# aticejiang/MLAgg-UNet

Measured on AMD Instinct MI355X. Metric: images/sec (train step) MLAgg-UNet-2D 256x256 bs10, higher is better.
Workload: dtype f32; 1 GPU; nnUNetTrainer_MLAgg_2D_dt_MS train step, AbdomenMRI-shaped 256x256x1, 14 classes, attention variant B (BASELINE.json configs[1]); batch_per_gpu=10, global_batch=10, parallelism=dp1, launch=eager, miopen=tuned find-db (mlagg-unet_amd/miopen_db), library_gemm=TunableOp table (mlagg-unet_amd/gemm_db), tuning off

## Files before the change

include/mlagg_hip.h:

```cpp
#ifndef MLAGG_HIP_H
#define MLAGG_HIP_H

#include <stddef.h>

#ifdef __cplusplus
extern "C" {
#endif

#define MLAGG_E_UNSUPPORTED (-1)
#define MLAGG_E_NULLPTR     (-2)
#define MLAGG_E_WORKSPACE   (-3)

#define MLAGG_DTYPE_F32  0
#define MLAGG_DTYPE_BF16 1
#define MLAGG_DTYPE_F16  2
#define MLAGG_DTYPE_BF16X3 3

const char *mlagg_version(void);
const char *mlagg_error_string(int code);

int mlagg_profile_kernel_count(void);
const char *mlagg_profile_kernel_name(int id);
int mlagg_profile_select(int id);
int mlagg_profile_collect(double *ms, int *counts);

size_t mlagg_selscan_state_floats(int batch, int dim, int L, int N);
int mlagg_selscan_fwd(const float *u, const float *delta, const float *A, const float *B, const float *C,
                      const float *D, const float *delta_bias, float *out, float *chunk_state,
                      int batch, int dim, int L, int N, int G, int delta_softplus, void *stream);

size_t mlagg_selscan_bwd_workspace_floats(int batch, int dim, int L, int N);
int mlagg_selscan_bwd(const float *u, const float *delta, const float *A, const float *B, const float *C,
                      const float *D, const float *delta_bias, const float *dout, const float *chunk_state,
                      float *du, float *ddelta, float *dA, float *dB, float *dC, float *dD,
                      float *ddelta_bias, float *workspace,
                      int batch, int dim, int L, int N, int G, int delta_softplus, void *stream);

int mlagg_selscan_lowrank_fwd(const float *u, const float *dtr, const float *Wdt, int R, const float *A, const float *B,
                              const float *C, const float *D, const float *delta_bias, float *out, float *chunk_state,
                              int batch, int dim, int L, int N, int G, int delta_softplus, void *stream);
int mlagg_selscan_lowrank_bwd(const float *u, const float *dtr, const float *Wdt, int R, const float *A, const float *B,
                              const float *C, const float *D, const float *delta_bias, const float *dout,
                              const float *chunk_state, float *du, float *ddtr, float *dWdt, float *dA, float *dB,
                              float *dC, float *dD, float *ddelta_bias, float *workspace, int batch, int dim, int L,
                              int N, int G, int delta_softplus, void *stream);

int mlagg_local_attn_fwd(const float *q, int q_stride, const float *kv, int kv_stride,
                         const float *lam, const float *subln_w, const float *lepe_w, const float *lepe_b,
                         float *out, int out_stride, int batch, int H, int W, int nh, float scale,
                         void *stream);
size_t mlagg_local_attn_bwd_workspace_floats(int batch, int H, int W, int nh);
int mlagg_local_attn_bwd(const float *q, int q_stride, const float *kv, int kv_stride,
                         const float *lam, const float *subln_w, const float *lepe_w,
                         const float *dout, int dout_stride,
                         float *dq, int dq_stride, float *dkv, int dkv_stride,
                         float *dlam, float *dsubln_w, float *dlepe_w, float *dlepe_b, float *workspace,
                         int batch, int H, int W, int nh, float scale, void *stream);

int mlagg_pooled_attn_fwd(const float *q, int q_stride, const float *kp, int kp_stride,
                          const float *vp, int vp_stride, const float *lam, const float *subln_w,
                          float *out, int out_stride,
                          float *lse,
                          float *o_pre,
                          int batch, int N, int P, int nh, float scale, void *stream);
size_t mlagg_pooled_attn_bwd_workspace_floats(int batch, int N, int P, int nh);
int mlagg_pooled_attn_bwd(const float *q, int q_stride, const float *kp, int kp_stride,
                          const float *vp, int vp_stride, const float *lam, const float *subln_w,
                          const float *dout, int dout_stride, const float *lse, const float *o_pre,
                          float *dq, int dq_stride, float *dkp, int dkp_stride, float *dvp, int dvp_stride,
                          float *dlam, float *dsubln_w, float *workspace,
                          int batch, int N, int P, int nh, float scale, void *stream);

int mlagg_dwconv3x3_fwd(const float *x, int x_stride, const float *w, const float *bias, const float *res, float *y,
                        int y_stride, float *pre, int batch, int H, int W, int C, int silu, void *stream);
size_t mlagg_dwconv3x3_bwd_workspace_floats(int batch, int H, int W, int C);
int mlagg_dwconv3x3_gated_fwd(const float *x, int x_stride, const float *w, const float *bias, const float *gate, int gate_stride, float *y,
                              int y_stride, float *pre, int batch, int H, int W, int C, void *stream);
int mlagg_dwconv3x3_gated_bwd(const float *x, int x_stride, const float *w, const float *dy, int dy_stride, const float *pre,
                              const float *gate, int gate_stride, float *dx, int dx_stride, float *dgate, int dgate_stride, float *dw,
                              float *dbias, float *workspace, int batch, int H, int W, int C, void *stream);
int mlagg_dwconv3x3_bwd(const float *x, int x_stride, const float *w, const float *dy, int dy_stride,
                        const float *pre, float *dx, int dx_stride, float *dw, float *dbias, float *workspace,
                        int batch, int H, int W, int C, int silu, void *stream);

int mlagg_linear_fwd(const float *x, int x_stride, const float *w, const float *bias, float *y, int y_stride,
                     int M, int N, int K, void *stream);
int mlagg_linear_dgrad(const float *dy, int dy_stride, const float *w, float *dx, int dx_stride, int M, int O, int I,
                       void *stream);
int mlagg_linear_lp_fwd(const float *x, int x_stride, const float *w, const float *bias, float *y, int y_stride,
                        int M, int N, int K, int dtype, void *stream);
int mlagg_linear_lp_dgrad(const float *dy, int dy_stride, const float *w, float *dx, int dx_stride, int M, int O, int I,
                          int dtype, void *stream);
size_t mlagg_linear_wgrad_workspace_floats(int M, int O, int I);
int mlagg_linear_wgrad(const float *dy, int dy_stride, const float *x, int x_stride, float *dW, float *db,
                       float *workspace, int M, int O, int I, void *stream);
int mlagg_linear_wgrad_x3(const float *dy, int dy_stride, const float *x, int x_stride, float *dW, float *db, float *workspace,
                          int M, int O, int I, void *stream);

int mlagg_flash_attn_fwd(const void *q, const void *k, const void *v, void *out, float *lse, int B, int N, int P, int nh,
                         int head_dim, float softmax_scale, int dtype, void *stream);
size_t mlagg_flash_attn_bwd_workspace_floats(int B, int N, int P, int nh, int head_dim);
int mlagg_flash_attn_bwd(const void *q, const void *k, const void *v, const void *out, const void *dout, const float *lse,
                         void *dq, float *workspace, int B, int N, int P, int nh, int head_dim, float softmax_scale,
                         int dtype, void *stream);

int mlagg_layernorm_supported(int C);
int mlagg_layernorm_fwd(const float *x, int x_stride, const float *gamma, const float *beta, float *y,
                        float *stats, int rows, int C, float eps, void *stream);
size_t mlagg_layernorm_bwd_workspace_floats(int rows, int C);
int mlagg_layernorm_bwd(const float *x, int x_stride, const float *dy, int dy_stride, const float *gamma,
                        const float *stats, float *dx, float *dgamma, float *dbeta, float *workspace,
                        int rows, int C, void *stream);
int mlagg_residual_layernorm_fwd(const float *skip, const float *branch, const float *scale, const float *gamma, const float *beta,
                                 float *xsum, float *y, float *stats, int rows, int rows_per_sample, int C, float eps, void *stream);
int mlagg_residual_layernorm_bwd(const float *xsum, const float *dy, int dy_stride, const float *dres, const float *scale,
                                 const float *gamma, const float *stats, float *dskip, float *dbranch, float *dgamma, float *dbeta,
                                 float *workspace, int rows, int rows_per_sample, int C, void *stream);

int mlagg_dwconv3d_fwd(const float *x, int x_stride, const float *w, const float *bias, float *y, int y_stride,
                       float *pre, int batch, int D, int H, int W, int C, int silu, void *stream);
size_t mlagg_dwconv3d_bwd_workspace_floats(int batch, int D, int H, int W, int C);
int mlagg_dwconv3d_bwd(const float *x, int x_stride, const float *w, const float *dy, int dy_stride, const float *pre,
                       float *dx, int dx_stride, float *dw, float *dbias, float *workspace, int batch, int D, int H,
                       int W, int C, int silu, void *stream);

int mlagg_dwconv3x3_nchw_fwd(const float *x, const float *w, const float *bias, float *y, int B, int C, int H, int W,
                             int stride, void *stream);
size_t mlagg_dwconv3x3_nchw_bwd_workspace_floats(int B, int C, int H, int W, int stride);
int mlagg_dwconv3x3_nchw_bwd(const float *x, const float *w, const float *dy, float *dx, float *dw, float *dbias,
                             float *workspace, int B, int C, int H, int W, int stride, void *stream);
int mlagg_dwconv3x3_nchw_bwd_res(const float *x, const float *w, const float *dy, const float *dres, float *dx, float *dw, float *dbias,
                                 float *workspace, int B, int C, int H, int W, int stride, void *stream);

int mlagg_cross_scan(const float *tok, int tok_stride, int blk_stride, float *seq, int B, int nscale,
                     const int *H, const int *W, int CB, int nblk, void *stream);
int mlagg_cross_merge(const float *seq, float *tok, int tok_stride, int blk_stride, int B, int nscale,
                      const int *H, const int *W, int CB, int nblk, void *stream);

int mlagg_conv1x1_supported(int O, int I, long P);
int mlagg_conv1x1_fwd(const float *x, long x_batch, const float *w, const float *bias, float *y, long y_batch, int B, int O, int I,
                      long P, void *stream);
size_t mlagg_conv1x1_wgrad_workspace_floats(int B, int O, int I, long P);
int mlagg_conv1x1_wgrad(const float *dy, long dy_batch, const float *x, long x_batch, float *dW, float *workspace, int B, int O,
                        int I, long P, void *stream);
int mlagg_conv1x1_fwd_lp(const float *x, long x_batch, const float *w, const float *bias, float *y, long y_batch, int B, int O, int I,
                         long P, int dtype, void *stream);
int mlagg_conv1x1_wgrad_lp(const float *dy, long dy_batch, const float *x, long x_batch, float *dW, float *workspace, int B, int O,
                           int I, long P, int dtype, void *stream);
int mlagg_conv1x1_fwd_ragged(const float *x, long x_batch, const float *w, const float *bias, float *y, long y_batch, int B, int O, int I,
                             int I_valid, long P, int dtype, void *stream);
int mlagg_conv1x1_fwd_acc(const float *x, long x_batch, const float *w, const float *bias, float *y, long y_batch, int B, int O, int I,
                          int I_valid, long P, int dtype, int accumulate, void *stream);

int mlagg_conv3x3_supported(int O, int I, int H, int W);
size_t mlagg_conv3x3_workspace_bytes(int O, int I);
int mlagg_conv3x3_fwd(const float *x, long x_batch, const float *w, int transposed, const float *bias, float *y, long y_batch,
                      void *workspace, int B, int O, int I, int H, int W, void *stream);
int mlagg_conv3x3x3_supported(int O, int I, int D, int H, int W);
size_t mlagg_conv3x3x3_workspace_bytes(int O, int I);
int mlagg_conv3x3x3_fwd(const float *x, long x_batch, const float *w, int transposed, const float *bias, float *y, long y_batch,
                        void *workspace, int B, int O, int I, int D, int H, int W, void *stream);
int mlagg_conv3x3_wgrad_supported(int O, int I, int H, int W);
int mlagg_conv3x3x3_wgrad_supported(int O, int I, int D, int H, int W);
size_t mlagg_conv3x3x3_wgrad_workspace_floats(int B, int O, int I, int D, int H, int W);
int mlagg_conv3x3x3_wgrad(const float *dy, long dy_batch, const float *x, long x_batch, float *dW, float *workspace, int B, int O,
                          int I, int D, int H, int W, void *stream);
size_t mlagg_conv3x3_wgrad_workspace_floats(int B, int O, int I, int H, int W);
int mlagg_conv3x3_wgrad(const float *dy, long dy_batch, const float *x, long x_batch, float *dW, float *workspace, int B, int O,
                        int I, int H, int W, void *stream);
int mlagg_conv3x3_fwd_lp(const float *x, long x_batch, const float *w, int transposed, const float *bias, float *y, long y_batch,
                         void *workspace, int B, int O, int I, int H, int W, int dtype, void *stream);
int mlagg_conv3x3_wgrad_lp(const float *dy, long dy_batch, const float *x, long x_batch, float *dW, float *workspace, int B, int O,
                           int I, int H, int W, int dtype, void *stream);

int mlagg_conv3x3_s2t_supported(int O, int I, int H, int W);
size_t mlagg_conv3x3_s2t_workspace_bytes(int O, int I);
int mlagg_conv3x3_s2t_fwd(const float *x, long x_batch, const float *w, float *y, long y_batch, void *workspace, int B, int O, int I,
                          int H, int W, int dtype, void *stream);
int mlagg_conv3x3_s2_dgrad(const float *dy, long dy_batch, long dy_chan_stride, long dy_row_stride, const float *w, float *dx,
                           long dx_batch, void *workspace, int B, int O, int I, int H, int W, int dtype, void *stream);
size_t mlagg_conv3x3_s2t_wgrad_workspace_floats(int B, int O, int I, int H, int W);
int mlagg_conv3x3_s2t_wgrad(const float *x, long x_batch, const float *dy, long dy_batch, long dy_chan_stride, long dy_row_stride,
                            float *dW, float *workspace, int B, int O, int I, int H, int W, int dtype, void *stream);

int mlagg_gelu_pool_fwd(const float *s, int s_stride, float *pooled, int batch, int H, int W, int d, int r, void *stream);
int mlagg_gelu_pool_bwd(const float *s, int s_stride, const float *dpooled, float *ds, int ds_stride, int batch, int H, int W, int d,
                        int r, void *stream);

int mlagg_gate_fwd(const float *a0, const float *a1, const float *act, int act_stride, float *out, long rows, int h,
                   void *stream);
int mlagg_gate_bwd(const float *dout, int dout_stride, const float *a0, const float *a1, const float *act, int act_stride,
                   float *da0, float *da1, float *dact, int dact_stride, long rows, int h, void *stream);

int mlagg_diff_lambda_fwd(const float *q1, const float *k1, const float *q2, const float *k2, float lambda_init, int n,
                          float *lam, float *saved_exp, void *stream);
int mlagg_diff_lambda_bwd(const float *dlam, const float *q1, const float *k1, const float *q2, const float *k2,
                          const float *saved_exp, int n, float *dq1, float *dk1, float *dq2, float *dk2, void *stream);
int mlagg_scaled_residual(const float *skip, const float *branch, const float *scale, float *out, int batch,
                          long per_sample, void *stream);
int mlagg_transpose_2d(const float *src, long src_batch_stride, float *dst, int batch, int R, int C, void *stream);
int mlagg_transpose_2d_into(const float *src, long src_batch_stride, float *dst, long dst_batch_stride, int batch, int R, int C,
                            void *stream);
int mlagg_pixel_shuffle2(const float *src, float *dst, int B, int O, int H, int W, int inverse, void *stream);
int mlagg_pixel_unshuffle2_strided(const float *src, long src_batch, float *dst, int B, int O, int H, int W, void *stream);
size_t mlagg_channel_sum_workspace_floats(int B, int C);
int mlagg_channel_sum(const float *g, float *out, float *workspace, int B, int C, long HW, void *stream);
size_t mlagg_column_sum_workspace_floats(int rows, int cols);
int mlagg_column_sum(const float *x, int x_stride, float *out, float *workspace, int rows, int cols, void *stream);

int mlagg_index_scan(const float *tok, long tok_stride, int blk_stride, const int *idx, float *seq, int B, int L, int K, int CB,
                     void *stream);
int mlagg_index_merge(const float *seq, const int *idx, float *tok, long tok_stride, int blk_stride, int B, int L, int K, int CB,
                      void *stream);
int mlagg_block_sum(const float *wide, float *out, long rows, int K, int CB, void *stream);

int mlagg_msmm_scan_supported(int d_inner, int d_state, int dt_rank, int directions, int L);
size_t mlagg_msmm_scan_state_floats(int batch, int L);
size_t mlagg_msmm_scan_fwd_workspace_floats(int batch, int L);
size_t mlagg_msmm_scan_bwd_workspace_floats(int batch, int L);
int mlagg_msmm_scan_fwd(const float *xc, const float *xdbl, const int *idx, const float *Wdt, const float *A, const float *D,
                        const float *delta_bias, float *y, float *state, float *workspace, int batch, int L, void *stream);
int mlagg_msmm_scan_bwd(const float *xc, const float *xdbl, const int *idx, const float *Wdt, const float *A, const float *D,
                        const float *delta_bias, const float *dy, const float *state, float *dxc, float *dxdbl, float *dWdt,
                        float *dA, float *dD, float *ddelta_bias, float *workspace, int batch, int L, void *stream);

int mlagg_selscan1_chunk(int B, int L, int K);
size_t mlagg_selscan1_state_floats(int B, int L, int C, int K);
int mlagg_selscan1_fwd(const float *tok, long tok_stride, const int *idx, const float *dtr, const float *Bs, const float *Cs,
                       const float *Wdt, int R, const float *A, const float *D, const float *bias, float *yk, float *state,
                       int B, int L, int C, int K, void *stream);
size_t mlagg_selscan1_bwd_workspace_floats(int B, int L, int C, int K, int R);
int mlagg_selscan1_bwd(const float *tok, long tok_stride, const int *idx, const float *dtr, const float *Bs, const float *Cs,
                       const float *Wdt, int R, const float *A, const float *D, const float *bias, const float *dout,
                       long dout_stride, const float *state, float *duk, float *ddtr, float *dBs, float *dCs, float *dparams,
                       float *workspace, int B, int L, int C, int K, void *stream);

int mlagg_channel_epilogue_fwd(float *x, const float *bias, const float *res, float *y, int B, int C, long HW, int act,
                               void *stream);
int mlagg_channel_gelu_bwd(const float *pre, const float *dy, float *dpre, float *dbias, float *workspace, int B, int C,
                           long HW, void *stream);
int mlagg_channel_epilogue_lp_fwd(const void *x, int x_dtype, const float *bias, const void *res, int res_dtype, void *y, int y_dtype,
                                  int B, int C, long HW, int act, void *stream);
int mlagg_channel_epilogue_lp_bwd(const void *x, int x_dtype, const float *bias, const void *res, int res_dtype, const void *dy,
                                  int dy_dtype, void *dx, int dx_dtype, float *dbias, float *workspace, int B, int C, long HW, int act,
                                  void *stream);

int mlagg_dice_ce_max_classes(void);
size_t mlagg_dice_ce_stats_workspace_floats(int B, int C, long HW);
int mlagg_dice_ce_stats(const float *logits, const float *target, float *stats_ip, float *stats_g, float *ce_sum,
                        float *workspace, int B, int C, long HW, int ignore_label, void *stream);
int mlagg_dice_ce_grad(const float *logits, const float *target, const float *g_ip, const float *g_ce, float *dlogits, int B,
                       int C, long HW, int ignore_label, void *stream);

size_t mlagg_plane_norm_fwd_workspace_floats(int B, int C, long HW);
int mlagg_plane_norm_fwd(const void *x, const float *gamma, const float *beta, const void *res, void *y, float *stats,
                         float *workspace, int B, int C, long HW, float eps, int act, float slope, int x_dtype, int res_dtype,
                         int y_dtype, void *stream);
size_t mlagg_plane_norm_bwd_workspace_floats(int B, int C, long HW);
int mlagg_plane_norm_bwd(const void *x, const void *dy, const float *gamma, const float *beta, const void *res, const float *stats,
                         void *dx, void *dres, float *dgamma, float *dbeta, float *workspace, int B, int C, long HW, int act,
                         float slope, int x_dtype, int dy_dtype, int res_dtype, void *stream);
int mlagg_plane_norm_bwd_strided(const void *x, const void *dy, long dy_batch, const float *gamma, const float *beta, const void *res,
                                 const float *stats, void *dx, void *dres, float *dgamma, float *dbeta, float *workspace, int B, int C,
                                 long HW, int act, float slope, int x_dtype, int dy_dtype, int res_dtype, void *stream);

int mlagg_pooled_attn_lp_fwd(const float *q, int q_stride, const float *kp, int kp_stride, const float *vp, int vp_stride,
                             const float *lam, const float *subln_w, float *out, int out_stride, float *lse, float *o1, float *o2,
                             int batch, int N, int P, int nh, float scale, int dtype, void *stream);
size_t mlagg_pooled_attn_lp_bwd_workspace_floats(int batch, int N, int P, int nh);
int mlagg_pooled_attn_lp_bwd(const float *q, int q_stride, const float *kp, int kp_stride, const float *vp, int vp_stride,
                             const float *lam, const float *subln_w, const float *dout, int dout_stride, const float *lse,
                             const float *o1, const float *o2, float *dq, int dq_stride, float *dkp, int dkp_stride, float *dvp,
                             int dvp_stride, float *dlam, float *dsubln_w, float *workspace, int batch, int N, int P, int nh,
                             float scale, int dtype, void *stream);

int mlagg_conv_pad_geometry(int D, int H, int W, int stride, int wide, int *Dq, int *Hq, int *Wq, long *guard);
int mlagg_volume_pad(const float *src, float *dst, int B, int C, int D, int H, int W, int stride, int wide, int as_output, int out_D,
                     int out_H, int out_W, void *stream);
size_t mlagg_conv_wgrad_taps_workspace_floats(int batch, long Q, int O, int I, int ntaps);
int mlagg_conv_taps(const float *xp, long x_batch, long x_row, const float *weight, long w_so, long w_si, int flip, const long *tap_off,
                    int ntaps, float *y, int B, int O, int I, int D, int H, int W, void *stream);
int mlagg_conv_wgrad_taps(const float *A, long a_batch, long a_row, const float *B, long b_batch, long b_row, const long *tap_off,
                          int ntaps, long Q, int O, int I, int batch, float *dW, int accumulate, float *workspace, void *stream);

size_t mlagg_weight_image_bytes(int rows, int cols);
int mlagg_weight_image(const float *w, int w_stride, void *img, void *img_t, int N, int K, void *stream);
int mlagg_weight_images(const void *jobs, int n_jobs, int max_tiles, void *stream);
int mlagg_linear_x3_supported(int M, int N, int K);
int mlagg_linear_x3(const float *x, int x_stride, const void *w_image, const float *bias, float *y, int y_stride, float *y_act,
                    const float *pre, int pre_stride, int M, int N, int K, int epilogue, void *stream);

int mlagg_adamw_chunk_elements(void);
int mlagg_adamw_clip_step(const void *tensor_table, const void *work_list, int n_work, double *sumsq, float lr, float beta1,
                          float beta2, float eps, float weight_decay, float max_norm, int step, void *stream);
int mlagg_adamw_clip_step_dev(const void *tensor_table, const void *work_list, int n_work, double *sumsq, const float *lr_dev,
                              int *step_dev, float beta1, float beta2, float eps, float weight_decay, float max_norm, void *stream);

int mlagg_sw_gather(const float *vol, int C, int X, int Y, int Z, const int *origins, int n, const int *flips, int V, float *out,
                    int tx, int ty, int tz, void *stream);
int mlagg_sw_fold(const float *out, int tile, int n, const int *flips, int V, int K, const float *gauss, int tx, int ty, int tz,
                  int ox, int oy, int oz, float *acc, float *w, int X, int Y, int Z, void *stream);
int mlagg_sw_finalize(const float *acc, const float *w, int K, int X, int Y, int Z, int lx, int ly, int lz, int X0, int Y0, int Z0,
                      float *logits, long long *labels, void *stream);

int mlagg_resample_linear(const float *in, int C, int X, int Y, int Z, long long sc, long long sx, long long sy, long long sz,
                          const int *tap_idx, const double *tap_w, float *out, int Xo, int Yo, int Zo, void *stream);
int mlagg_export_segmentation(const float *logits, int K, int X, int Y, int Z, long long sc, long long sx, long long sy, long long sz,
                              const int *tap_idx, const double *tap_w, int Xc, int Yc, int Zc, const int *box_lo, const int *shape,
                              const int *perm, unsigned char *labels, float *probs, void *stream);

#define MLAGG_PP_NONE          0
#define MLAGG_PP_CT            1
#define MLAGG_PP_ZSCORE        2
#define MLAGG_PP_ZSCORE_MASKED 3
#define MLAGG_PP_RESCALE01     4
#define MLAGG_PP_RGB01         5
#define MLAGG_PP_STATS_PARTIALS 256
int mlagg_pp_nonzero_box(const float *in, int C, int X, int Y, int Z, long long sc, long long sx, long long sy, long long sz, int *box,
                         void *stream);
int mlagg_pp_channel_stats(const float *in, int C, int X, int Y, int Z, long long sc, long long sx, long long sy, long long sz,
                           const int *lo, const int *ext, int c, int scheme, const unsigned char *mask, double *partials,
                           float *params, double *stats, void *stream);
int mlagg_pp_normalize(const float *in, int C, int X, int Y, int Z, long long sc, long long sx, long long sy, long long sz,
                       const int *lo, const int *ext, const int *schemes, const float *params, const unsigned char *mask, float *out,
                       void *stream);
int mlagg_pp_clip_ranges(const float *x, int C, int X, int Y, int Z, int axis, unsigned *lo, unsigned *hi, void *stream);
int mlagg_pp_cubic_lines_per_block(int n_in, int M);
int mlagg_pp_cubic_axis(const void *in, int in_f64, void *out, int out_f64, long long outer, int n_in, long long inner, int n_out,
                        const int *start, const double *w, int P0, int M, const double *fir, const unsigned *clip_lo,
                        const unsigned *clip_hi, long long clip_cstride, long long clip_dstride, int clip_D, void *stream);
int mlagg_pp_gather_axis(const double *in, float *out, long long outer, int n_in, long long inner, int n_out, const int *idx,
                         const double *w, void *stream);

#define MLAGG_PP_RANK_BLOCK 2048
#define MLAGG_PP_MAX_GROUPS 64
int mlagg_pp_seg_crop(const short *seg, int X, int Y, int Z, long long sx, long long sy, long long sz, const int *lo, const int *ext,
                      const unsigned char *mask, short *out, int max_label, unsigned long long *hist, void *stream);
int mlagg_pp_seg_resize(const short *in, int X, int Y, int Z, const int *tap_idx, const double *tap_w, short *out, int Xo, int Yo,
                        int Zo, int max_label, unsigned long long *hist, void *stream);
size_t mlagg_pp_rank_rows(long long N);
int mlagg_pp_rank_counts(const short *seg, long long N, const unsigned long long *groups, int max_label, int n_groups,
                         long long *table, long long *totals, void *stream);
int mlagg_pp_rank_select(const short *seg, long long N, int Y, int Z, const unsigned long long *groups, int max_label, int n_groups,
                         int group, const long long *table, const long long *totals, const long long *ranks, long long n_ranks,
                         long long *coords, const float *image, int C, long long sc, long long sx, long long sy, long long sz,
                         float *values, void *stream);

int mlagg_keep_largest_component(const unsigned char *labels, int X, int Y, int Z, const unsigned char *group, int background_label,
                                 int *parent, int *size, int *stats, unsigned char *out, void *stream);

#define MLAGG_SURFACE_STATS_PER_LABEL 10
#define MLAGG_SURFACE_DESC_FIELDS 16
#define MLAGG_SURFACE_MAX_LINE 2560
int mlagg_surface_stats(const unsigned char *gt, const unsigned char *pred, int X, int Y, int Z, const unsigned char *wanted,
                        int *stats, void *stream);
int mlagg_surface_prepare(const unsigned char *gt, const unsigned char *pred, int X, int Y, int Z, const long long *desc, int n_labels,
                          long long total, long long max_crop, long long zlines, long long ylines, int nmax_y, double s1, double s2, unsigned char *codes,
                          int *ft, int *counts, void *stream);
int mlagg_surface_reduce(const unsigned char *codes, const int *ft, const long long *desc, int n_labels, long long total,
                         long long xlines, int nmax_x, const double *tol, const double *area, double s0, double s1, double s2,
                         double *partial, double *sums, double *pairs, int *pair_count, void *stream);

int mlagg_aug3d_resample(const float *vol, const short *lab, int B, int C, int Xi, int Yi, int Zi, const double *affine,
                         const int *resample, float *out, float *out_lab, int Xo, int Yo, int Zo, void *stream);

#ifdef __cplusplus
}
#endif
#endif
```

mlagg-unet_amd/csrc/channel_epilogue.hip:

```cpp
#include <hip/hip_runtime.h>
#include <stdint.h>

#include "internal.h"
#include "lpio.h"
#include "mlagg_hip.h"
#include "prof.h"

namespace {

__device__ __forceinline__ float gelu_f(float x) { return 0.5f * x * (1.f + erff(x * 0.70710678118654752f)); }
__device__ __forceinline__ float gelu_grad_f(float x)
{
    const float cdf = 0.5f * (1.f + erff(x * 0.70710678118654752f));
    return cdf + x * 0.3989422804014327f * __expf(-0.5f * x * x);
}

template <bool GELU>
__global__ void __launch_bounds__(256)
channel_epilogue_fwd_kernel(float *__restrict__ x, const float *__restrict__ bias, const float *__restrict__ res,
                            float *__restrict__ y, int C, long HW)
{
    const int c = blockIdx.x, b = blockIdx.y;
    const size_t off = ((size_t)b * C + c) * HW;
    const float bv = bias ? bias[c] : 0.f;
    float *xp = x + off;
    const float *rp = res ? res + off : nullptr;
    float *yp = GELU ? y + off : xp;
    const long n4 = ((HW & 3) == 0) ? HW >> 2 : 0;
    for (long i = threadIdx.x; i < n4; i += 256) {
        float4 v = reinterpret_cast<float4 *>(xp)[i];
        v.x += bv; v.y += bv; v.z += bv; v.w += bv;
        if (rp) {
            const float4 r = reinterpret_cast<const float4 *>(rp)[i];
            v.x += r.x; v.y += r.y; v.z += r.z; v.w += r.w;
        }
        if (GELU) {
            reinterpret_cast<float4 *>(xp)[i] = v;
            v = make_float4(gelu_f(v.x), gelu_f(v.y), gelu_f(v.z), gelu_f(v.w));
        }
        reinterpret_cast<float4 *>(yp)[i] = v;
    }
    for (long i = 4 * n4 + threadIdx.x; i < HW; i += 256) {
        float v = xp[i] + bv + (rp ? rp[i] : 0.f);
        if (GELU) { xp[i] = v; v = gelu_f(v); }
        yp[i] = v;
    }
}

__global__ void __launch_bounds__(256)
channel_gelu_bwd_kernel(const float *__restrict__ pre, const float *__restrict__ dy, float *__restrict__ dpre,
                        float *__restrict__ part, int C, long HW)
{
    __shared__ float red[4];
    const int c = blockIdx.x, b = blockIdx.y;
    const size_t off = ((size_t)b * C + c) * HW;
    const float *pp = pre + off, *gp = dy + off;
    float *dp = dpre + off;
    float s = 0.f;
    const long n4 = ((HW & 3) == 0) ? HW >> 2 : 0;
    for (long i = threadIdx.x; i < n4; i += 256) {
        const float4 p = reinterpret_cast<const float4 *>(pp)[i], g = reinterpret_cast<const float4 *>(gp)[i];
        const float4 d = make_float4(g.x * gelu_grad_f(p.x), g.y * gelu_grad_f(p.y), g.z * gelu_grad_f(p.z), g.w * gelu_grad_f(p.w));
        reinterpret_cast<float4 *>(dp)[i] = d;
        s += (d.x + d.y) + (d.z + d.w);
    }
    for (long i = 4 * n4 + threadIdx.x; i < HW; i += 256) {
        const float d = gp[i] * gelu_grad_f(pp[i]);
        dp[i] = d;
        s += d;
    }
    if (part) {
#pragma unroll
        for (int o = 32; o > 0; o >>= 1) s += __shfl_xor(s, o, 64);
        if ((threadIdx.x & 63) == 0) red[threadIdx.x >> 6] = s;
        __syncthreads();
        if (threadIdx.x == 0) part[(size_t)b * C + c] = (red[0] + red[1]) + (red[2] + red[3]);
    }
}

using namespace mlagg_lpio;

template <bool GELU>
__global__ void __launch_bounds__(256)
channel_epilogue_lp_fwd_kernel(const void *__restrict__ x, int xdt, const float *__restrict__ bias, const void *__restrict__ res, int rdt,
                               void *__restrict__ y, int ydt, int C, long HW)
{
    const int c = blockIdx.x, b = blockIdx.y;
    const long plane = (long)b * C + c;
    const float bv = bias ? bias[c] : 0.f;
    const void *xp = plane_ptr(x, plane, HW, xdt);
    const void *rp = res ? plane_ptr(res, plane, HW, rdt) : nullptr;
    void *yp = plane_ptr(y, plane, HW, ydt);
    const long n4 = HW >> 2;
    constexpr int UN = 4;
    for (long i0 = threadIdx.x; i0 < n4; i0 += 256 * UN) {
        float4 v[UN], r[UN];
#pragma unroll
        for (int u = 0; u < UN; ++u) {
            const long i = min(i0 + 256 * u, n4 - 1);
            v[u] = ld4(xp, i, xdt);
            r[u] = rp ? ld4(rp, i, rdt) : make_float4(0.f, 0.f, 0.f, 0.f);
        }
#pragma unroll
        for (int u = 0; u < UN; ++u) {
            const long i = i0 + 256 * u;
            if (i < n4) {
                float4 o = make_float4(v[u].x + bv + r[u].x, v[u].y + bv + r[u].y, v[u].z + bv + r[u].z, v[u].w + bv + r[u].w);
                if (GELU) o = make_float4(gelu_f(o.x), gelu_f(o.y), gelu_f(o.z), gelu_f(o.w));
                st4(yp, i, ydt, o);
            }
        }
    }
}

template <bool GELU>
__global__ void __launch_bounds__(256)
channel_epilogue_lp_bwd_kernel(const void *__restrict__ x, int xdt, const float *__restrict__ bias, const void *__restrict__ res, int rdt,
                               const void *__restrict__ dy, int gdt, void *__restrict__ dx, int dxdt, float *__restrict__ part, int C,
                               long HW)
{
    __shared__ float red[4];
    const int c = blockIdx.x, b = blockIdx.y;
    const long plane = (long)b * C + c;
    const float bv = (GELU && bias) ? bias[c] : 0.f;
    const void *xp = GELU ? plane_ptr(x, plane, HW, xdt) : nullptr;
    const void *rp = (GELU && res) ? plane_ptr(res, plane, HW, rdt) : nullptr;
    const void *gp = plane_ptr(dy, plane, HW, gdt);
    void *dp = plane_ptr(dx, plane, HW, dxdt);
    const long n4 = HW >> 2;
    float s = 0.f;
    constexpr int UN = 4;
    for (long i0 = threadIdx.x; i0 < n4; i0 += 256 * UN) {
        float4 v[UN], r[UN], g[UN];
#pragma unroll
        for (int u = 0; u < UN; ++u) {
            const long i = min(i0 + 256 * u, n4 - 1);
            g[u] = ld4(gp, i, gdt);
            v[u] = GELU ? ld4(xp, i, xdt) : make_float4(0.f, 0.f, 0.f, 0.f);
            r[u] = rp ? ld4(rp, i, rdt) : make_float4(0.f, 0.f, 0.f, 0.f);
        }
#pragma unroll
        for (int u = 0; u < UN; ++u) {
            const long i = i0 + 256 * u;
            if (i < n4) {
                float4 d = g[u];
                if (GELU)
                    d = make_float4(d.x * gelu_grad_f(v[u].x + bv + r[u].x), d.y * gelu_grad_f(v[u].y + bv + r[u].y),
                                    d.z * gelu_grad_f(v[u].z + bv + r[u].z), d.w * gelu_grad_f(v[u].w + bv + r[u].w));
                st4(dp, i, dxdt, d);
                s += (d.x + d.y) + (d.z + d.w);
            }
        }
    }
    if (part) {
#pragma unroll
        for (int o = 32; o > 0; o >>= 1) s += __shfl_xor(s, o, 64);
        if ((threadIdx.x & 63) == 0) red[threadIdx.x >> 6] = s;
        __syncthreads();
        if (threadIdx.x == 0) part[plane] = (red[0] + red[1]) + (red[2] + red[3]);
    }
}

inline bool lp_ok(int dt) { return dt == MLAGG_DTYPE_F32 || dt == MLAGG_DTYPE_BF16 || dt == MLAGG_DTYPE_F16; }
inline bool lp_aligned(const void *p, int dt) { return (((uintptr_t)p) & (dt == 0 ? 15 : 7)) == 0; }

}

extern "C" int mlagg_channel_epilogue_lp_fwd(const void *x, int x_dtype, const float *bias, const void *res, int res_dtype, void *y,
                                             int y_dtype, int B, int C, long HW, int act, void *stream)
{
    if (!x || !y) return MLAGG_E_NULLPTR;
    if (B <= 0 || C <= 0 || HW <= 0 || B > 65535 || (HW & 3) || (act != 0 && act != 1)) return MLAGG_E_UNSUPPORTED;
    if (!lp_ok(x_dtype) || !lp_ok(y_dtype) || (res && !lp_ok(res_dtype))) return MLAGG_E_UNSUPPORTED;
    if (!lp_aligned(x, x_dtype) || !lp_aligned(y, y_dtype) || (res && !lp_aligned(res, res_dtype))) return MLAGG_E_UNSUPPORTED;
    hipStream_t st = static_cast<hipStream_t>(stream);
    MLAGG_TIMED(K_CHANNEL_EPI, st);
    if (act == 1) hipLaunchKernelGGL(channel_epilogue_lp_fwd_kernel<true>, dim3(C, B), dim3(256), 0, st, x, x_dtype, bias, res, res_dtype, y, y_dtype, C, HW);
    else hipLaunchKernelGGL(channel_epilogue_lp_fwd_kernel<false>, dim3(C, B), dim3(256), 0, st, x, x_dtype, bias, res, res_dtype, y, y_dtype, C, HW);
    return (int)hipGetLastError();
}

extern "C" int mlagg_channel_epilogue_lp_bwd(const void *x, int x_dtype, const float *bias, const void *res, int res_dtype,
                                             const void *dy, int dy_dtype, void *dx, int dx_dtype, float *dbias, float *workspace,
                                             int B, int C, long HW, int act, void *stream)
{
    if (!dy || !dx || (act == 1 && !x) || (dbias && !workspace)) return MLAGG_E_NULLPTR;
    if (B <= 0 || C <= 0 || HW <= 0 || B > 65535 || (HW & 3) || (act != 0 && act != 1)) return MLAGG_E_UNSUPPORTED;
    if (!lp_ok(dy_dtype) || !lp_ok(dx_dtype) || (act == 1 && !lp_ok(x_dtype)) || (act == 1 && res && !lp_ok(res_dtype))) return MLAGG_E_UNSUPPORTED;
    if (!lp_aligned(dy, dy_dtype) || !lp_aligned(dx, dx_dtype) || (act == 1 && !lp_aligned(x, x_dtype)) ||
        (act == 1 && res && !lp_aligned(res, res_dtype)))
        return MLAGG_E_UNSUPPORTED;
    hipStream_t st = static_cast<hipStream_t>(stream);
    MLAGG_TIMED(K_CHANNEL_EPI, st);
    float *part = dbias ? workspace : nullptr;
    if (act == 1) hipLaunchKernelGGL(channel_epilogue_lp_bwd_kernel<true>, dim3(C, B), dim3(256), 0, st, x, x_dtype, bias, res, res_dtype, dy, dy_dtype, dx, dx_dtype, part, C, HW);
    else hipLaunchKernelGGL(channel_epilogue_lp_bwd_kernel<false>, dim3(C, B), dim3(256), 0, st, x, x_dtype, bias, res, res_dtype, dy, dy_dtype, dx, dx_dtype, part, C, HW);
    if (dbias)
        hipLaunchKernelGGL(mlagg_internal::column_sum_kernel<false>, dim3((C + 63) / 64), dim3(1024), 0, st, workspace, B, C, C, dbias);
    return (int)hipGetLastError();
}

extern "C" int mlagg_channel_epilogue_fwd(float *x, const float *bias, const float *res, float *y, int B, int C, long HW, int act,
                                          void *stream)
{
    if (!x || (act == 1 && !y)) return MLAGG_E_NULLPTR;
    if (B <= 0 || C <= 0 || HW <= 0 || B > 65535 || (act != 0 && act != 1)) return MLAGG_E_UNSUPPORTED;
    if ((((uintptr_t)x) & 15) || (res && (((uintptr_t)res) & 15)) || (y && (((uintptr_t)y) & 15))) return MLAGG_E_UNSUPPORTED;
    hipStream_t st = static_cast<hipStream_t>(stream);
    MLAGG_TIMED(K_CHANNEL_EPI, st);
    if (act == 1) hipLaunchKernelGGL(channel_epilogue_fwd_kernel<true>, dim3(C, B), dim3(256), 0, st, x, bias, res, y, C, HW);
    else hipLaunchKernelGGL(channel_epilogue_fwd_kernel<false>, dim3(C, B), dim3(256), 0, st, x, bias, res, y, C, HW);
    return (int)hipGetLastError();
}

extern "C" int mlagg_channel_gelu_bwd(const float *pre, const float *dy, float *dpre, float *dbias, float *workspace, int B, int C,
                                      long HW, void *stream)
{
    if (!pre || !dy || !dpre || (dbias && !workspace)) return MLAGG_E_NULLPTR;
    if (B <= 0 || C <= 0 || HW <= 0 || B > 65535) return MLAGG_E_UNSUPPORTED;
    if ((((uintptr_t)pre) & 15) || (((uintptr_t)dy) & 15) || (((uintptr_t)dpre) & 15)) return MLAGG_E_UNSUPPORTED;
    hipStream_t st = static_cast<hipStream_t>(stream);
    MLAGG_TIMED(K_CHANNEL_EPI, st);
    hipLaunchKernelGGL(channel_gelu_bwd_kernel, dim3(C, B), dim3(256), 0, st, pre, dy, dpre, dbias ? workspace : nullptr, C, HW);
    if (dbias)
        hipLaunchKernelGGL(mlagg_internal::column_sum_kernel<false>, dim3((C + 63) / 64), dim3(1024), 0, st, workspace, B, C, C, dbias);
    return (int)hipGetLastError();
}
```

mlagg-unet_amd/csrc/conv1x1.hip:

```cpp
#include <hip/hip_runtime.h>

#include <cstdlib>

#include "mlagg_hip.h"
#include "prof.h"
#include "bf16x3.h"
#include "opmode.h"
#include "internal.h"

namespace {

using bf16x3::f32x16;

template <int T>
struct __attribute__((packed, aligned(4))) FVec {
    float v[T];
};

struct C1Geom {
    int B, O, I, P;
    long x_batch, y_batch;
    int I_valid;
    int accumulate;
};

using opmode::split8;

template <int TO, int TP, int DT>
__global__ void __launch_bounds__(64)
conv1x1_fwd_kernel(const float *__restrict__ X, const float *__restrict__ W, const float *__restrict__ bias, float *__restrict__ Y,
                   C1Geom g)
{
    const int lane = threadIdx.x, col = lane & 31, kh = lane >> 5;
    const int p0 = blockIdx.x * (32 * TP), o0 = blockIdx.y * (32 * TO), b = blockIdx.z;
    f32x16 acc[TO][TP];
#pragma unroll
    for (int a = 0; a < TO; ++a)
#pragma unroll
        for (int j = 0; j < TP; ++j)
#pragma unroll
            for (int r = 0; r < 16; ++r) acc[a][j][r] = 0.f;
    const int pnat = p0 + TP * col, pc = min(pnat, g.P - TP);
    const float *xb = X + (size_t)b * g.x_batch + pc;
    const int lastrow = g.I_valid - 1;
    const float *wb[TO];
#pragma unroll
    for (int a = 0; a < TO; ++a) wb[a] = W + (size_t)min(o0 + 32 * a + col, g.O - 1) * g.I + 8 * kh;
    const int nblk = g.I / 16;
    float4 wa[2][TO][2];
    FVec<TP> xv[2][8];
    auto fetch = [&](float4 (&A)[TO][2], FVec<TP> (&Xv)[8], int blk) {
        const int kb = 16 * min(blk, nblk - 1);
#pragma unroll
        for (int t = 0; t < 8; ++t) Xv[t] = *reinterpret_cast<const FVec<TP> *>(xb + (size_t)min(kb + 8 * kh + t, lastrow) * g.P);
#pragma unroll
        for (int a = 0; a < TO; ++a) {
            A[a][0] = *reinterpret_cast<const float4 *>(wb[a] + kb);
            A[a][1] = *reinterpret_cast<const float4 *>(wb[a] + kb + 4);
        }
    };
    auto consume = [&](const float4 (&A)[TO][2], const FVec<TP> (&Xv)[8]) {
        uint4 bq[TP][3];
#pragma unroll
        for (int j = 0; j < TP; ++j) {
            const float f[8] = {Xv[0].v[j], Xv[1].v[j], Xv[2].v[j], Xv[3].v[j], Xv[4].v[j], Xv[5].v[j], Xv[6].v[j], Xv[7].v[j]};
            split8<DT>(f, bq[j]);
        }
        uint4 aq[TO][3];
#pragma unroll
        for (int a = 0; a < TO; ++a) {
            const float f[8] = {A[a][0].x, A[a][0].y, A[a][0].z, A[a][0].w, A[a][1].x, A[a][1].y, A[a][1].z, A[a][1].w};
            split8<DT>(f, aq[a]);
        }
        opmode::mfma_tiles<DT, TO, TP>(aq, bq, acc);
    };
    fetch(wa[0], xv[0], 0);
    int blk = 0;
    for (; blk + 2 <= nblk; blk += 2) {
        fetch(wa[1], xv[1], blk + 1);
        consume(wa[0], xv[0]);
        fetch(wa[0], xv[0], blk + 2);
        consume(wa[1], xv[1]);
    }
    if (blk < nblk) consume(wa[0], xv[0]);
    float *yb = Y + (size_t)b * g.y_batch + pc;
#pragma unroll
    for (int a = 0; a < TO; ++a) {
#pragma unroll
        for (int r = 0; r < 16; ++r) {
            const int o = o0 + 32 * a + (r & 3) + 8 * (r >> 2) + 4 * kh;
            if (o >= g.O) continue;
            const float bv = bias ? bias[o] : 0.f;
            float *dst = yb + (size_t)o * g.P;
            if (pc == pnat) {
                FVec<TP> v;
#pragma unroll
                for (int j = 0; j < TP; ++j) v.v[j] = acc[a][j][r] + bv;
                if (g.accumulate) {
                    const FVec<TP> old = *reinterpret_cast<const FVec<TP> *>(dst);
#pragma unroll
                    for (int j = 0; j < TP; ++j) v.v[j] += old.v[j];
                }
                *reinterpret_cast<FVec<TP> *>(dst) = v;
            } else {
#pragma unroll
                for (int j = 0; j < TP; ++j)
                    if (pc + j >= pnat) dst[j] = acc[a][j][r] + bv + (g.accumulate ? dst[j] : 0.f);
            }
        }
    }
}

struct W1Geom {
    int B, O, I, P;
    long dy_batch, x_batch;
    int slab, nslabs;
};

template <int TO, int TI, int DT>
__global__ void __launch_bounds__(64)
conv1x1_wgrad_kernel(const float *__restrict__ dY, const float *__restrict__ X, float *__restrict__ part, W1Geom g)
{
    const int lane = threadIdx.x, col = lane & 31, kh = lane >> 5;
    const int b = blockIdx.x / g.nslabs, s = blockIdx.x % g.nslabs;
    const int o0 = blockIdx.y * (32 * TO), i0 = blockIdx.z * (32 * TI);
    f32x16 acc[TO][TI];
#pragma unroll
    for (int a = 0; a < TO; ++a)
#pragma unroll
        for (int j = 0; j < TI; ++j)
#pragma unroll
            for (int r = 0; r < 16; ++r) acc[a][j][r] = 0.f;
    const int pb = s * g.slab, pe = min(pb + g.slab, g.P);
    const int nblk = (pe - pb) / 16;
    const float *ap[TO], *bp[TI];
#pragma unroll
    for (int a = 0; a < TO; ++a) ap[a] = dY + (size_t)b * g.dy_batch + (size_t)min(o0 + 32 * a + col, g.O - 1) * g.P + pb + 8 * kh;
#pragma unroll
    for (int j = 0; j < TI; ++j) bp[j] = X + (size_t)b * g.x_batch + (size_t)min(i0 + 32 * j + col, g.I - 1) * g.P + pb + 8 * kh;
    float4 av[2][TO][2], bv[2][TI][2];
    auto fetch = [&](float4 (&A)[TO][2], float4 (&Bv)[TI][2], int blk) {
        const int off = 16 * min(blk, nblk - 1);
#pragma unroll
        for (int a = 0; a < TO; ++a) {
            A[a][0] = *reinterpret_cast<const float4 *>(ap[a] + off);
            A[a][1] = *reinterpret_cast<const float4 *>(ap[a] + off + 4);
        }
#pragma unroll
        for (int j = 0; j < TI; ++j) {
            Bv[j][0] = *reinterpret_cast<const float4 *>(bp[j] + off);
            Bv[j][1] = *reinterpret_cast<const float4 *>(bp[j] + off + 4);
        }
    };
    auto consume = [&](const float4 (&A)[TO][2], const float4 (&Bv)[TI][2]) {
        uint4 bq[TI][3];
#pragma unroll
        for (int j = 0; j < TI; ++j) {
            const float f[8] = {Bv[j][0].x, Bv[j][0].y, Bv[j][0].z, Bv[j][0].w, Bv[j][1].x, Bv[j][1].y, Bv[j][1].z, Bv[j][1].w};
            split8<DT>(f, bq[j]);
        }
        uint4 aq[TO][3];
#pragma unroll
        for (int a = 0; a < TO; ++a) {
            const float f[8] = {A[a][0].x, A[a][0].y, A[a][0].z, A[a][0].w, A[a][1].x, A[a][1].y, A[a][1].z, A[a][1].w};
            split8<DT>(f, aq[a]);
        }
        opmode::mfma_tiles<DT, TO, TI>(aq, bq, acc);
    };
    if (nblk > 0) {
        fetch(av[0], bv[0], 0);
        int blk = 0;
        for (; blk + 2 <= nblk; blk += 2) {
            fetch(av[1], bv[1], blk + 1);
            consume(av[0], bv[0]);
            fetch(av[0], bv[0], blk + 2);
            consume(av[1], bv[1]);
        }
        if (blk < nblk) consume(av[0], bv[0]);
    }
    float *prow = part + (size_t)blockIdx.x * ((size_t)g.O * g.I);
#pragma unroll
    for (int a = 0; a < TO; ++a) {
#pragma unroll
        for (int j = 0; j < TI; ++j) {
            const int i = i0 + 32 * j + col;
            if (i >= g.I) continue;
#pragma unroll
            for (int r = 0; r < 16; ++r) {
                const int o = o0 + 32 * a + (r & 3) + 8 * (r >> 2) + 4 * kh;
                if (o < g.O) prow[(size_t)o * g.I + i] = acc[a][j][r];
            }
        }
    }
}

int make_wgeom(W1Geom &g, int B, int O, int I, int P, long dy_batch, long x_batch)
{
    if (B <= 0 || O <= 0 || I <= 0 || P <= 0 || (P & 15)) return MLAGG_E_UNSUPPORTED;
    if (dy_batch < (long)O * P || x_batch < (long)I * P || ((dy_batch | x_batch) & 3)) return MLAGG_E_UNSUPPORTED;
    g = W1Geom{B, O, I, P, dy_batch, x_batch, 0, 0};
    const int og = (O + 95) / 96, ig = (I + 95) / 96;
    static const int target = [] { const char *e = getenv("MLAGG_K18_WAVES"); const int v = e ? atoi(e) : 0; return v > 0 ? v : 1536; }();
    int per_sample = (target + B * og * ig - 1) / (B * og * ig);
    if (per_sample < 1) per_sample = 1;
    int slab = (P + per_sample - 1) / per_sample;
    slab = ((slab + 15) / 16) * 16;
    if (slab < 64) slab = 64;
    g.slab = slab;
    g.nslabs = (P + slab - 1) / slab;
    if ((long)B * g.nslabs > 2147483647L || og > 65535 || ig > 65535) return MLAGG_E_UNSUPPORTED;
    return 0;
}

void pick_fwd_tile(int B, int O, int I, int P, int &to, int &tp)
{
    static const char *env = getenv("MLAGG_K18_TILE");
    if (env && env[0] >= '1' && env[0] <= '3' && env[1] == ',' && env[2] >= '1' && env[2] <= '3') {
        to = env[0] - '0';
        tp = env[2] - '0';
        if (32 * (to - 1) >= O) to = (O + 31) / 32;
    }
}

template <int TO, int TP>
void launch_fwd(const float *x, const float *w, const float *bias, float *y, const C1Geom &g, int dt, hipStream_t st)
{
    const dim3 grid((g.P + 32 * TP - 1) / (32 * TP), (g.O + 32 * TO - 1) / (32 * TO), g.B);
    if (dt == MLAGG_DTYPE_BF16)
        hipLaunchKernelGGL((conv1x1_fwd_kernel<TO, TP, MLAGG_DTYPE_BF16>), grid, dim3(64), 0, st, x, w, bias, y, g);
    else if (dt == MLAGG_DTYPE_F16)
        hipLaunchKernelGGL((conv1x1_fwd_kernel<TO, TP, MLAGG_DTYPE_F16>), grid, dim3(64), 0, st, x, w, bias, y, g);
    else
        hipLaunchKernelGGL((conv1x1_fwd_kernel<TO, TP, MLAGG_DTYPE_BF16X3>), grid, dim3(64), 0, st, x, w, bias, y, g);
}

template <int TO, int TI>
void launch_wgrad(const float *dy, const float *x, float *part, const W1Geom &g, int dt, hipStream_t st)
{
    const dim3 grid(g.B * g.nslabs, (g.O + 32 * TO - 1) / (32 * TO), (g.I + 32 * TI - 1) / (32 * TI));
    if (dt == MLAGG_DTYPE_BF16)
        hipLaunchKernelGGL((conv1x1_wgrad_kernel<TO, TI, MLAGG_DTYPE_BF16>), grid, dim3(64), 0, st, dy, x, part, g);
    else if (dt == MLAGG_DTYPE_F16)
        hipLaunchKernelGGL((conv1x1_wgrad_kernel<TO, TI, MLAGG_DTYPE_F16>), grid, dim3(64), 0, st, dy, x, part, g);
    else
        hipLaunchKernelGGL((conv1x1_wgrad_kernel<TO, TI, MLAGG_DTYPE_BF16X3>), grid, dim3(64), 0, st, dy, x, part, g);
}

}

extern "C" int mlagg_conv1x1_supported(int O, int I, long P)
{
    return O > 0 && I > 0 && (I % 16) == 0 && P >= 96 && (P % 16) == 0 && P < (1L << 30);
}

extern "C" int mlagg_conv1x1_fwd_ragged(const float *x, long x_batch, const float *w, const float *bias, float *y, long y_batch, int B,
                                        int O, int I, int I_valid, long P, int dtype, void *stream)
{
    return mlagg_conv1x1_fwd_acc(x, x_batch, w, bias, y, y_batch, B, O, I, I_valid, P, dtype, 0, stream);
}

extern "C" int mlagg_conv1x1_fwd_acc(const float *x, long x_batch, const float *w, const float *bias, float *y, long y_batch, int B,
                                     int O, int I, int I_valid, long P, int dtype, int accumulate, void *stream)
{
    if (!x || !w || !y) return MLAGG_E_NULLPTR;
    if (!opmode::valid(dtype) || I_valid <= 0 || I_valid > I) return MLAGG_E_UNSUPPORTED;
    if (B <= 0 || B > 65535 || !mlagg_conv1x1_supported(O, I, P)) return MLAGG_E_UNSUPPORTED;
    if (x_batch < (long)I_valid * P || y_batch < (long)O * P || (reinterpret_cast<uintptr_t>(w) & 15)) return MLAGG_E_UNSUPPORTED;
    C1Geom g{B, O, I, (int)P, x_batch, y_batch, I_valid, accumulate ? 1 : 0};
    hipStream_t st = static_cast<hipStream_t>(stream);
    MLAGG_TIMED(K_CONV1X1, st);
    int to = O <= 32 ? 1 : (O <= 64 ? 2 : 3), tp = O <= 64 ? 3 : 2;
    pick_fwd_tile(B, O, I, (int)P, to, tp);
    switch (to * 4 + tp) {
    case 1 * 4 + 1: launch_fwd<1, 1>(x, w, bias, y, g, dtype, st); break;
    case 1 * 4 + 2: launch_fwd<1, 2>(x, w, bias, y, g, dtype, st); break;
    case 1 * 4 + 3: launch_fwd<1, 3>(x, w, bias, y, g, dtype, st); break;
    case 2 * 4 + 1: launch_fwd<2, 1>(x, w, bias, y, g, dtype, st); break;
    case 2 * 4 + 2: launch_fwd<2, 2>(x, w, bias, y, g, dtype, st); break;
    case 2 * 4 + 3: launch_fwd<2, 3>(x, w, bias, y, g, dtype, st); break;
    case 3 * 4 + 1: launch_fwd<3, 1>(x, w, bias, y, g, dtype, st); break;
    case 3 * 4 + 2: launch_fwd<3, 2>(x, w, bias, y, g, dtype, st); break;
    default: launch_fwd<3, 3>(x, w, bias, y, g, dtype, st); break;
    }
    return (int)hipGetLastError();
}

extern "C" int mlagg_conv1x1_fwd_lp(const float *x, long x_batch, const float *w, const float *bias, float *y, long y_batch, int B,
                                    int O, int I, long P, int dtype, void *stream)
{
    return mlagg_conv1x1_fwd_ragged(x, x_batch, w, bias, y, y_batch, B, O, I, I, P, dtype, stream);
}

extern "C" int mlagg_conv1x1_fwd(const float *x, long x_batch, const float *w, const float *bias, float *y, long y_batch, int B,
                                 int O, int I, long P, void *stream)
{
    return mlagg_conv1x1_fwd_lp(x, x_batch, w, bias, y, y_batch, B, O, I, P, MLAGG_DTYPE_BF16X3, stream);
}

extern "C" size_t mlagg_conv1x1_wgrad_workspace_floats(int B, int O, int I, long P)
{
    W1Geom g;
    if (P >= (1L << 30) || make_wgeom(g, B, O, I, (int)P, (long)O * P, (long)I * P)) return 0;
    return (size_t)B * g.nslabs * O * I;
}

extern "C" int mlagg_conv1x1_wgrad_lp(const float *dy, long dy_batch, const float *x, long x_batch, float *dW, float *workspace, int B,
                                      int O, int I, long P, int dtype, void *stream)
{
    if (!dy || !x || !dW || !workspace) return MLAGG_E_NULLPTR;
    if (!opmode::valid(dtype)) return MLAGG_E_UNSUPPORTED;
    if (P >= (1L << 30)) return MLAGG_E_UNSUPPORTED;
    W1Geom g;
    if (int rc = make_wgeom(g, B, O, I, (int)P, dy_batch, x_batch)) return rc;
    if ((reinterpret_cast<uintptr_t>(dy) | reinterpret_cast<uintptr_t>(x)) & 15) return MLAGG_E_UNSUPPORTED;
    hipStream_t st = static_cast<hipStream_t>(stream);
    MLAGG_TIMED(K_CONV1X1, st);
    const int to = O > 64 ? 3 : (O + 31) / 32, ti = I > 64 ? 3 : (I + 31) / 32;
    switch (to * 4 + ti) {
    case 1 * 4 + 1: launch_wgrad<1, 1>(dy, x, workspace, g, dtype, st); break;
    case 1 * 4 + 2: launch_wgrad<1, 2>(dy, x, workspace, g, dtype, st); break;
    case 1 * 4 + 3: launch_wgrad<1, 3>(dy, x, workspace, g, dtype, st); break;
    case 2 * 4 + 1: launch_wgrad<2, 1>(dy, x, workspace, g, dtype, st); break;
    case 2 * 4 + 2: launch_wgrad<2, 2>(dy, x, workspace, g, dtype, st); break;
    case 2 * 4 + 3: launch_wgrad<2, 3>(dy, x, workspace, g, dtype, st); break;
    case 3 * 4 + 1: launch_wgrad<3, 1>(dy, x, workspace, g, dtype, st); break;
    case 3 * 4 + 2: launch_wgrad<3, 2>(dy, x, workspace, g, dtype, st); break;
    default: launch_wgrad<3, 3>(dy, x, workspace, g, dtype, st); break;
    }
    const int n = O * I;
    hipLaunchKernelGGL(mlagg_internal::column_sum_kernel<false>, dim3((n + 63) / 64), dim3(1024), 0, st, workspace, B * g.nslabs, n, n,
                       dW);
    return (int)hipGetLastError();
}

extern "C" int mlagg_conv1x1_wgrad(const float *dy, long dy_batch, const float *x, long x_batch, float *dW, float *workspace, int B,
                                   int O, int I, long P, void *stream)
{
    return mlagg_conv1x1_wgrad_lp(dy, dy_batch, x, x_batch, dW, workspace, B, O, I, P, MLAGG_DTYPE_BF16X3, stream);
}
```

mlagg-unet_amd/csrc/conv3x3.hip:

```cpp
#include <hip/hip_runtime.h>

#include <cstdlib>

#include "mlagg_hip.h"
#include "prof.h"
#include "bf16x3.h"
#include "opmode.h"

namespace {

using bf16x3::f32x16;
typedef unsigned u32x4 __attribute__((ext_vector_type(4)));

template <int T>
struct __attribute__((packed, aligned(4))) FVec {
    float v[T];
};

struct C3Geom {
    int B, O, I, D, H, W, P;
    long x_batch, y_batch;
};

template <int DT>
__global__ void __launch_bounds__(256)
conv3x3_weight_image_kernel(const float *__restrict__ w, unsigned short *__restrict__ img, int O, int I, int ntaps, int flip)
{
    const int n = ntaps * O * I;
    const int idx = blockIdx.x * blockDim.x + threadIdx.x;
    if (idx >= n) return;
    const int i = idx % I, o = (idx / I) % O, t = idx / (I * O);
    const float v = flip ? w[((size_t)i * O + o) * ntaps + (ntaps - 1 - t)] : w[((size_t)o * I + i) * ntaps + t];
    unsigned short p[3];
    opmode::pieces<DT>(v, p);
#pragma unroll
    for (int q = 0; q < opmode::Form<DT>::NQ; ++q) img[(size_t)q * n + idx] = p[q];
}

#ifndef K19_INTERLEAVE
#define K19_INTERLEAVE 0
#endif
constexpr int WAVES = 4;

#ifndef K19_OCC3
#define K19_OCC3 1
#endif
template <int TO, int TP, int NR, int DT>
__global__ void __launch_bounds__(64 * WAVES, (K19_OCC3 && NR == 3 && TO <= 2 && TO * TP <= 4) ? 3 : 2)
conv3x3_kernel(const float *__restrict__ X, const unsigned short *__restrict__ Wimg, const float *__restrict__ bias,
               float *__restrict__ Y, C3Geom g)
{
    constexpr int ROWS = 32 * TO;
    constexpr int NQ = opmode::Form<DT>::NQ, NT = opmode::Form<DT>::NT;
    constexpr int STAGE = 3 * NQ * ROWS * 2;
    constexpr int WL = (STAGE + 64 * WAVES - 1) / (64 * WAVES);
    __shared__ u32x4 sW[2][STAGE];
    const int tid = threadIdx.x, lane = tid & 63, wave = tid >> 6, col = lane & 31, kh = lane >> 5;
    const int p0 = (blockIdx.x * WAVES + wave) * (32 * TP), o0 = blockIdx.y * ROWS, b = blockIdx.z;
    f32x16 acc[TO][TP];
#pragma unroll
    for (int a = 0; a < TO; ++a)
#pragma unroll
        for (int j = 0; j < TP; ++j)
#pragma unroll
            for (int r = 0; r < 16; ++r) acc[a][j][r] = 0.f;
    const int pnat = p0 + TP * col, pc = max(min(pnat, g.P - TP), 0);
    const int x0 = pc % g.W, yz = pc / g.W, y0 = yz % g.H, z0 = yz / g.H;
    bool row_ok[NR];
#pragma unroll
    for (int r = 0; r < NR; ++r) {
        const int kz = NR == 9 ? r / 3 : 1, ky = NR == 9 ? r % 3 : r;
        row_ok[r] = (unsigned)(z0 + kz - 1) < (unsigned)g.D && (unsigned)(y0 + ky - 1) < (unsigned)g.H;
    }
    const bool left_ok = x0 > 0, right_ok = x0 + TP < g.W;
    const __amdgpu_buffer_rsrc_t xrs = __builtin_amdgcn_make_buffer_rsrc(const_cast<float *>(X + (size_t)b * g.x_batch), 0, 0x7fffffff, 0x00020000);
    constexpr unsigned OOB = 0x80000000u;
    unsigned offc[NR], offl[NR], offr[NR];
#pragma unroll
    for (int r = 0; r < NR; ++r) {
        const int kz = NR == 9 ? r / 3 : 1, ky = NR == 9 ? r % 3 : r;
        const int q = pc + (kz - 1) * g.H * g.W + (ky - 1) * g.W;
        offc[r] = row_ok[r] ? 4u * (unsigned)(8 * kh * g.P + q) : OOB;
        offl[r] = (row_ok[r] && left_ok) ? 4u * (unsigned)(8 * kh * g.P + q - 1) : OOB;
        offr[r] = (row_ok[r] && right_ok) ? 4u * (unsigned)(8 * kh * g.P + q + TP) : OOB;
    }
    const size_t img = (size_t)(3 * NR) * g.O * g.I;
    const size_t tstride = (size_t)g.O * g.I;
    const int nblk = g.I / 16, nstage = NR * nblk;
    unsigned wsrc[WL];
#pragma unroll
    for (int i = 0; i < WL; ++i) {
        const int e = min(tid + 64 * WAVES * i, STAGE - 1);
        const int h = e & 1, row = (e >> 1) % ROWS, q = ((e >> 1) / ROWS) % NQ, tt = (e >> 1) / (NQ * ROWS);
        wsrc[i] = 2u * (unsigned)(q * img + tt * tstride + (size_t)min(o0 + row, g.O - 1) * g.I + 8 * h);
    }
    u32x4 wreg[WL];
#define K19_WFETCH(S)                                                                                                         \
    {                                                                                                                         \
        const int sc_ = min((S), nstage - 1), blk_ = sc_ / NR, srow_ = sc_ - NR * blk_;                                       \
        const char *base_ = reinterpret_cast<const char *>(Wimg + (size_t)(3 * srow_) * tstride + 16 * blk_);                \
        _Pragma("unroll") for (int i_ = 0; i_ < WL; ++i_) wreg[i_] = *reinterpret_cast<const u32x4 *>(base_ + (size_t)wsrc[i_]); \
    }
#define K19_WSTORE(BUF)                                                                                                       \
    {                                                                                                                         \
        _Pragma("unroll") for (int i_ = 0; i_ < WL; ++i_) sW[(BUF)][min(tid + 64 * WAVES * i_, STAGE - 1)] = wreg[i_];        \
    }
    FVec<TP> xc[2][8];
    float xl[2][8], xr[2][8];
    auto xfetch = [&](FVec<TP> (&C)[8], float (&L)[8], float (&R)[8], int blk_, int ky) __attribute__((always_inline)) {
        const int blk = min(blk_, nblk - 1);
#pragma unroll
        for (int r = 0; r < 8; ++r) {
            const unsigned so = 4u * (unsigned)((16 * blk + r) * g.P);
            if constexpr (TP == 1) {
                C[r].v[0] = __builtin_bit_cast(float, __builtin_amdgcn_raw_buffer_load_b32(xrs, offc[ky], so, 0));
            } else {
                static_assert(TP == 2, "pixel runs of one or two");
                C[r].v[0] = __builtin_bit_cast(float, __builtin_amdgcn_raw_buffer_load_b32(xrs, offc[ky], so, 0));
                C[r].v[1] = __builtin_bit_cast(float, __builtin_amdgcn_raw_buffer_load_b32(xrs, offc[ky] + 4u, so, 0));
            }
            L[r] = __builtin_bit_cast(float, __builtin_amdgcn_raw_buffer_load_b32(xrs, offl[ky], so, 0));
            R[r] = __builtin_bit_cast(float, __builtin_amdgcn_raw_buffer_load_b32(xrs, offr[ky], so, 0));
        }
    };
    auto consume = [&](const u32x4 *wst, const FVec<TP> (&C)[8], const float (&L)[8], const float (&R)[8], int ky)
                       __attribute__((always_inline)) {
        uint4 src[TP + 2][3];
#pragma unroll
        for (int m = 0; m < TP + 2; ++m) {
            float f[8];
#pragma unroll
            for (int r = 0; r < 8; ++r) f[r] = m == 0 ? L[r] : (m == TP + 1 ? R[r] : C[r].v[(m >= 1 && m <= TP) ? m - 1 : 0]);
            opmode::split8<DT>(f, src[m]);
        }
#if K19_INTERLEAVE
#pragma unroll
        for (int i = 0; i < 3 * NT * TO * TP; ++i) {
            __builtin_amdgcn_sched_group_barrier(0x008, 1, 0);
            __builtin_amdgcn_sched_group_barrier(0x002, K19_INTERLEAVE, 0);
        }
#endif
#pragma unroll
        for (int tt = 0; tt < 3; ++tt) {
            uint4 aq[TO][3];
#pragma unroll
            for (int a = 0; a < TO; ++a)
#pragma unroll
                for (int q = 0; q < NQ; ++q) {
                    const u32x4 v = wst[(tt * NQ + q) * ROWS * 2 + (32 * a + col) * 2 + kh];
                    aq[a][q] = make_uint4(v.x, v.y, v.z, v.w);
                }
#pragma unroll
            for (int term = 0; term < NT; ++term)
#pragma unroll
                for (int a = 0; a < TO; ++a)
#pragma unroll
                    for (int j = 0; j < TP; ++j)
                        acc[a][j] = opmode::mfma<DT>(aq[a][opmode::Form<DT>::termA(term)], src[j + tt][opmode::Form<DT>::termB(term)], acc[a][j]);
        }
    };
    auto stage = [&](int blk_, int ky, int par) __attribute__((always_inline)) {
        K19_WFETCH(NR * blk_ + ky + 1)
        xfetch(xc[par ^ 1], xl[par ^ 1], xr[par ^ 1], ky == NR - 1 ? blk_ + 1 : blk_, ky == NR - 1 ? 0 : ky + 1);
        consume(sW[par], xc[par], xl[par], xr[par], ky);
        K19_WSTORE(par ^ 1)
        __syncthreads();
    };
    K19_WFETCH(0)
    K19_WSTORE(0)
    xfetch(xc[0], xl[0], xr[0], 0, 0);
    __syncthreads();
    int blk = 0;
#pragma unroll 1
    for (; blk + 2 <= nblk; blk += 2) {
#pragma unroll
        for (int r = 0; r < NR; ++r) stage(blk, r, r & 1);
#pragma unroll
        for (int r = 0; r < NR; ++r) stage(blk + 1, r, (r + 1) & 1);
    }
    if (blk < nblk) {
#pragma unroll
        for (int r = 0; r < NR; ++r) stage(blk, r, r & 1);
    }
    float *yb = Y + (size_t)b * g.y_batch + pc;
#pragma unroll
    for (int a = 0; a < TO; ++a) {
#pragma unroll
        for (int r = 0; r < 16; ++r) {
            const int o = o0 + 32 * a + (r & 3) + 8 * (r >> 2) + 4 * kh;
            if (o >= g.O) continue;
            const float bv = bias ? bias[o] : 0.f;
            float *dst = yb + (size_t)o * g.P;
            if (pc == pnat) {
                FVec<TP> v;
#pragma unroll
                for (int j = 0; j < TP; ++j) v.v[j] = acc[a][j][r] + bv;
                *reinterpret_cast<FVec<TP> *>(dst) = v;
            } else {
#pragma unroll
                for (int j = 0; j < TP; ++j)
                    if (pc + j >= pnat && pnat < g.P) dst[j] = acc[a][j][r] + bv;
            }
        }
    }
}

#undef K19_WFETCH
#undef K19_WSTORE

struct W3Geom {
    int B, O, I, D, H, W, P;
    int nz;
    long dy_batch, x_batch;
    int slab, nslabs;
    long x_last;
};

template <int DT>
__global__ void __launch_bounds__(64)
conv3x3_wgrad_kernel(const float *__restrict__ dY, const float *__restrict__ X, float *__restrict__ part, W3Geom g)
{
    const int lane = threadIdx.x, col = lane & 31, kh = lane >> 5;
    const int kz = (int)(blockIdx.x % g.nz) + (g.nz == 1 ? 1 : 0);
    const int bs = blockIdx.x / g.nz, b = bs / g.nslabs, s = bs % g.nslabs;
    const int o0 = blockIdx.y * 32, i0 = blockIdx.z * 32;
    f32x16 acc[1][9];
#pragma unroll
    for (int t = 0; t < 9; ++t)
#pragma unroll
        for (int r = 0; r < 16; ++r) acc[0][t][r] = 0.f;
    const int pb = s * g.slab, pe = min(pb + g.slab, g.P);
    const int nblk = (pe - pb) / 16;
    const int oc = min(o0 + col, g.O - 1), ic = min(i0 + col, g.I - 1);
    const float *ap = dY + (size_t)b * g.dy_batch + (size_t)oc * g.P + pb + 8 * kh;
    const long xrow = (long)b * g.x_batch + (long)ic * g.P + pb + 8 * kh;
    float4 av[2][2], bv[2][2];
    float be[2][2];
    auto fetch = [&](float4 (&A)[2], float4 (&Bv)[2], float (&E)[2], int blk, int ky) __attribute__((always_inline)) {
        const int bc = min(blk, nblk - 1);
        if (ky == 0) {
            A[0] = *reinterpret_cast<const float4 *>(ap + 16 * bc);
            A[1] = *reinterpret_cast<const float4 *>(ap + 16 * bc + 4);
        }
        const long want = xrow + 16 * bc + (long)(ky - 1) * g.W + (long)(kz - 1) * g.H * g.W;
        const long at = min(max(want, 0L), g.x_last);
        Bv[0] = *reinterpret_cast<const float4 *>(X + at);
        Bv[1] = *reinterpret_cast<const float4 *>(X + at + 4);
        E[0] = X[min(max(want - 1, 0L), g.x_last + 7)];
        E[1] = X[min(max(want + 8, 0L), g.x_last + 7)];
    };
    uint4 aq[1][3];
    auto consume = [&](const float4 (&A)[2], const float4 (&Bv)[2], const float (&E)[2], int blk, int ky) __attribute__((always_inline)) {
        if (ky == 0) {
            const float f[8] = {A[0].x, A[0].y, A[0].z, A[0].w, A[1].x, A[1].y, A[1].z, A[1].w};
            opmode::split8<DT>(f, aq[0]);
        }
        const int p = pb + 16 * blk + 8 * kh;
        const int x0 = p % g.W, yz = p / g.W, y = yz % g.H, z = yz / g.H;
        const bool rok = (unsigned)(y + ky - 1) < (unsigned)g.H && (unsigned)(z + kz - 1) < (unsigned)g.D;
        if (!__any(rok)) return;
        const float left = (!rok || x0 == 0) ? 0.f : E[0];
        const float right = (!rok || x0 + 8 == g.W) ? 0.f : E[1];
        float4 c0 = Bv[0], c1 = Bv[1];
        if (!rok) c0 = c1 = make_float4(0.f, 0.f, 0.f, 0.f);
        unsigned d[3][5];
        opmode::split<DT>(left, c0.x, d[0][0], d[1][0], d[2][0]);
        opmode::split<DT>(c0.y, c0.z, d[0][1], d[1][1], d[2][1]);
        opmode::split<DT>(c0.w, c1.x, d[0][2], d[1][2], d[2][2]);
        opmode::split<DT>(c1.y, c1.z, d[0][3], d[1][3], d[2][3]);
        opmode::split<DT>(c1.w, right, d[0][4], d[1][4], d[2][4]);
        uint4 bq[3][3];
#pragma unroll
        for (int q = 0; q < opmode::Form<DT>::NQ; ++q) {
            bq[0][q] = make_uint4(d[q][0], d[q][1], d[q][2], d[q][3]);
            bq[2][q] = make_uint4(d[q][1], d[q][2], d[q][3], d[q][4]);
            bq[1][q] = make_uint4(__builtin_amdgcn_alignbit(d[q][1], d[q][0], 16), __builtin_amdgcn_alignbit(d[q][2], d[q][1], 16),
                                  __builtin_amdgcn_alignbit(d[q][3], d[q][2], 16), __builtin_amdgcn_alignbit(d[q][4], d[q][3], 16));
        }
#pragma unroll
        for (int term = 0; term < opmode::Form<DT>::NT; ++term)
#pragma unroll
            for (int kx = 0; kx < 3; ++kx)
                acc[0][3 * ky + kx] = opmode::mfma<DT>(aq[0][opmode::Form<DT>::termA(term)], bq[kx][opmode::Form<DT>::termB(term)],
                                                       acc[0][3 * ky + kx]);
    };
    if (nblk > 0) {
        fetch(av[0], bv[0], be[0], 0, 0);
#pragma unroll 1
        for (int blk = 0; blk < nblk; blk += 2) {
            fetch(av[1], bv[1], be[1], blk, 1);
            consume(av[0], bv[0], be[0], blk, 0);
            fetch(av[0], bv[0], be[0], blk, 2);
            consume(av[0], bv[1], be[1], blk, 1);
            fetch(av[1], bv[1], be[1], blk + 1, 0);
            consume(av[0], bv[0], be[0], blk, 2);
            if (blk + 1 < nblk) {
                fetch(av[0], bv[0], be[0], blk + 1, 1);
                consume(av[1], bv[1], be[1], blk + 1, 0);
                fetch(av[1], bv[1], be[1], blk + 1, 2);
                consume(av[1], bv[0], be[0], blk + 1, 1);
                fetch(av[0], bv[0], be[0], blk + 2, 0);
                consume(av[1], bv[1], be[1], blk + 1, 2);
            }
        }
    }
    const int ntaps = 9 * g.nz, t0 = g.nz == 1 ? 0 : 9 * kz;
    float *prow = part + (size_t)bs * ((size_t)ntaps * g.O * g.I);
    const int i = i0 + col;
#pragma unroll
    for (int t = 0; t < 9; ++t)
#pragma unroll
        for (int r = 0; r < 16; ++r) {
            const int o = o0 + (r & 3) + 8 * (r >> 2) + 4 * kh;
            if (o < g.O && i < g.I) prow[((size_t)(t0 + t) * g.O + o) * g.I + i] = acc[0][t][r];
        }
}

__global__ void __launch_bounds__(1024)
conv3x3_wgrad_reduce_kernel(const float *__restrict__ part, int nparts, int O, int I, int ntaps, float *__restrict__ dW)
{
    __shared__ float red[16][65];
    const int n = ntaps * O * I;
    const int cx = threadIdx.x & 63, rg = threadIdx.x >> 6;
    const int idx = blockIdx.x * 64 + cx;
    float s0 = 0.f, s1 = 0.f;
    if (idx < n) {
        int r = rg;
        for (; r + 16 < nparts; r += 32) {
            s0 += part[(size_t)r * n + idx];
            s1 += part[(size_t)(r + 16) * n + idx];
        }
        if (r < nparts) s0 += part[(size_t)r * n + idx];
    }
    red[rg][cx] = s0 + s1;
    __syncthreads();
    if (rg == 0 && idx < n) {
        float v = 0.f;
#pragma unroll
        for (int k = 0; k < 16; ++k) v += red[k][cx];
        const int i = idx % I, o = (idx / I) % O, t = idx / (I * O);
        dW[((size_t)o * I + i) * ntaps + t] = v;
    }
}

struct W16Geom {
    int B, O, I, H, W, P;
    long dy_batch, x_batch;
    int slab, nslabs, nbs;
    long x_last;
    int q32, r32;
};

template <int TO, int TI, int DT>
__global__ void __launch_bounds__(64)
conv3x3_wgrad16_kernel(const float *__restrict__ dY, const float *__restrict__ X, float *__restrict__ part, W16Geom g)
{
    using opmode::f32x4;
    constexpr int NQ = opmode::Form<DT>::NQ, NT = opmode::Form<DT>::NT;
    const int lane = threadIdx.x, r16 = lane & 15, kg = lane >> 4;
    const int id = blockIdx.x, slot = id >> 3;
    const int ky = slot % 3, bs = (slot / 3) * 8 + (id & 7);
    if (bs >= g.nbs) return;
    const int b = bs / g.nslabs, s = bs % g.nslabs;
    const int o0 = blockIdx.y * (16 * TO), i0 = blockIdx.z * (16 * TI);
    f32x4 acc[TO][TI][3];
#pragma unroll
    for (int a = 0; a < TO; ++a)
#pragma unroll
        for (int j = 0; j < TI; ++j)
#pragma unroll
            for (int kx = 0; kx < 3; ++kx) acc[a][j][kx] = f32x4{0.f, 0.f, 0.f, 0.f};
    const int pb = s * g.slab, pe = min(pb + g.slab, g.P);
    const int nblk = (pe - pb + 31) / 32;
    const float *ap[TO];
    long xrow[TI];
#pragma unroll
    for (int a = 0; a < TO; ++a) ap[a] = dY + (size_t)b * g.dy_batch + (size_t)min(o0 + 16 * a + r16, g.O - 1) * g.P;
#pragma unroll
    for (int j = 0; j < TI; ++j) xrow[j] = (long)b * g.x_batch + (long)min(i0 + 16 * j + r16, g.I - 1) * g.P + (long)(ky - 1) * g.W;
    struct Raw {
        float4 a[TO][2], b[TI][2];
        float e[TI][2];
    };
    auto fetch = [&](Raw &R, int blk) __attribute__((always_inline)) {
        const int p = min(pb + 32 * min(blk, nblk - 1) + 8 * kg, g.P - 8);
#pragma unroll
        for (int a = 0; a < TO; ++a) {
            R.a[a][0] = *reinterpret_cast<const float4 *>(ap[a] + p);
            R.a[a][1] = *reinterpret_cast<const float4 *>(ap[a] + p + 4);
        }
#pragma unroll
        for (int j = 0; j < TI; ++j) {
            const long want = xrow[j] + p;
            const long at = min(max(want, 0L), g.x_last);
            R.b[j][0] = *reinterpret_cast<const float4 *>(X + at);
            R.b[j][1] = *reinterpret_cast<const float4 *>(X + at + 4);
            R.e[j][0] = X[min(max(want - 1, 0L), g.x_last + 7)];
            R.e[j][1] = X[min(max(want + 8, 0L), g.x_last + 7)];
        }
    };
    int x0 = (pb + 8 * kg) % g.W, y = (pb + 8 * kg) / g.W, pl = pb + 8 * kg;
    auto consume = [&](const Raw &R) __attribute__((always_inline)) {
        const bool live = pl < pe;
        const bool rok = (unsigned)(y + ky - 1) < (unsigned)g.H;
        if (__any(live && rok)) {
            uint4 aq[TO][3];
#pragma unroll
            for (int a = 0; a < TO; ++a) {
                float f[8] = {R.a[a][0].x, R.a[a][0].y, R.a[a][0].z, R.a[a][0].w, R.a[a][1].x, R.a[a][1].y, R.a[a][1].z, R.a[a][1].w};
#pragma unroll
                for (int k = 0; k < 8; ++k) f[k] = live ? f[k] : 0.f;
                opmode::split8<DT>(f, aq[a]);
            }
#pragma unroll
            for (int j = 0; j < TI; ++j) {
                float4 c0 = R.b[j][0], c1 = R.b[j][1];
                if (!rok) c0 = c1 = make_float4(0.f, 0.f, 0.f, 0.f);
                const float left = (!rok || x0 == 0) ? 0.f : R.e[j][0];
                const float right = (!rok || x0 + 8 == g.W) ? 0.f : R.e[j][1];
                unsigned d[3][5];
                opmode::split<DT>(left, c0.x, d[0][0], d[1][0], d[2][0]);
                opmode::split<DT>(c0.y, c0.z, d[0][1], d[1][1], d[2][1]);
                opmode::split<DT>(c0.w, c1.x, d[0][2], d[1][2], d[2][2]);
                opmode::split<DT>(c1.y, c1.z, d[0][3], d[1][3], d[2][3]);
                opmode::split<DT>(c1.w, right, d[0][4], d[1][4], d[2][4]);
                uint4 bq[3][3];
#pragma unroll
                for (int q = 0; q < NQ; ++q) {
                    bq[0][q] = make_uint4(d[q][0], d[q][1], d[q][2], d[q][3]);
                    bq[2][q] = make_uint4(d[q][1], d[q][2], d[q][3], d[q][4]);
                    bq[1][q] = make_uint4(__builtin_amdgcn_alignbit(d[q][1], d[q][0], 16), __builtin_amdgcn_alignbit(d[q][2], d[q][1], 16),
                                          __builtin_amdgcn_alignbit(d[q][3], d[q][2], 16), __builtin_amdgcn_alignbit(d[q][4], d[q][3], 16));
                }
#pragma unroll
                for (int term = 0; term < NT; ++term)
#pragma unroll
                    for (int a = 0; a < TO; ++a)
#pragma unroll
                        for (int kx = 0; kx < 3; ++kx)
                            acc[a][j][kx] = opmode::mfma16<DT>(aq[a][opmode::Form<DT>::termA(term)], bq[kx][opmode::Form<DT>::termB(term)],
                                                               acc[a][j][kx]);
            }
        }
        pl += 32;
        x0 += g.r32;
        y += g.q32;
        if (x0 >= g.W) {
            x0 -= g.W;
            ++y;
        }
    };
    Raw r0, r1;
    fetch(r0, 0);
    int blk = 0;
#pragma unroll 1
    for (; blk + 1 < nblk; blk += 2) {
        fetch(r1, blk + 1);
        consume(r0);
        fetch(r0, blk + 2);
        consume(r1);
    }
    if (blk < nblk) consume(r0);
    float *prow = part + (size_t)bs * ((size_t)9 * g.O * g.I) + (size_t)(3 * ky) * g.O * g.I;
#pragma unroll
    for (int a = 0; a < TO; ++a)
#pragma unroll
        for (int j = 0; j < TI; ++j) {
            const int i = i0 + 16 * j + r16;
#pragma unroll
            for (int kx = 0; kx < 3; ++kx)
#pragma unroll
                for (int r = 0; r < 4; ++r) {
                    const int o = o0 + 16 * a + 4 * kg + r;
                    if (o < g.O && i < g.I) prow[((size_t)kx * g.O + o) * g.I + i] = acc[a][j][kx][r];
                }
        }
}

template <int TO, int TI, int DT>
__global__ void __launch_bounds__(64)
conv3x3_wgrad16_lds_kernel(const float *__restrict__ dY, const float *__restrict__ X, float *__restrict__ part, W16Geom g, long dy_last)
{
    using opmode::f32x4;
    constexpr int NQ = opmode::Form<DT>::NQ, NT = opmode::Form<DT>::NT;
    constexpr int AP = 36, BP = 44;
    constexpr int AROWS = 16 * TO, BROWS = 16 * TI;
    constexpr int NLA = AROWS / 8;
    constexpr int NLB = (BROWS * 10 + 63) / 64;
    __shared__ float sA[2][AROWS * AP];
    __shared__ float sB[2][BROWS * BP];
    const int lane = threadIdx.x, r16 = lane & 15, kg = lane >> 4;
    const int id = blockIdx.x, slot = id >> 3;
    const int ky = slot % 3, bs = (slot / 3) * 8 + (id & 7);
    if (bs >= g.nbs) return;
    const int b = bs / g.nslabs, s = bs % g.nslabs;
    const int o0 = blockIdx.y * (16 * TO), i0 = blockIdx.z * (16 * TI);
    f32x4 acc[TO][TI][3];
#pragma unroll
    for (int a = 0; a < TO; ++a)
#pragma unroll
        for (int j = 0; j < TI; ++j)
#pragma unroll
            for (int kx = 0; kx < 3; ++kx) acc[a][j][kx] = f32x4{0.f, 0.f, 0.f, 0.f};
    const int pb = s * g.slab, pe = min(pb + g.slab, g.P);
    const int nblk = (pe - pb + 31) / 32;
    int offA[NLA], offB[NLB];
    int ldsA[NLA], ldsB[NLB];
#pragma unroll
    for (int m = 0; m < NLA; ++m) {
        const int row = 8 * m + (lane >> 3), c = lane & 7;
        offA[m] = min(o0 + row, g.O - 1) * g.P + 4 * c;
        ldsA[m] = row * AP + 4 * c;
    }
#pragma unroll
    for (int m = 0; m < NLB; ++m) {
        const int idx = 64 * m + lane, row = min(idx / 10, BROWS - 1), c = idx % 10;
        offB[m] = min(i0 + row, g.I - 1) * g.P + 4 * c;
        ldsB[m] = row * BP + 4 * c;
    }
    const long baseA = (long)b * g.dy_batch + pb;
    const long baseB = (long)b * g.x_batch + pb + (long)(ky - 1) * g.W - 4;
    opmode::f32x4 ga[NLA], gb[NLB];
    auto fetch = [&](int blk) __attribute__((always_inline)) {
        const long ua = baseA + 32L * min(blk, nblk - 1), ub = baseB + 32L * min(blk, nblk - 1);
        const int hiA = (int)min(dy_last - ua, 0x7fffffffL);
        const int loB = (int)min(max(-ub, 0L), 0x7fffffffL), hiB = (int)min(g.x_last + 4 - ub, 0x7fffffffL);
        const float *pa = dY + ua, *pbx = X + ub;
#pragma unroll
        for (int m = 0; m < NLA; ++m) ga[m] = *reinterpret_cast<const opmode::f32x4 *>(pa + min(offA[m], hiA));
#pragma unroll
        for (int m = 0; m < NLB; ++m) gb[m] = *reinterpret_cast<const opmode::f32x4 *>(pbx + min(max(offB[m], loB), hiB));
    };
    auto stage = [&](int buf) __attribute__((always_inline)) {
#pragma unroll
        for (int m = 0; m < NLA; ++m) *reinterpret_cast<opmode::f32x4 *>(&sA[buf][ldsA[m]]) = ga[m];
#pragma unroll
        for (int m = 0; m < NLB; ++m) *reinterpret_cast<opmode::f32x4 *>(&sB[buf][ldsB[m]]) = gb[m];
    };
    int x0 = (pb + 8 * kg) % g.W, y = (pb + 8 * kg) / g.W, pl = pb + 8 * kg;
    auto consume = [&](int buf) __attribute__((always_inline)) {
        const bool live = pl < pe;
        const bool rok = (unsigned)(y + ky - 1) < (unsigned)g.H;
        if (__any(live && rok)) {
            uint4 aq[TO][3];
#pragma unroll
            for (int a = 0; a < TO; ++a) {
                const float *src = &sA[buf][(16 * a + r16) * AP + 8 * kg];
                const float4 v0 = *reinterpret_cast<const float4 *>(src), v1 = *reinterpret_cast<const float4 *>(src + 4);
                float f[8] = {v0.x, v0.y, v0.z, v0.w, v1.x, v1.y, v1.z, v1.w};
#pragma unroll
                for (int k = 0; k < 8; ++k) f[k] = live ? f[k] : 0.f;
                opmode::split8<DT>(f, aq[a]);
            }
#pragma unroll
            for (int j = 0; j < TI; ++j) {
                const float *src = &sB[buf][(16 * j + r16) * BP + 8 * kg];
                float4 c0 = *reinterpret_cast<const float4 *>(src + 4), c1 = *reinterpret_cast<const float4 *>(src + 8);
                if (!rok) c0 = c1 = make_float4(0.f, 0.f, 0.f, 0.f);
                const float left = (!rok || x0 == 0) ? 0.f : src[3];
                const float right = (!rok || x0 + 8 == g.W) ? 0.f : src[12];
                unsigned d[3][5];
                opmode::split<DT>(left, c0.x, d[0][0], d[1][0], d[2][0]);
                opmode::split<DT>(c0.y, c0.z, d[0][1], d[1][1], d[2][1]);
                opmode::split<DT>(c0.w, c1.x, d[0][2], d[1][2], d[2][2]);
                opmode::split<DT>(c1.y, c1.z, d[0][3], d[1][3], d[2][3]);
                opmode::split<DT>(c1.w, right, d[0][4], d[1][4], d[2][4]);
                uint4 bq[3][3];
#pragma unroll
                for (int q = 0; q < NQ; ++q) {
                    bq[0][q] = make_uint4(d[q][0], d[q][1], d[q][2], d[q][3]);
                    bq[2][q] = make_uint4(d[q][1], d[q][2], d[q][3], d[q][4]);
                    bq[1][q] = make_uint4(__builtin_amdgcn_alignbit(d[q][1], d[q][0], 16), __builtin_amdgcn_alignbit(d[q][2], d[q][1], 16),
                                          __builtin_amdgcn_alignbit(d[q][3], d[q][2], 16), __builtin_amdgcn_alignbit(d[q][4], d[q][3], 16));
                }
#pragma unroll
                for (int term = 0; term < NT; ++term)
#pragma unroll
                    for (int a = 0; a < TO; ++a)
#pragma unroll
                        for (int kx = 0; kx < 3; ++kx)
                            acc[a][j][kx] = opmode::mfma16<DT>(aq[a][opmode::Form<DT>::termA(term)], bq[kx][opmode::Form<DT>::termB(term)],
                                                               acc[a][j][kx]);
            }
        }
        pl += 32;
        x0 += g.r32;
        y += g.q32;
        if (x0 >= g.W) {
            x0 -= g.W;
            ++y;
        }
    };
    fetch(0);
    stage(0);
    fetch(1);
    int blk = 0;
#pragma unroll 1
    for (; blk + 1 < nblk; blk += 2) {
        consume(0);
        stage(1);
        fetch(blk + 2);
        consume(1);
        stage(0);
        fetch(blk + 3);
    }
    if (blk < nblk) consume(0);
    float *prow = part + (size_t)bs * ((size_t)9 * g.O * g.I) + (size_t)(3 * ky) * g.O * g.I;
#pragma unroll
    for (int a = 0; a < TO; ++a)
#pragma unroll
        for (int j = 0; j < TI; ++j) {
            const int i = i0 + 16 * j + r16;
#pragma unroll
            for (int kx = 0; kx < 3; ++kx)
#pragma unroll
                for (int r = 0; r < 4; ++r) {
                    const int o = o0 + 16 * a + 4 * kg + r;
                    if (o < g.O && i < g.I) prow[((size_t)kx * g.O + o) * g.I + i] = acc[a][j][kx][r];
                }
        }
}

int make_w16geom(W16Geom &g, int B, int O, int I, int H, int W, long dy_batch, long x_batch, int to, int ti)
{
    if (B <= 0 || O <= 0 || I <= 0 || H <= 0 || W <= 0 || (W & 7)) return MLAGG_E_UNSUPPORTED;
    const long P = (long)H * W;
    if (P >= (1L << 28) || dy_batch < (long)O * P || x_batch < (long)I * P || ((dy_batch | x_batch) & 3)) return MLAGG_E_UNSUPPORTED;
    g = W16Geom{B, O, I, H, W, (int)P, dy_batch, x_batch, 0, 0, 0, (long)(B - 1) * x_batch + (long)I * P - 8, 32 / W, 32 % W};
    const int og = (O + 16 * to - 1) / (16 * to), ig = (I + 16 * ti - 1) / (16 * ti);
    static const int target = [] { const char *e = getenv("MLAGG_K19W16_WAVES"); const int v = e ? atoi(e) : 0; return v > 0 ? v : 2048; }();
    int per_sample = (target + B * og * ig * 3 - 1) / (B * og * ig * 3);
    const long cap = (256L << 20) / (4L * 9 * O * I) / B;
    if (per_sample > cap) per_sample = (int)cap;
    if (per_sample < 1) per_sample = 1;
    int slab = (int)((P + per_sample - 1) / per_sample);
    slab = ((slab + 31) / 32) * 32;
    if (slab < 256) slab = 256;
    g.slab = slab;
    g.nslabs = (int)((P + slab - 1) / slab);
    if ((long)B * g.nslabs > (1L << 26) || og > 65535 || ig > 65535) return MLAGG_E_UNSUPPORTED;
    g.nbs = B * g.nslabs;
    return 0;
}

int w16_tiles(int O, int I, int dt, int &to, int &ti)
{
    static const int mode = [] { const char *e = getenv("MLAGG_K19W16"); return e ? atoi(e) : -1; }();
    if (!mode) return 0;
    to = 3;
    ti = I <= 16 ? 1 : 3;
    return mode < 0 ? (dt == MLAGG_DTYPE_BF16X3 ? 1 : 2) : mode;
}

int make_w3geom(W3Geom &g, int B, int O, int I, int D, int H, int W, long dy_batch, long x_batch)
{
    if (B <= 0 || O <= 0 || I <= 0 || D <= 0 || H <= 0 || W <= 0 || (W & 7)) return MLAGG_E_UNSUPPORTED;
    const long P = (long)D * H * W;
    if ((P & 15) || P >= (1L << 28) || dy_batch < (long)O * P || x_batch < (long)I * P || ((dy_batch | x_batch) & 3)) return MLAGG_E_UNSUPPORTED;
    g = W3Geom{B, O, I, D, H, W, (int)P, D > 1 ? 3 : 1, dy_batch, x_batch, 0, 0, (long)(B - 1) * x_batch + (long)I * P - 8};
    const int og = (O + 31) / 32, ig = (I + 31) / 32;
    static const int target = [] { const char *e = getenv("MLAGG_K19W_WAVES"); const int v = e ? atoi(e) : 0; return v > 0 ? v : 2048; }();
    int per_sample = (target + B * og * ig * g.nz - 1) / (B * og * ig * g.nz);
    const long cap = (256L << 20) / (4L * 9 * g.nz * O * I) / B;
    if (per_sample > cap) per_sample = (int)cap;
    if (per_sample < 1) per_sample = 1;
    int slab = (int)((P + per_sample - 1) / per_sample);
    slab = ((slab + 15) / 16) * 16;
    if (slab < 64) slab = 64;
    g.slab = slab;
    g.nslabs = (int)((P + slab - 1) / slab);
    if ((long)B * g.nslabs > 2147483647L || og > 65535 || ig > 65535) return MLAGG_E_UNSUPPORTED;
    return 0;
}


template <int TO, int TP>
void launch(const float *x, const unsigned short *wimg, const float *bias, float *y, const C3Geom &g, int dt, hipStream_t st)
{
    const int groups = (g.P + 32 * TP - 1) / (32 * TP);
    const dim3 grid((groups + WAVES - 1) / WAVES, (g.O + 32 * TO - 1) / (32 * TO), g.B);
    if (g.D > 1)
        hipLaunchKernelGGL((conv3x3_kernel<TO, TP, 9, MLAGG_DTYPE_BF16X3>), grid, dim3(64 * WAVES), 0, st, x, wimg, bias, y, g);
    else if (dt == MLAGG_DTYPE_BF16)
        hipLaunchKernelGGL((conv3x3_kernel<TO, TP, 3, MLAGG_DTYPE_BF16>), grid, dim3(64 * WAVES), 0, st, x, wimg, bias, y, g);
    else if (dt == MLAGG_DTYPE_F16)
        hipLaunchKernelGGL((conv3x3_kernel<TO, TP, 3, MLAGG_DTYPE_F16>), grid, dim3(64 * WAVES), 0, st, x, wimg, bias, y, g);
    else
        hipLaunchKernelGGL((conv3x3_kernel<TO, TP, 3, MLAGG_DTYPE_BF16X3>), grid, dim3(64 * WAVES), 0, st, x, wimg, bias, y, g);
}

}

namespace {
constexpr long K19_MAX_PLANE = (1LL << 32) / 36 - 1;

int conv_fwd(const float *x, long x_batch, const float *w, int transposed, const float *bias, float *y, long y_batch, void *workspace,
             int B, int O, int I, int D, int H, int W, int dt, void *stream)
{
    if (!x || !w || !y || !workspace) return MLAGG_E_NULLPTR;
    if (!opmode::valid(dt) || (D > 1 && dt != MLAGG_DTYPE_BF16X3)) return MLAGG_E_UNSUPPORTED;
    const long P = (long)D * H * W;
    if (B <= 0 || B > 65535 || O <= 0 || I <= 0 || (I % 16) || D <= 0 || H <= 0 || W <= 0 || P < 96 || P > K19_MAX_PLANE)
        return MLAGG_E_UNSUPPORTED;
    if (x_batch < (long)I * P || y_batch < (long)O * P || (reinterpret_cast<uintptr_t>(workspace) & 15)) return MLAGG_E_UNSUPPORTED;
    if ((long)I * P * 4 >= (1L << 31) - 64) return MLAGG_E_UNSUPPORTED;
    C3Geom g{B, O, I, D, H, W, (int)P, x_batch, y_batch};
    hipStream_t st = static_cast<hipStream_t>(stream);
    MLAGG_TIMED(K_CONV3X3, st);
    unsigned short *img = static_cast<unsigned short *>(workspace);
    const int ntaps = D > 1 ? 27 : 9;
    const int n = ntaps * O * I;
    const dim3 igrid((n + 255) / 256);
    if (dt == MLAGG_DTYPE_BF16)
        hipLaunchKernelGGL(conv3x3_weight_image_kernel<MLAGG_DTYPE_BF16>, igrid, dim3(256), 0, st, w, img, O, I, ntaps, transposed ? 1 : 0);
    else if (dt == MLAGG_DTYPE_F16)
        hipLaunchKernelGGL(conv3x3_weight_image_kernel<MLAGG_DTYPE_F16>, igrid, dim3(256), 0, st, w, img, O, I, ntaps, transposed ? 1 : 0);
    else
        hipLaunchKernelGGL(conv3x3_weight_image_kernel<MLAGG_DTYPE_BF16X3>, igrid, dim3(256), 0, st, w, img, O, I, ntaps, transposed ? 1 : 0);
    int to = O <= 32 ? 1 : 2, tp = 2;
    if (O % 96 == 0 && P >= 16384) {
        to = 3;
        tp = P >= 65536 ? 2 : 1;
    }
    if (W % tp) tp = 1;
    static const char *env = getenv("MLAGG_K19_TILE");
    if (env && env[0] >= '1' && env[0] <= '3' && env[1] == ',' && env[2] >= '1' && env[2] <= '3') {
        to = env[0] - '0';
        tp = env[2] - '0';
        if (32 * (to - 1) >= O) to = (O + 31) / 32;
        if (W % tp) tp = 1;
    }
    if (tp == 3) tp = 2 - (W & 1);
    switch (to * 4 + tp) {
    case 1 * 4 + 1: launch<1, 1>(x, img, bias, y, g, dt, st); break;
    case 1 * 4 + 2: launch<1, 2>(x, img, bias, y, g, dt, st); break;
    case 2 * 4 + 1: launch<2, 1>(x, img, bias, y, g, dt, st); break;
    case 2 * 4 + 2: launch<2, 2>(x, img, bias, y, g, dt, st); break;
    case 3 * 4 + 1: launch<3, 1>(x, img, bias, y, g, dt, st); break;
    default: launch<3, 2>(x, img, bias, y, g, dt, st); break;
    }
    return (int)hipGetLastError();
}
}

extern "C" int mlagg_conv3x3_supported(int O, int I, int H, int W)
{
    return O > 0 && I > 0 && (I % 16) == 0 && H > 0 && W > 0 && (long)H * W >= 96 && (long)H * W <= (1LL << 32) / 36 - 1 &&
           (long)I * H * W * 4 < (1L << 31) - 64;
}

extern "C" size_t mlagg_conv3x3_workspace_bytes(int O, int I) { return O > 0 && I > 0 ? (size_t)3 * 9 * O * I * 2 : 0; }

extern "C" int mlagg_conv3x3_fwd(const float *x, long x_batch, const float *w, int transposed, const float *bias, float *y,
                                 long y_batch, void *workspace, int B, int O, int I, int H, int W, void *stream)
{
    return conv_fwd(x, x_batch, w, transposed, bias, y, y_batch, workspace, B, O, I, 1, H, W, MLAGG_DTYPE_BF16X3, stream);
}

extern "C" int mlagg_conv3x3_fwd_lp(const float *x, long x_batch, const float *w, int transposed, const float *bias, float *y,
                                    long y_batch, void *workspace, int B, int O, int I, int H, int W, int dtype, void *stream)
{
    return conv_fwd(x, x_batch, w, transposed, bias, y, y_batch, workspace, B, O, I, 1, H, W, dtype, stream);
}

extern "C" int mlagg_conv3x3x3_supported(int O, int I, int D, int H, int W)
{
    return O > 0 && I > 0 && (I % 16) == 0 && D > 0 && H > 0 && W > 0 && (long)D * H * W >= 96 && (long)D * H * W <= (1LL << 32) / 36 - 1 &&
           (long)I * D * H * W * 4 < (1L << 31) - 64;
}

extern "C" size_t mlagg_conv3x3x3_workspace_bytes(int O, int I) { return O > 0 && I > 0 ? (size_t)3 * 27 * O * I * 2 : 0; }

extern "C" int mlagg_conv3x3x3_fwd(const float *x, long x_batch, const float *w, int transposed, const float *bias, float *y,
                                   long y_batch, void *workspace, int B, int O, int I, int D, int H, int W, void *stream)
{
    if (D <= 1) return MLAGG_E_UNSUPPORTED;
    return conv_fwd(x, x_batch, w, transposed, bias, y, y_batch, workspace, B, O, I, D, H, W, MLAGG_DTYPE_BF16X3, stream);
}

extern "C" int mlagg_conv3x3_wgrad_supported(int O, int I, int H, int W)
{
    return O > 0 && I > 0 && H > 0 && W >= 8 && (W % 8) == 0 && ((long)H * W) % 16 == 0;
}

extern "C" int mlagg_conv3x3x3_wgrad_supported(int O, int I, int D, int H, int W)
{
    return O > 0 && I > 0 && D > 1 && H > 0 && W >= 8 && (W % 8) == 0 && ((long)D * H * W) % 16 == 0;
}

namespace {
size_t wgrad_ws(int B, int O, int I, int D, int H, int W)
{
    int to = 0, ti = 0;
    if (D == 1 && w16_tiles(O, I, MLAGG_DTYPE_BF16X3, to, ti)) {
        W16Geom g16;
        if (make_w16geom(g16, B, O, I, H, W, (long)O * H * W, (long)I * H * W, to, ti)) return 0;
        return (size_t)g16.nbs * 9 * O * I;
    }
    W3Geom g;
    if (make_w3geom(g, B, O, I, D, H, W, (long)O * D * H * W, (long)I * D * H * W)) return 0;
    return (size_t)B * g.nslabs * 9 * g.nz * O * I;
}

int wgrad3(const float *dy, long dy_batch, const float *x, long x_batch, float *dW, float *workspace, int B, int O, int I, int D, int H,
           int W, int dt, void *stream)
{
    if (!dy || !x || !dW || !workspace) return MLAGG_E_NULLPTR;
    if (!opmode::valid(dt)) return MLAGG_E_UNSUPPORTED;
    if ((reinterpret_cast<uintptr_t>(dy) & 15) || (reinterpret_cast<uintptr_t>(x) & 3)) return MLAGG_E_UNSUPPORTED;
    hipStream_t st = static_cast<hipStream_t>(stream);
    int to = 0, ti = 0;
    const int w16 = D == 1 ? w16_tiles(O, I, dt, to, ti) : 0;
    const bool lds_ok = !(reinterpret_cast<uintptr_t>(x) & 15) && (long)max(O, I) * H * W < (1L << 30);
    if (w16) {
        W16Geom g;
        if (int rc = make_w16geom(g, B, O, I, H, W, dy_batch, x_batch, to, ti)) return rc;
        MLAGG_TIMED(K_CONV3X3, st);
        const dim3 grid(24 * ((g.nbs + 7) / 8), (O + 16 * to - 1) / (16 * to), (I + 16 * ti - 1) / (16 * ti));
        const long dy_last = (long)(B - 1) * dy_batch + (long)O * H * W - 4;
        const bool lds = w16 == 2 && lds_ok;
#define K19W16_LAUNCH(TI_, DT_)                                                                                                       \
    if (lds) hipLaunchKernelGGL((conv3x3_wgrad16_lds_kernel<3, TI_, DT_>), grid, dim3(64), 0, st, dy, x, workspace, g, dy_last);        \
    else hipLaunchKernelGGL((conv3x3_wgrad16_kernel<3, TI_, DT_>), grid, dim3(64), 0, st, dy, x, workspace, g)
        if (ti == 1) {
            if (dt == MLAGG_DTYPE_BF16) { K19W16_LAUNCH(1, MLAGG_DTYPE_BF16); }
            else if (dt == MLAGG_DTYPE_F16) { K19W16_LAUNCH(1, MLAGG_DTYPE_F16); }
            else { K19W16_LAUNCH(1, MLAGG_DTYPE_BF16X3); }
        } else {
            if (dt == MLAGG_DTYPE_BF16) { K19W16_LAUNCH(3, MLAGG_DTYPE_BF16); }
            else if (dt == MLAGG_DTYPE_F16) { K19W16_LAUNCH(3, MLAGG_DTYPE_F16); }
            else { K19W16_LAUNCH(3, MLAGG_DTYPE_BF16X3); }
        }
#undef K19W16_LAUNCH
        const int n = 9 * O * I;
        hipLaunchKernelGGL(conv3x3_wgrad_reduce_kernel, dim3((n + 63) / 64), dim3(1024), 0, st, workspace, g.nbs, O, I, 9, dW);
        return (int)hipGetLastError();
    }
    W3Geom g;
    if (int rc = make_w3geom(g, B, O, I, D, H, W, dy_batch, x_batch)) return rc;
    MLAGG_TIMED(K_CONV3X3, st);
    const dim3 grid(B * g.nslabs * g.nz, (O + 31) / 32, (I + 31) / 32);
    if (dt == MLAGG_DTYPE_BF16)
        hipLaunchKernelGGL(conv3x3_wgrad_kernel<MLAGG_DTYPE_BF16>, grid, dim3(64), 0, st, dy, x, workspace, g);
    else if (dt == MLAGG_DTYPE_F16)
        hipLaunchKernelGGL(conv3x3_wgrad_kernel<MLAGG_DTYPE_F16>, grid, dim3(64), 0, st, dy, x, workspace, g);
    else
        hipLaunchKernelGGL(conv3x3_wgrad_kernel<MLAGG_DTYPE_BF16X3>, grid, dim3(64), 0, st, dy, x, workspace, g);
    const int ntaps = 9 * g.nz, n = ntaps * O * I;
    hipLaunchKernelGGL(conv3x3_wgrad_reduce_kernel, dim3((n + 63) / 64), dim3(1024), 0, st, workspace, B * g.nslabs, O, I, ntaps, dW);
    return (int)hipGetLastError();
}
}

extern "C" size_t mlagg_conv3x3_wgrad_workspace_floats(int B, int O, int I, int H, int W) { return wgrad_ws(B, O, I, 1, H, W); }
extern "C" size_t mlagg_conv3x3x3_wgrad_workspace_floats(int B, int O, int I, int D, int H, int W) { return D > 1 ? wgrad_ws(B, O, I, D, H, W) : 0; }

extern "C" int mlagg_conv3x3_wgrad(const float *dy, long dy_batch, const float *x, long x_batch, float *dW, float *workspace, int B,
                                   int O, int I, int H, int W, void *stream)
{
    return wgrad3(dy, dy_batch, x, x_batch, dW, workspace, B, O, I, 1, H, W, MLAGG_DTYPE_BF16X3, stream);
}

extern "C" int mlagg_conv3x3_wgrad_lp(const float *dy, long dy_batch, const float *x, long x_batch, float *dW, float *workspace, int B,
                                      int O, int I, int H, int W, int dtype, void *stream)
{
    return wgrad3(dy, dy_batch, x, x_batch, dW, workspace, B, O, I, 1, H, W, dtype, stream);
}

extern "C" int mlagg_conv3x3x3_wgrad(const float *dy, long dy_batch, const float *x, long x_batch, float *dW, float *workspace, int B,
                                     int O, int I, int D, int H, int W, void *stream)
{
    if (D <= 1) return MLAGG_E_UNSUPPORTED;
    return wgrad3(dy, dy_batch, x, x_batch, dW, workspace, B, O, I, D, H, W, MLAGG_DTYPE_BF16X3, stream);
}
```

mlagg-unet_amd/model.py:

```python
import math
from typing import Sequence

import torch
import torch.nn as nn
import torch.nn.functional as F

from . import ops

LAMBDA_INIT = 0.8


class _DropPathPool:

    active = None

    def __init__(self):
        self.order, self.keep, self.masks, self.pos, self.recording = [], None, None, 0, False
        self.injected, self.forced = None, False

    def inject(self, factors):
        self.injected = factors

    def begin(self, batch, device):
        if self.injected is not None:
            self.masks = self.injected.to(device=device, dtype=torch.float32).contiguous()
            if self.masks.dim() != 2 or self.masks.shape[1] != batch:
                raise RuntimeError("injected DropPath factors must be (n_calls, batch)")
            self.injected, self.forced, self.pos = None, True, 0
        elif not self.order:
            self.recording = True
        else:
            if self.keep is None or self.keep.device != device or self.keep.shape[1] != batch:
                self.keep = torch.tensor(self.order, device=device, dtype=torch.float32)[:, None].expand(-1, batch).contiguous()
            self.masks = torch.bernoulli(self.keep).div_(self.keep)
            self.pos = 0
        _DropPathPool.active = self

    def end(self):
        forced, self.forced = self.forced, False
        self.recording = False
        _DropPathPool.active = None
        if forced and self.pos != self.masks.shape[0]:
            raise RuntimeError(f"{self.masks.shape[0]} DropPath factors were injected, the forward made {self.pos} calls")

    def next(self, keep, batch):
        if self.forced:
            if self.pos >= self.masks.shape[0]:
                raise RuntimeError("more DropPath calls than injected factors")
            self.pos += 1
            return self.masks[self.pos - 1]
        if self.recording:
            self.order.append(keep)
            return None
        if self.pos >= len(self.order) or self.order[self.pos] != keep or self.masks.shape[1] != batch:
            raise RuntimeError("DropPath call order changed between forward passes")
        self.pos += 1
        return self.masks[self.pos - 1]


class DropPath(nn.Module):

    def __init__(self, p: float = 0.0):
        super().__init__()
        self.drop_prob = float(p)

    def scale_mask(self, x):
        if self.drop_prob == 0.0 or not self.training:
            return None
        keep = 1.0 - self.drop_prob
        pool = _DropPathPool.active
        if pool is not None:
            row = pool.next(keep, x.shape[0])
            if row is not None:
                return row
        return torch.empty(x.shape[0], device=x.device, dtype=x.dtype).bernoulli_(keep).div_(keep)

    def forward(self, x):
        m = self.scale_mask(x)
        return x if m is None else x * m.view((-1,) + (1,) * (x.dim() - 1))

    def residual_norm(self, skip, branch, norm):
        if branch.is_cuda:
            return ops.residual_layer_norm(skip, branch, self.scale_mask(branch), norm.weight, norm.bias, norm.eps)
        x = self.residual(skip, branch)
        return x, norm(x)

    def residual(self, skip, branch):
        m = self.scale_mask(branch)
        if m is None:
            return skip + branch
        if branch.is_cuda and (branch.numel() // branch.shape[0]) % 4 == 0:
            return ops.scaled_residual(skip, branch, m)
        return torch.addcmul(skip, branch, m.view((-1,) + (1,) * (branch.dim() - 1)))


_NO_DROP = DropPath(0.0)


class _ConvMixin:

    def _lib_conv(self, x, w):
        raise NotImplementedError

    def _native(self, x, form):
        return ops.conv2d(x, self.weight, self.stride, self.padding, self.dilation, self.groups, self.transposed, self.output_padding,
                          form)

    def raw(self, x):
        y = self._native(x, ops.conv_form())
        if y is None:
            cdt = ops.conv_dtype()
            y = self._lib_conv(ops.lp(x, cdt), ops.lp(self.weight, cdt))
        return y

    def fused(self, x, res=None, act=ops.EPI_NONE, dtype=None):
        if not x.is_cuda or getattr(self, "padding_mode", "zeros") != "zeros":
            y = self._eager(x)
            y = y if res is None else y + res
            return F.gelu(y) if act == ops.EPI_GELU else y
        y = self.raw(x)
        if y.dtype == torch.float32:
            return ops.channel_epilogue(y, self.bias, res if res is None or res.dtype == torch.float32 else res.float(), act)
        if y.numel() // (y.shape[0] * y.shape[1]) % 4:
            return ops.channel_epilogue(y.float(), self.bias, None if res is None else res.float(), act)
        return ops.channel_epilogue_lp(y, self.bias, res, act, dtype or torch.float32)

    def _device_forward(self, x):
        y = self.raw(x)
        if y.dtype == torch.float32:
            return y if self.bias is None else ops.channel_bias(y, self.bias)
        if y.numel() // (y.shape[0] * y.shape[1]) % 4:
            y = y.float()
            return y if self.bias is None else ops.channel_bias(y, self.bias)
        return ops.channel_epilogue_lp(y, self.bias, None, ops.EPI_NONE, torch.float32)


class Conv2d(_ConvMixin, nn.Conv2d):

    def _lib_conv(self, x, w):
        return F.conv2d(x, w, None, self.stride, self.padding, self.dilation, self.groups)

    def _eager(self, x):
        return nn.Conv2d.forward(self, x)

    def forward(self, x):
        if not x.is_cuda or self.padding_mode != "zeros":
            return nn.Conv2d.forward(self, x)
        return self._device_forward(x)


class ConvTranspose2d(_ConvMixin, nn.ConvTranspose2d):
    def _lib_conv(self, x, w):
        return F.conv_transpose2d(x, w, None, self.stride, self.padding, self.output_padding, self.groups, self.dilation)

    def _eager(self, x):
        return nn.ConvTranspose2d.forward(self, x)

    def forward(self, x, output_size=None):
        if not x.is_cuda or output_size is not None:
            return nn.ConvTranspose2d.forward(self, x, output_size)
        return self._device_forward(x)


class GroupNorm(nn.GroupNorm):

    def forward(self, x, out_dtype=None):
        if self.num_groups == self.num_channels and x.is_cuda and x.dim() == 4:
            return ops.plane_norm(x, self.weight, self.bias, self.eps, out_dtype=out_dtype)
        return super().forward(x)


def _chain_dtype(x):
    cdt = ops.conv_dtype()
    pixels = x.numel() // (x.shape[0] * x.shape[1])
    if cdt == torch.float32 or pixels % 4:
        return None
    if pixels >= ops.LP_K_MIN_PIXELS:
        return None
    return cdt


def _instance_norm_act(norm, x, act=ops.ACT_NONE, slope=0.0, res=None, out_dtype=None):
    if x.is_cuda and not norm.track_running_stats:
        return ops.plane_norm(x, norm.weight, norm.bias, norm.eps, act, slope, res, out_dtype or torch.float32)
    y = norm(x) if res is None else norm(x) + res
    return F.leaky_relu(y, slope) if act == ops.ACT_LEAKY else (F.silu(y) if act == ops.ACT_SILU else y)


class Linear(nn.Linear):

    def forward(self, x):
        return ops.linear(x, self.weight, self.bias)


class LayerNorm(nn.LayerNorm):

    def forward(self, x):
        return ops.layer_norm(x, self.weight, self.bias, self.eps)


class Mlp(nn.Module):
    def __init__(self, dim, hidden):
        super().__init__()
        self.fc1 = Linear(dim, hidden)
        self.fc2 = Linear(hidden, dim)

    def forward(self, x):
        return ops.mlp(x, self.fc1.weight, self.fc1.bias, self.fc2.weight, self.fc2.bias)


class RMSNormWeight(nn.Module):

    def __init__(self, dim):
        super().__init__()
        self.weight = nn.Parameter(torch.ones(dim))


class _StackFn(torch.autograd.Function):

    @staticmethod
    def forward(ctx, buf, ranges, *params):
        ctx.ranges, ctx.shapes = ranges, [tuple(p.shape) for p in params]
        return buf.detach()

    @staticmethod
    def backward(ctx, g):
        out, off = [None, None], 0
        for (lo, hi), shape in zip(ctx.ranges, ctx.shapes):
            piece = g[off:off + hi - lo]
            if lo == 0 and hi == shape[0]:
                out.append(piece)
            else:
                full = torch.zeros(shape, device=g.device, dtype=g.dtype)
                full[lo:hi] = piece
                out.append(full)
            off += hi - lo
        return tuple(out)


def _capturing(t):
    return t.is_cuda and torch.cuda.is_current_stream_capturing()


class _Stack:

    def __init__(self, sources):
        self.sources, self.buf, self.sig = sources, None, None

    @staticmethod
    def _norm(srcs):
        return [(t[0], int(t[1]), int(t[2])) if isinstance(t, tuple) else (t, 0, int(t.shape[0])) for t in srcs]

    def _views(self, srcs):
        rows = sum(hi - lo for _, lo, hi in srcs)
        shape = (rows,) + tuple(srcs[0][0].shape[1:])
        dev, dt = srcs[0][0].device, srcs[0][0].dtype
        if self.buf is None or self.buf.device != dev or tuple(self.buf.shape) != shape:
            self.buf = torch.empty(shape, device=dev, dtype=dt)
            self.sig = None
        out, off = [], 0
        for _, lo, hi in srcs:
            out.append(self.buf[off:off + hi - lo])
            off += hi - lo
        return out

    @staticmethod
    def _rows(srcs):
        return [t.detach()[lo:hi] for t, lo, hi in srcs]

    @staticmethod
    def signature(srcs):
        return (ops.image_epoch(),) + tuple(t._version for t, _, _ in srcs) + tuple(t.data_ptr() for t, _, _ in srcs)

    def stale(self, srcs):
        return self.sig != self.signature(srcs) or _capturing(srcs[0][0])

    def get(self):
        srcs = self._norm(self.sources())
        views = self._views(srcs)
        if self.stale(srcs):
            with torch.no_grad():
                torch._foreach_copy_(views, self._rows(srcs))
            self.sig = self.signature(srcs)
        out = _StackFn.apply(self.buf, [(lo, hi) for _, lo, hi in srcs], *[t for t, _, _ in srcs])
        out._mlagg_buffer = self.buf
        return out


def refresh_stacks(stacks):
    dst, src, done = [], [], []
    for st in stacks:
        srcs = st._norm(st.sources())
        views = st._views(srcs)
        if st.stale(srcs):
            dst += views
            src += st._rows(srcs)
            done.append((st, srcs))
    if dst:
        with torch.no_grad():
            torch._foreach_copy_(dst, src)
    for st, srcs in done:
        st.sig = st.signature(srcs)


class AggregatedAttention(nn.Module):

    def __init__(self, dim, input_resolution, num_heads, local, sr_ratio, variant="B"):
        super().__init__()
        self.dim, self.num_heads, self.local, self.variant = dim, num_heads, local, variant
        self.head_dim = dim // num_heads // 2
        if self.head_dim != 24:
            raise RuntimeError("the gfx950 attention kernels are built for head_dim 24 (every MLAgg-UNet stage)")
        self.scale = self.head_dim ** -0.5
        for nm in ("lambda_q1", "lambda_k1", "lambda_q2", "lambda_k2"):
            setattr(self, nm, nn.Parameter(torch.zeros(self.head_dim).normal_(0, 0.1)))
        self.subln = RMSNormWeight(2 * self.head_dim)
        self.H, self.W = input_resolution
        if not local:
            self.sr_ratio = sr_ratio
            self.pool_H, self.pool_W = self.H // sr_ratio, self.W // sr_ratio
            self.sr = Conv2d(dim, dim, 1)
            self.norm = LayerNorm(dim)
        self.q = Linear(dim, dim)
        self.kv = Linear(dim, 2 * dim)
        self.lepe = Conv2d(dim, dim, 3, padding=1, groups=dim)
        self._w_stack, self._b_stack = _Stack(self._stacked_weights), _Stack(self._stacked_biases)

    def _stacked_weights(self):
        if self.local:
            return [self.q.weight, self.kv.weight]
        d = self.q.weight.shape[0]
        return [self.q.weight, (self.kv.weight, d, 2 * d), self.sr.weight.view(d, d)]

    def _stacked_biases(self):
        if self.local:
            return [self.q.bias, self.kv.bias]
        d = self.q.bias.shape[0]
        return [self.q.bias, (self.kv.bias, d, 2 * d), self.sr.bias]

    def lambda_full(self):
        return ops.diff_lambda(self.lambda_q1, self.lambda_k1, self.lambda_q2, self.lambda_k2, LAMBDA_INIT)

    def forward(self, x):
        B, N, d = x.shape
        lam = self.lambda_full()
        if self.local:
            qkv = ops.linear(x, self._w_stack.get(), self._b_stack.get())
            q, kv = ops.split_cols(qkv, (d, 2 * d))
            return ops.local_diff_attn(q, kv, lam, self.subln.weight, self.lepe.weight, self.lepe.bias,
                                       self.H, self.W, self.num_heads, self.scale)
        qvs = ops.linear(x, self._w_stack.get(), self._b_stack.get())
        q, v_full, s_pre = ops.split_cols(qvs, (d, d, d))
        if self.H % self.sr_ratio == 0 and self.W % self.sr_ratio == 0:
            r = self.sr_ratio
            if s_pre.is_cuda:
                pooled = ops.gelu_pool(s_pre, self.H, self.W, r)
            else:
                pooled = F.gelu(s_pre).view(B, self.pool_H, r, self.pool_W, r, d).mean(dim=(2, 4)).reshape(B, -1, d)
        else:
            img = F.gelu(s_pre).view(B, self.H, self.W, d).permute(0, 3, 1, 2)
            pooled = F.adaptive_avg_pool2d(img, (self.pool_H, self.pool_W)).flatten(2).transpose(1, 2)
        k_pool, v_pool = self.kv(self.norm(pooled)).split([d, d], dim=-1)
        scale = self.scale if self.variant == "B" else self.scale * self.scale
        o = ops.pooled_diff_attn(q, k_pool, v_pool, lam, self.subln.weight, self.num_heads, scale)
        return ops.dwconv3x3_nlc(v_full, self.lepe.weight, self.lepe.bias, self.H, self.W, silu=False, res=o)


class MLLABlock(nn.Module):

    def __init__(self, dim, input_resolution, num_heads, mlp_ratio, drop_path, sr_ratio, variant="B"):
        super().__init__()
        self.dim, self.input_resolution = dim, tuple(input_resolution)
        self.norm1 = LayerNorm(dim)
        self.in_proj = Linear(dim, dim)
        self.act_proj = Linear(dim, dim)
        self.dwc = Conv2d(dim, dim, 3, padding=1, groups=dim)
        self.attn = nn.ModuleList([
            AggregatedAttention(dim // 2, input_resolution, num_heads // 2, True, sr_ratio, variant),
            AggregatedAttention(dim // 2, input_resolution, num_heads // 2, False, sr_ratio, variant)])
        self.out_proj = Linear(dim, dim)
        self.drop_path = DropPath(drop_path) if drop_path > 0.0 else nn.Identity()
        self.norm2 = LayerNorm(dim)
        self.mlp = Mlp(dim, int(dim * mlp_ratio))
        self._w_stack, self._b_stack = _Stack(self._stacked_weights), _Stack(self._stacked_biases)

    def _stacked_weights(self):
        return [self.act_proj.weight, self.in_proj.weight]

    def _stacked_biases(self):
        return [self.act_proj.bias, self.in_proj.bias]

    def forward_tokens(self, x, xn=None, next_norm=None):
        H, W = self.input_resolution
        C = self.dim
        if xn is None:
            xn = self.norm1(x)
        ai = ops.linear(xn, self._w_stack.get(), self._b_stack.get())
        h = C // 2
        act_pre, xz_in = ops.split_cols(ai, (C, C))
        xz = ops.dwconv3x3_nlc(xz_in, self.dwc.weight, self.dwc.bias, H, W, silu=True)
        xa, za = ops.split_cols(xz, (h, h))
        gated = ops.gate(self.attn[0](xa), self.attn[1](za), act_pre)
        dp = self.drop_path if isinstance(self.drop_path, DropPath) else _NO_DROP
        x, n2 = dp.residual_norm(x, self.out_proj(gated), self.norm2)
        y = self.mlp(n2)
        if next_norm is not None:
            return dp.residual_norm(x, y, next_norm)
        return dp.residual(x, y)

    def forward(self, x):
        B, C, h, w = x.shape
        if (h, w) != self.input_resolution:
            raise RuntimeError("input feature has wrong size")
        return _TokensToMap.apply(self.forward_tokens(_MapToTokens.apply(x)), h, w)


def _flip(t3):
    if t3.is_cuda:
        return ops.transpose_2d(t3)
    return t3.transpose(1, 2).contiguous()


class _ZeroGradParam(torch.autograd.Function):

    @staticmethod
    def forward(ctx, y, p):
        ctx.save_for_backward(p)
        return y.view_as(y)

    @staticmethod
# ... 422 lines not shown
```

mlagg-unet_amd/ops.py:

```python
import ctypes

import numpy as np
import torch

from . import _lib

_launch = _lib.launch
_stream = _lib.stream
_C = _lib.CONSTANTS


PRECISIONS = {"fp32": torch.float32, "bf16": torch.bfloat16, "fp16": torch.float16}
_LP_CODE = {torch.bfloat16: _C["MLAGG_DTYPE_BF16"], torch.float16: _C["MLAGG_DTYPE_F16"]}
import threading as _threading


class _ComputeStack(_threading.local):

    def __init__(self):
        self.stack = [torch.float32]


_COMPUTE = _ComputeStack()

# ... 1501 lines not shown
        ctx.save_for_backward(scale)
        return out

    @staticmethod
    def backward(ctx, g):
        (scale,) = ctx.saved_tensors
        g = _require(g.contiguous(), "grad")
        B = scale.numel()
        db = torch.empty_like(g)
        _launch("mlagg_scaled_residual", None, _ptr(g), _ptr(scale), _ptr(db), B, g.numel() // B)
        return g, db, None


def scaled_residual(skip, branch, scale):
    return ScaledResidualFn.apply(skip, branch, scale)


class DiceCEStatsFn(torch.autograd.Function):

    @staticmethod
    def forward(ctx, n, ignore_label, *tensors):
        logits, targets = tensors[:n], tensors[n:]
        ctx.ignore = int(ignore_label)
        B, C = logits[0].shape[:2]
        dev = logits[0].device
        lib = _lib.lib()
        if C > lib.mlagg_dice_ce_max_classes():
            raise RuntimeError(f"dice_ce_stats: at most {lib.mlagg_dice_ce_max_classes()} classes")
        buf = torch.empty(n * B * 3 * C + n, device=dev, dtype=torch.float32)
        ip = buf[:n * B * 2 * C].view(n, B, 2, C)
        gt = buf[n * B * 2 * C:n * B * 3 * C].view(n, B, C)
        ce = buf[n * B * 3 * C:]
        saved = []
        for i, (z, t) in enumerate(zip(logits, targets)):
            z = _require(z.contiguous(), "logits")
            t = _require(t.contiguous(), "target")
            if z.shape[:2] != (B, C) or t.numel() * C != z.numel():
                raise RuntimeError("dice_ce_stats: logits / target shapes of a level do not match")
            hw = z.numel() // (B * C)
            ws = torch.empty(lib.mlagg_dice_ce_stats_workspace_floats(B, C, hw), device=dev, dtype=torch.float32)
            _launch("mlagg_dice_ce_stats", _ptr(z), _ptr(t), _ptr(ip[i]), _ptr(gt[i]), ce.data_ptr() + 4 * i, _ptr(ws), B, C, hw,
                    ctx.ignore)
            saved += [z, t]
        ctx.save_for_backward(*saved)
        ctx.n = n
        ctx.mark_non_differentiable(gt)
        return ip, gt, ce

    @staticmethod
    def backward(ctx, g_ip, g_gt, g_ce):
        n = ctx.n
        saved = ctx.saved_tensors
        B, C = saved[0].shape[:2]
        g_ip = torch.zeros(n, B, 2, C, device=saved[0].device) if g_ip is None else _require(g_ip.contiguous(), "g_ip")
        g_ce = torch.zeros(n, device=saved[0].device) if g_ce is None else _require(g_ce.contiguous(), "g_ce")
        grads = []
        for i in range(n):
            z, t = saved[2 * i], saved[2 * i + 1]
            dz = torch.empty_like(z)
            _launch("mlagg_dice_ce_grad", _ptr(z), _ptr(t), _ptr(g_ip[i]), g_ce.data_ptr() + 4 * i, _ptr(dz), B, C, z.numel() // (B * C),
                    ctx.ignore)
            grads.append(dz)
        return (None, None, *grads, *([None] * n))


def dice_ce_stats(logits, targets, ignore_label=None):
    return DiceCEStatsFn.apply(len(logits), -1 if ignore_label is None else int(ignore_label), *logits, *targets)


def transpose_2d(src):
    _require(src, "src")
    B, R, C = src.shape
    if not (src.stride(2) == 1 and src.stride(1) == C and src.stride(0) >= R * C and src.data_ptr() % 16 == 0
            and (C % 4 or src.stride(0) % 4 == 0)):
        src = src.contiguous()
    dst = torch.empty(B, C, R, device=src.device, dtype=torch.float32)
    _launch("mlagg_transpose_2d", _ptr(src), src.stride(0), _ptr(dst), B, R, C)
    return dst


class ChannelBiasFn(torch.autograd.Function):

    @staticmethod
    def forward(ctx, x, bias):
        ctx.mark_dirty(x)
        x.add_(bias.view(1, -1, *([1] * (x.dim() - 2))))
        return x

    @staticmethod
    def backward(ctx, g):
        g = _require(g.contiguous(), "grad")
        B, C = g.shape[:2]
        db = torch.empty(C, device=g.device, dtype=torch.float32)
        ws = torch.empty(_lib.lib().mlagg_channel_sum_workspace_floats(B, C), device=g.device, dtype=torch.float32)
        _launch("mlagg_channel_sum", _ptr(g), _ptr(db), _ptr(ws), B, C, g.numel() // (B * C))
        return g, db


def channel_bias(x, bias):
    return ChannelBiasFn.apply(x, bias)


EPI_NONE, EPI_GELU = 0, 1


class ChannelEpilogueFn(torch.autograd.Function):

    @staticmethod
    def forward(ctx, x, bias, res, act):
        x = _require(x, "x")
        if not x.is_contiguous():
            raise RuntimeError("channel_epilogue: contiguous NCHW map expected")
        res = None if res is None else _require(res.contiguous(), "res", x.shape)
        B, C = x.shape[:2]
        hw = x.numel() // (B * C)
        if act == EPI_GELU and x._version != 0:
            raise RuntimeError("channel_epilogue(GELU): x must be the fresh output of the producing call")
        y = torch.empty_like(x) if act == EPI_GELU else None
        _launch("mlagg_channel_epilogue_fwd", _ptr(x), _ptr(bias), _ptr(res), _ptr(y), B, C, hw, int(act))
        ctx.meta = (int(act), bias is not None, res is not None)
        if act == EPI_GELU:
            ctx.save_for_backward(x)
            return y
        ctx.mark_dirty(x)
        return x

    @staticmethod
    def backward(ctx, dy):
        act, has_bias, has_res = ctx.meta
        dy = _require(dy.contiguous(), "dy")
        B, C = dy.shape[:2]
        hw = dy.numel() // (B * C)
        db = torch.empty(C, device=dy.device, dtype=torch.float32) if has_bias else None
        ws = torch.empty(_lib.lib().mlagg_channel_sum_workspace_floats(B, C), device=dy.device, dtype=torch.float32) if has_bias else None
        if act == EPI_GELU:
            (pre,) = ctx.saved_tensors
            dx = torch.empty_like(dy)
            _launch("mlagg_channel_gelu_bwd", _ptr(pre), _ptr(dy), _ptr(dx), _ptr(db), _ptr(ws), B, C, hw)
        else:
            dx = dy
            if has_bias:
                _launch("mlagg_channel_sum", _ptr(dy), _ptr(db), _ptr(ws), B, C, hw)
        return dx, db, (dx if has_res else None), None


def channel_epilogue(x, bias=None, res=None, act=EPI_NONE):
    return ChannelEpilogueFn.apply(x, bias, res, act)


def column_sum(x2):
    _require(x2, "x")
    rows, cols = x2.shape
    out = torch.empty(cols, device=x2.device, dtype=torch.float32)
    n = _lib.lib().mlagg_column_sum_workspace_floats(rows, cols)
    ws = torch.empty(n, device=x2.device, dtype=torch.float32) if n else None
    _launch("mlagg_column_sum", _ptr(x2), x2.stride(0), _ptr(out), _ptr(ws), rows, cols)
    return out


ACT_NONE, ACT_LEAKY, ACT_SILU = 0, 1, 2


_DT_CODE = {torch.float32: _C["MLAGG_DTYPE_F32"], **_LP_CODE}


def _require_map(t, name, shape=None):
    if not (isinstance(t, torch.Tensor) and t.is_cuda and t.dtype in _DT_CODE):
        raise RuntimeError(f"{name}: expected an fp32 / bf16 / fp16 tensor on the MI355X device, got "
                           f"{getattr(t, 'dtype', type(t))} on {getattr(t, 'device', '?')}")
    if shape is not None and tuple(t.shape) != tuple(shape):
        raise RuntimeError(f"{name}: expected shape {tuple(shape)}, got {tuple(t.shape)}")
    return t


def _map_slice(t, name):
    if t.is_cuda and t.dim() >= 3 and not t.is_contiguous():
        inner, want = 1, []
        for v in reversed(t.shape[1:]):
            want.append(inner)
            inner *= int(v)
        want.reverse()
        plane = inner // int(t.shape[1])
        if tuple(t.stride()[1:]) == tuple(want) and t.stride(0) >= inner and t.stride(0) % plane == 0 and t.stride(0) % 4 == 0 and \
                t.data_ptr() % 16 == 0 and t.dtype in _DT_CODE:
            return t, t.stride(0)
    t = _require_map(t.contiguous(), name)
    return t, 0


class PlaneNormFn(torch.autograd.Function):

    @staticmethod
    def forward(ctx, x, gamma, beta, res, eps, act, slope, out_dtype):
        x = _require_map(x.contiguous(), "x")
        res = None if res is None else _require_map(res.contiguous(), "res", x.shape)
        B, C = x.shape[:2]
        hw = x.numel() // (B * C)
        y = torch.empty(x.shape, device=x.device, dtype=out_dtype or x.dtype)
        stats = torch.empty(B * C, 2, device=x.device, dtype=torch.float32)
        nws = _lib.lib().mlagg_plane_norm_fwd_workspace_floats(B, C, hw)
        ws = torch.empty(nws, device=x.device, dtype=torch.float32) if nws else None
        _launch("mlagg_plane_norm_fwd", _ptr(x), _ptr(gamma), _ptr(beta), _ptr(res), _ptr(y), _ptr(stats), _ptr(ws), B, C, hw, float(eps),
                int(act), float(slope), _DT_CODE[x.dtype], 0 if res is None else _DT_CODE[res.dtype], _DT_CODE[y.dtype])
        ctx.save_for_backward(x, gamma, beta, res, stats)
        ctx.meta = (int(act), float(slope))
        return y

    @staticmethod
    def backward(ctx, dy):
        x, gamma, beta, res, stats = ctx.saved_tensors
        act, slope = ctx.meta
        dy, dyb = _map_slice(dy, "dy")
        B, C = x.shape[:2]
        hw = x.numel() // (B * C)
        lib = _lib.lib()
        dx = torch.empty_like(x)
        dres = torch.empty_like(res) if (res is not None and ctx.needs_input_grad[3]) else None
        dg = torch.empty_like(gamma) if gamma is not None else None
        db = torch.empty_like(beta) if beta is not None else None
        segmented = lib.mlagg_plane_norm_fwd_workspace_floats(B, C, hw) > 0
        ws = torch.empty(lib.mlagg_plane_norm_bwd_workspace_floats(B, C, hw), device=x.device, dtype=torch.float32) \
            if (dg is not None or db is not None or segmented) else None
        _launch("mlagg_plane_norm_bwd_strided", _ptr(x), _ptr(dy), dyb, _ptr(gamma), _ptr(beta), _ptr(res), _ptr(stats), _ptr(dx),
                _ptr(dres), _ptr(dg), _ptr(db), _ptr(ws), B, C, hw, act, slope, _DT_CODE[x.dtype], _DT_CODE[dy.dtype],
                0 if res is None else _DT_CODE[res.dtype])
        return dx, dg, db, dres, None, None, None, None


def plane_norm(x, gamma, beta, eps=1e-5, act=ACT_NONE, slope=0.0, res=None, out_dtype=None):
    return PlaneNormFn.apply(x, gamma, beta, res, eps, act, slope, out_dtype)


class ChannelEpilogueLpFn(torch.autograd.Function):

    @staticmethod
    def forward(ctx, x, bias, res, act, out_dtype):
        x = _require_map(x.contiguous(), "x")
        res = None if res is None else _require_map(res.contiguous(), "res", x.shape)
        B, C = x.shape[:2]
        hw = x.numel() // (B * C)
        y = torch.empty(x.shape, device=x.device, dtype=out_dtype)
        _launch("mlagg_channel_epilogue_lp_fwd", _ptr(x), _DT_CODE[x.dtype], _ptr(bias), _ptr(res),
                0 if res is None else _DT_CODE[res.dtype], _ptr(y), _DT_CODE[y.dtype], B, C, hw, int(act))
        ctx.save_for_backward(x if act == EPI_GELU else None, bias, res if act == EPI_GELU else None)
        ctx.meta = (int(act), x.dtype, None if res is None else res.dtype, tuple(x.shape))
        return y

    @staticmethod
    def backward(ctx, dy):
        x, bias, res = ctx.saved_tensors
        act, xdt, rdt, shape = ctx.meta
        dy = _require_map(dy.contiguous(), "dy", shape)
        B, C = shape[:2]
        hw = dy.numel() // (B * C)
        dx = torch.empty(shape, device=dy.device, dtype=xdt)
        db = torch.empty(C, device=dy.device, dtype=torch.float32) if bias is not None else None
        ws = (torch.empty(_lib.lib().mlagg_channel_sum_workspace_floats(B, C), device=dy.device, dtype=torch.float32)
              if bias is not None else None)
        _launch("mlagg_channel_epilogue_lp_bwd", _ptr(x), _DT_CODE[xdt], _ptr(bias), _ptr(res), 0 if res is None else _DT_CODE[res.dtype],
                _ptr(dy), _DT_CODE[dy.dtype], _ptr(dx), _DT_CODE[xdt], _ptr(db), _ptr(ws), B, C, hw, act)
        dres = None
        if rdt is not None and ctx.needs_input_grad[2]:
            src = dy if act == EPI_NONE else dx
            dres = src if src.dtype == rdt else (dx if dx.dtype == rdt else src.to(rdt))
        return dx, db, dres, None, None


def channel_epilogue_lp(x, bias=None, res=None, act=EPI_NONE, out_dtype=torch.float32):
    return ChannelEpilogueLpFn.apply(x, bias, res, act, out_dtype)


def _planes(t, name):
    _require(t, name)
    inner, want = 1, []
    for v in reversed(t.shape[1:]):
        want.append(inner)
        inner *= int(v)
    want.reverse()
    if tuple(t.stride()[1:]) != tuple(want) or t.stride(0) < inner or t.stride(0) % 4 or t.data_ptr() % 16:
        t = t.contiguous()
    return t, t.stride(0), inner // int(t.shape[1])


K18 = _os.environ.get("MLAGG_K18", "1") == "1"
K18_FWD_MIN_PIXELS = int(_os.environ.get("MLAGG_K18_FWD_MIN_PIXELS", "4096"))
K18_FWD_MIN_K = int(_os.environ.get("MLAGG_K18_FWD_MIN_K", "96"))
K18_WGRAD_MIN_PIXELS = int(_os.environ.get("MLAGG_K18_WGRAD_MIN_PIXELS", "4096"))


K18_THIN_CH = 32


def _k18_product(O, I, P, form=_DTYPE_BF16X3):
    I16 = -(-I // 16) * 16
    if not bool(_lib.lib().mlagg_conv1x1_supported(O, I16, P)):
        return False
    if form != _DTYPE_BF16X3:
        return P >= LP_K_MIN_PIXELS
    if P >= K18_FWD_MIN_PIXELS and min(O, I) <= K18_THIN_CH:
        return True
    return I == I16 and P >= K18_FWD_MIN_PIXELS and I >= K18_FWD_MIN_K


def _conv1x1_k18(x, xb, w, y, B, O, I, P, form, accumulate=False):
    if y is None:
        y = torch.empty((B, O) + tuple(x.shape[2:]), device=x.device, dtype=torch.float32)
    I16 = -(-I // 16) * 16
    if I16 != I:
        wp = torch.zeros(O, I16, device=w.device, dtype=torch.float32)
        wp[:, :I] = w
        w = wp
    _flop("K18", 2 * B * O * I * P)
    _launch("mlagg_conv1x1_fwd_acc", _ptr(x), xb, _ptr(w), None, _ptr(y), O * P, B, O, I16, I, P, form, int(accumulate))
    return y


def _conv1x1_wgrad(dy, dyb, x, B, O, I, P, form):
    dW = torch.empty(O, I, device=x.device, dtype=torch.float32)
    ws = torch.empty(_lib.lib().mlagg_conv1x1_wgrad_workspace_floats(B, O, I, P), device=x.device, dtype=torch.float32)
    _flop("K18", 2 * B * O * I * P)
    _launch("mlagg_conv1x1_wgrad_lp", _ptr(dy), dyb, _ptr(x), x.stride(0), _ptr(dW), _ptr(ws), B, O, I, P, form)
    return dW


class Conv1x1Fn(torch.autograd.Function):

    @staticmethod
    def forward(ctx, x, weight, form=_DTYPE_BF16X3, plan=None):
        x, xb, P = _planes(x, "x")
        B, I = x.shape[:2]
        O = weight.shape[0]
        plan = plan or _conv1x1_plan(O, I, P, form)
        w = _require(weight.reshape(O, I).contiguous(), "weight")
        y = _conv1x1_k18(x, xb, w, None, B, O, I, P, form) if plan[0] else _lib_conv(x, weight, 1, 0, False, form)
        ctx.save_for_backward(x, w)
        ctx.wshape, ctx.plan, ctx.form = weight.shape, plan, form
        return y

    @staticmethod
    def backward(ctx, dy):
        x, w = ctx.saved_tensors
        B, I = x.shape[:2]
        O = w.shape[0]
        dy, dyb, P = _planes(dy, "dy")
        form = ctx.form
        dx = dW = None
        if ctx.needs_input_grad[0]:
            if ctx.plan[1]:
                wt = transpose_2d(w.unsqueeze(0))[0]
                dx = _conv1x1_k18(dy, dyb, wt, None, B, I, O, P, form)
            else:
                dx = _lib_conv_bwd(dy, x, w.view(ctx.wshape), 1, 0, False, (True, False, False), form)[0]
        if ctx.needs_input_grad[1]:
            dW = _conv1x1_wgrad(dy, dyb, x, B, O, I, P, form).view(ctx.wshape)
        return dx, dW, None, None


def _conv1x1_plan(O, I, P, form):
    return ("K18" if _k18_product(O, I, P, form) else None, "K18" if _k18_product(I, O, P, form) else None, "K18")


def _pixel_shuffle2(src, B, O, H, W, inverse):
    src = _require(src.contiguous(), "src")
    dst = torch.empty((B, 4 * O, H, W) if inverse else (B, O, 2 * H, 2 * W), device=src.device, dtype=torch.float32)
    _launch("mlagg_pixel_shuffle2", _ptr(src), _ptr(dst), B, O, H, W, int(inverse))
    return dst


class ConvT2x2Fn(torch.autograd.Function):

    @staticmethod
    def forward(ctx, x, weight, form=_DTYPE_BF16X3):
        x, xb, P = _planes(x, "x")
        B, I, H, W = x.shape
        O = weight.shape[1]
        w4 = _require(weight.permute(2, 3, 1, 0).reshape(4 * O, I).contiguous(), "weight")
        z = _conv1x1_k18(x, xb, w4, None, B, 4 * O, I, P, form)
        ctx.save_for_backward(x, w4)
        ctx.form, ctx.O = form, O
        return _pixel_shuffle2(z, B, O, H, W, False)

    @staticmethod
    def backward(ctx, dy):
        x, w4 = ctx.saved_tensors
        B, I, H, W = x.shape
        O, form, P = ctx.O, ctx.form, H * W
        dy, dyb = _map_slice(dy, "dy")
        if dy.dtype != torch.float32:
            dy, dyb = dy.float(), 0
        dyu = torch.empty(B, 4 * O, H, W, device=x.device, dtype=torch.float32)
        _launch("mlagg_pixel_unshuffle2_strided", _ptr(dy), dyb, _ptr(dyu), B, O, H, W)
        dx = dW = None
        if ctx.needs_input_grad[0]:
            wt = transpose_2d(w4.unsqueeze(0))[0]
            dx = _conv1x1_k18(dyu, 4 * O * P, wt, None, B, I, 4 * O, P, form)
        if ctx.needs_input_grad[1]:
            dW = _conv1x1_wgrad(dyu, 4 * O * P, x, B, 4 * O, I, P, form).view(2, 2, O, I).permute(3, 2, 0, 1).contiguous()
        return dx, dW, None


K19 = _os.environ.get("MLAGG_K19", "1") == "1"
K19_MIN_PIXELS = int(_os.environ.get("MLAGG_K19_MIN_PIXELS", "1024"))


K19_WGRAD = _os.environ.get("MLAGG_K19_WGRAD", "1") == "1"
K19_WGRAD_MIN_PIXELS = int(_os.environ.get("MLAGG_K19_WGRAD_MIN_PIXELS", "1024"))
K19_WGRAD_MIN_CH = int(_os.environ.get("MLAGG_K19_WGRAD_MIN_CH", "48"))


def _k19_wgrad(O, I, H, W, form=_DTYPE_BF16X3):
    if form != _DTYPE_BF16X3:
        return K19_WGRAD and H * W >= LP_K_MIN_PIXELS and bool(_lib.lib().mlagg_conv3x3_wgrad_supported(O, I, H, W))
    return (K19_WGRAD and H * W >= K19_WGRAD_MIN_PIXELS and max(O, I) >= K19_WGRAD_MIN_CH and
            bool(_lib.lib().mlagg_conv3x3_wgrad_supported(O, I, H, W)))


def _k19_product(O, I, H, W, form=_DTYPE_BF16X3):
    floor = K19_MIN_PIXELS if form == _DTYPE_BF16X3 else LP_K_MIN_PIXELS
    return K19 and H * W >= floor and bool(_lib.lib().mlagg_conv3x3_supported(O, I, H, W))


def _conv3x3_plan(O, I, H, W, form):
    return tuple("K19" if on else None for on in (_k19_product(O, I, H, W, form), _k19_product(I, O, H, W, form), _k19_wgrad(O, I, H, W, form)))


def _conv3x3_k19(x, xb, w, transposed, O, I, H, W, form, out=None):
    B = x.shape[0]
    y = torch.empty(B, O, H, W, device=x.device, dtype=torch.float32) if out is None else out
    ws = torch.empty(_lib.lib().mlagg_conv3x3_workspace_bytes(O, I), device=x.device, dtype=torch.uint8)
    _flop("K19", 2 * 9 * B * O * I * H * W)
    _launch("mlagg_conv3x3_fwd_lp", _ptr(x), xb, _ptr(w), int(transposed), None, _ptr(y), y.stride(0), _ptr(ws), B, O, I, H, W, form)
    return y


class Conv3x3Fn(torch.autograd.Function):

    @staticmethod
    def forward(ctx, x, weight, form=_DTYPE_BF16X3, slot=None, plan=None):
        ctx.slot = slot
        x, xb, P = _planes(x, "x")
        B, I, H, W = x.shape
        O = weight.shape[0]
        plan = plan or _conv3x3_plan(O, I, H, W, form)
        w = _require(weight.contiguous(), "weight")
        y = _conv3x3_k19(x, xb, w, False, O, I, H, W, form) if plan[0] else _lib_conv(x, w, 1, 1, False, form)
        ctx.save_for_backward(x, w)
        ctx.plan, ctx.form = plan, form
        return y

    @staticmethod
    def backward(ctx, dy):
        x, w = ctx.saved_tensors
        B, I, H, W = x.shape
        O = w.shape[0]
        (_, dgrad, wgrad), form = ctx.plan, ctx.form
        dx = dW = None
        if ctx.needs_input_grad[0]:
            if dgrad:
                dy, dyb, _ = _planes(dy, "dy")
                out = ctx.slot.view() if ctx.slot is not None else None
                dx = _conv3x3_k19(dy, dyb, w, True, I, O, H, W, form, out)
            else:
                dx = _lib_conv_bwd(dy, x, w, 1, 1, False, (True, False, False), form)[0]
        if ctx.needs_input_grad[1]:
            if wgrad:
                lib = _lib.lib()
                dy, dyb, _ = _planes(dy, "dy")
                dW = torch.empty(O, I, 3, 3, device=x.device, dtype=torch.float32)
                ws = torch.empty(lib.mlagg_conv3x3_wgrad_workspace_floats(B, O, I, H, W), device=x.device, dtype=torch.float32)
                _flop("K19", 2 * 9 * B * O * I * H * W)
                _launch("mlagg_conv3x3_wgrad_lp", _ptr(dy), dyb, _ptr(x), x.stride(0), _ptr(dW), _ptr(ws), B, O, I, H, W, form)
            else:
                dW = _lib_conv_bwd(dy.contiguous(), x, w, 1, 1, False, (False, True, False), form)[1]
        return dx, dW, None, None, None


K19T = _os.environ.get("MLAGG_K19T", "1") == "1"
K19T_WGRAD = _os.environ.get("MLAGG_K19T_WGRAD", "0") == "1"


def _k19t_shape(O, I, H, W, form=_DTYPE_BF16X3):
    floor = K19_MIN_PIXELS if form == _DTYPE_BF16X3 else LP_K_MIN_PIXELS
    return K19T and H * W >= floor and bool(_lib.lib().mlagg_conv3x3_s2t_supported(O, I, H, W))


def _s2t_plan(O, I, H, W, form):
    on = _k19t_shape(O, I, H, W, form)
    return ("K19t" if on else None,) * 2 + ("K19t" if on and K19T_WGRAD else None,)


def _k19t_fwd(x, xb, w, O, I, H, W, form):
    B = x.shape[0]
    y = torch.empty(B, O, 2 * H - 1, 2 * W - 1, device=x.device, dtype=torch.float32)
    ws = torch.empty(_lib.lib().mlagg_conv3x3_s2t_workspace_bytes(O, I), device=x.device, dtype=torch.uint8)
    _flop("K19", 2 * 9 * B * O * I * H * W)
    _launch("mlagg_conv3x3_s2t_fwd", _ptr(x), xb, _ptr(w), _ptr(y), y.stride(0), _ptr(ws), B, O, I, H, W, form)
    return y


def _k19t_dgrad(dy, w, O, I, H, W, form):
    B = dy.shape[0]
    dx = torch.empty(B, I, H, W, device=dy.device, dtype=torch.float32)
    ws = torch.empty(_lib.lib().mlagg_conv3x3_s2t_workspace_bytes(O, I), device=dy.device, dtype=torch.uint8)
    _flop("K19", 2 * 9 * B * O * I * H * W)
    _launch("mlagg_conv3x3_s2_dgrad", _ptr(dy), dy.stride(0), dy.stride(1), dy.stride(2), _ptr(w), _ptr(dx), dx.stride(0), _ptr(ws), B, O,
            I, H, W, form)
    return dx


def _k19t_wgrad(x, xb, dy, O, I, H, W, form):
    B = x.shape[0]
    dW = torch.empty(I, O, 3, 3, device=x.device, dtype=torch.float32)
    ws = torch.empty(_lib.lib().mlagg_conv3x3_s2t_wgrad_workspace_floats(B, O, I, H, W), device=x.device, dtype=torch.float32)
    _flop("K19", 2 * 9 * B * O * I * H * W)
    _launch("mlagg_conv3x3_s2t_wgrad", _ptr(x), xb, _ptr(dy), dy.stride(0), dy.stride(1), dy.stride(2), _ptr(dW), _ptr(ws), B, O, I, H, W,
            form)
    return dW


class ConvT3x3S2Fn(torch.autograd.Function):

    @staticmethod
    def forward(ctx, x, weight, form=_DTYPE_BF16X3, plan=None):
        x, xb, _ = _planes(x, "x")
        B, I, H, W = x.shape
        O = int(weight.shape[1])
        plan = plan or _s2t_plan(O, I, H, W, form)
        w = _require(weight.contiguous(), "weight")
        y = _k19t_fwd(x, xb, w, O, I, H, W, form) if plan[0] else _lib_conv(x, w, 2, 1, True, form)
        ctx.save_for_backward(x, w)
        ctx.plan, ctx.form = plan, form
        return y

    @staticmethod
    def backward(ctx, dy):
        x, w = ctx.saved_tensors
        B, I, H, W = x.shape
        O = int(w.shape[1])
        (_, dgrad, wgrad), form = ctx.plan, ctx.form
        if dgrad and (dy.stride(3) != 1 or dy.data_ptr() % 4):
            dy = dy.contiguous()
        dx = dW = None
        if ctx.needs_input_grad[0]:
            dx = _k19t_dgrad(dy, w, O, I, H, W, form) if dgrad else _lib_conv_bwd(dy, x, w, 2, 1, True, (True, False, False), form)[0]
        if ctx.needs_input_grad[1]:
            dW = _k19t_wgrad(x, x.stride(0), dy, O, I, H, W, form) if wgrad else _lib_conv_bwd(dy, x, w, 2, 1, True, (False, True, False), form)[1]
        return dx, dW, None, None


def _fp32_map(x, nd):
    return x.is_cuda and x.dtype == torch.float32 and x.dim() == nd + 2


def _all(v, n):
    return all(int(a) == n for a in v)


def conv_plan(x, weight, stride, padding, dilation, groups, transposed, output_padding, form):
    if not (_fp32_map(x, 2) and groups == 1 and _all(dilation, 1) and _all(output_padding, 0)):
        return None
    geom = tuple(tuple(int(v) for v in t) for t in (weight.shape[2:], stride, padding)) + (bool(transposed),)
    I, O = (int(weight.shape[0]), int(weight.shape[1])) if transposed else (int(weight.shape[1]), int(weight.shape[0]))
    H, W = int(x.shape[2]), int(x.shape[3])
    P, one = H * W, form != _DTYPE_BF16X3
    if geom[:3] == ((1, 1), (1, 1), (0, 0)):
        if not (K18 and P >= (LP_K_MIN_PIXELS if one else K18_WGRAD_MIN_PIXELS) and P % 16 == 0):
            return None
        plan = _conv1x1_plan(O, I, P, form)
        return None if transposed and None in plan else plan
    if geom == ((2, 2), (2, 2), (0, 0), True):
        ok = K18 and W % 2 == 0 and P % 16 == 0 and _k18_product(4 * O, I, P, form) and _k18_product(I, 4 * O, P, form)
        return ("K18",) * 3 if ok else None
    if geom == ((3, 3), (1, 1), (1, 1), False):
        plan = _conv3x3_plan(O, I, H, W, form)
        return plan if K19 and (plan[0] or plan[1] or (one and plan[2])) else None
    if geom == ((3, 3), (2, 2), (1, 1), True):
        plan = _s2t_plan(O, I, H, W, form)
        return plan if plan[0] else None
    return None


def conv2d(x, weight, stride, padding, dilation, groups, transposed, output_padding, form):
    plan = conv_plan(x, weight, stride, padding, dilation, groups, transposed, output_padding, form)
    if plan is None:
        return None
    k = int(weight.shape[2])
    if k == 1:
        return Conv1x1Fn.apply(x, weight.permute(1, 0, 2, 3) if transposed else weight, form, plan)
    if k == 2:
        return ConvT2x2Fn.apply(x, weight, form)
    if transposed:
        return ConvT3x3S2Fn.apply(x, weight, form, plan)
    return Conv3x3Fn.apply(x, weight, form, claim_slot(x), plan)


def conv1x1_supported(x, weight, stride, padding, dilation, groups, form=_DTYPE_BF16X3):
    return tuple(weight.shape[2:]) == (1, 1) and conv_plan(x, weight, stride, padding, dilation, groups, False, (0, 0), form) is not None


def conv3x3_supported(x, weight, stride, padding, dilation, groups, form=_DTYPE_BF16X3):
    return tuple(weight.shape[2:]) == (3, 3) and conv_plan(x, weight, stride, padding, dilation, groups, False, (0, 0), form) is not None


def conv_t2x2_supported(x, weight, stride, padding, output_padding, dilation, groups, form=_DTYPE_BF16X3):
    return tuple(weight.shape[2:]) == (2, 2) and conv_plan(x, weight, stride, padding, dilation, groups, True, output_padding, form) is not None


def conv3x3_s2t_supported(x, weight, stride, padding, output_padding, dilation, groups, form=_DTYPE_BF16X3):
    return tuple(weight.shape[2:]) == (3, 3) and conv_plan(x, weight, stride, padding, dilation, groups, True, output_padding, form) is not None


def conv1x1(x, weight, form=_DTYPE_BF16X3):
    return Conv1x1Fn.apply(x, weight, form)


def conv3x3(x, weight, form=_DTYPE_BF16X3):
    return Conv3x3Fn.apply(x, weight, form, claim_slot(x))


def conv_t2x2(x, weight, form=_DTYPE_BF16X3):
    return ConvT2x2Fn.apply(x, weight, form)


def conv3x3_s2t(x, weight, form=_DTYPE_BF16X3):
    return ConvT3x3S2Fn.apply(x, weight, form)


K19_3D = _os.environ.get("MLAGG_K19_3D", "1") == "1"
K19_3D_WGRAD = _os.environ.get("MLAGG_K19_3D_WGRAD", "1") == "1"


def _conv3x3x3_k19(x, xb, w, transposed, O, I, dims):
    B = x.shape[0]
    D, H, W = dims
    y = torch.empty(B, O, D, H, W, device=x.device, dtype=torch.float32)
    ws = torch.empty(_lib.lib().mlagg_conv3x3x3_workspace_bytes(O, I), device=x.device, dtype=torch.uint8)
    _launch("mlagg_conv3x3x3_fwd", _ptr(x), xb, _ptr(w), int(transposed), None, _ptr(y), O * D * H * W, _ptr(ws), B, O, I, D, H, W)
    return y


def _pad_geometry(D, H, W, stride, wide=False):
    Dq, Hq, Wq, guard = ctypes.c_int(), ctypes.c_int(), ctypes.c_int(), ctypes.c_long()
    _lib.check(_lib.lib().mlagg_conv_pad_geometry(D, H, W, stride, int(wide), ctypes.byref(Dq), ctypes.byref(Hq), ctypes.byref(Wq),
                                                  ctypes.byref(guard)), "mlagg_conv_pad_geometry")
    return Dq.value, Hq.value, Wq.value, guard.value


K16 = _os.environ.get("MLAGG_K16", "1") == "1"


class _Padded:

    def __init__(self, t, dims, stride, wide, as_output_of=None):
        t = _require(t.contiguous(), "map")
        self.B, self.C = t.shape[:2]
        self.dims = tuple(dims)
        self.stride, self.wide = stride, wide
        self.Dq, self.Hq, self.Wq, self.guard = _pad_geometry(*self.dims, stride, wide)
        self.Q = self.Dq * self.Hq * self.Wq
        self.row = 2 * self.guard + self.Q
        self.nph = 1 if (stride == 1 or as_output_of is not None) else 8
        self.buf = torch.empty(self.B, self.nph, self.C, self.row, device=t.device, dtype=torch.float32)
        od = tuple(t.shape[2:]) if t.dim() == 5 else (1,) + tuple(t.shape[2:])
        if as_output_of is None:
            _launch("mlagg_volume_pad", _ptr(t), _ptr(self.buf), self.B, self.C, *self.dims, stride, int(wide), 0, 0, 0, 0)
        else:
            _launch("mlagg_volume_pad", _ptr(t), _ptr(self.buf), self.B, self.C, *self.dims, stride, int(wide), 1, *od)

    def ptr(self):
        return self.buf.data_ptr() + 4 * self.guard


def _tap_offsets(k, nd, stride, Hq, Wq, I=0, row=0):
    taps = []
    kz_range = range(k) if nd == 3 else (k // 2,)
    for kz in kz_range:
        for ky in range(k):
            for kx in range(k):
                if stride == 1:
                    dz = (kz - k // 2) if nd == 3 else 0
                    taps.append(dz * Hq * Wq + (ky - k // 2) * Wq + (kx - k // 2))
                else:
                    az, ay, ax = (kz, ky, kx) if k == 3 else (1, 1, 1)
                    ph = ((az & 1) << 2) | ((ay & 1) << 1) | (ax & 1)
                    taps.append(ph * I * row + (az >> 1) * Hq * Wq + (ay >> 1) * Wq + (ax >> 1))
    return taps


def _wgrad_from_padded(xp, dyp, k, nd):
    O, I, B = dyp.C, xp.C, xp.B
    taps = _tap_offsets(k, nd, xp.stride, xp.Hq, xp.Wq, I, xp.row)
    ntaps = len(taps)
    Q8 = (xp.Q + 7) & ~7
    off = (ctypes.c_long * ntaps)(*taps)
    dW = torch.empty(O, I, ntaps, device=xp.buf.device, dtype=torch.float32)
    ws = torch.empty(_lib.lib().mlagg_conv_wgrad_taps_workspace_floats(B, Q8, O, I, ntaps), device=xp.buf.device, dtype=torch.float32)
    _launch("mlagg_conv_wgrad_taps", dyp.ptr(), O * dyp.row, dyp.row, xp.ptr(), xp.nph * I * xp.row, xp.row, off, ntaps, Q8, O, I, B,
            _ptr(dW), 0, _ptr(ws))
    return dW


def conv_weight_grad(x, dy, k, stride):
    nd = x.dim() - 2
    dims = tuple(x.shape[2:]) if nd == 3 else (1,) + tuple(x.shape[2:])
    xp = _Padded(x, dims, stride, False)
    dyp = _Padded(dy, dims, stride, False, as_output_of=xp)
    return _wgrad_from_padded(xp, dyp, k, nd)


def _conv_taps(src, weight, O, I, k, flip, dims):
    ntaps = k ** 3
    taps = _tap_offsets(k, 3, 1, src.Hq, src.Wq)
    off = (ctypes.c_long * ntaps)(*taps)
    y = torch.empty(src.B, O, *dims, device=src.buf.device, dtype=torch.float32)
    w = _require(weight.contiguous(), "weight")
    if flip:
        w_so, w_si = ntaps, O * ntaps
    else:
        w_so, w_si = I * ntaps, ntaps
    _launch("mlagg_conv_taps", src.ptr(), src.C * src.row, src.row, _ptr(w), w_so, w_si, int(flip), off, ntaps, _ptr(y), src.B, O, I, *dims)
    return y


def conv_wgrad_supported(x, weight, stride, padding):
    nd, k = x.dim() - 2, int(weight.shape[2])
    return (nd in (2, 3) and _fp32_map(x, nd) and k in (1, 3) and _all(weight.shape[2:], k) and _all(padding, k // 2)
            and len(set(int(v) for v in stride)) == 1
            and (int(stride[0]) == 1 or (int(stride[0]) == 2 and nd == 3 and all(int(v) > 1 for v in x.shape[2:]))))


def conv_taps_supported(x, weight, stride, padding):
    return (K16 and x.dim() == 5 and conv_wgrad_supported(x, weight, stride, padding) and int(stride[0]) == 1 and x.shape[-1] % 4 == 0
            and x.shape[1] >= 8)


def conv3x3x3_supported(x, weight, stride, padding):
    return (K19_3D and _fp32_map(x, 3) and tuple(weight.shape[2:]) == (3, 3, 3) and _all(stride, 1) and _all(padding, 1)
            and bool(_lib.lib().mlagg_conv3x3x3_supported(int(weight.shape[0]), int(weight.shape[1]), *(int(v) for v in x.shape[2:]))))


def conv_nd_plan(x, weight, stride, padding):
    if conv3x3x3_supported(x, weight, stride, padding):
        O, I, dims, lib = int(weight.shape[0]), int(weight.shape[1]), tuple(int(v) for v in x.shape[2:]), _lib.lib()
        return ("K19", "K19" if lib.mlagg_conv3x3x3_supported(I, O, *dims) else None,
                "K19" if K19_3D_WGRAD and lib.mlagg_conv3x3x3_wgrad_supported(O, I, *dims) else "K15")
    if conv_taps_supported(x, weight, stride, padding):
        return "K16", "K16", "K15"
    return (None, None, "K15") if conv_wgrad_supported(x, weight, stride, padding) else None


class ConvNdFn(torch.autograd.Function):

    @staticmethod
    def forward(ctx, x, weight, stride, padding, plan):
        dims = tuple(int(v) for v in x.shape[2:])
        O, I = int(weight.shape[0]), int(weight.shape[1])
        ctx.xp = None
        if plan[0] == "K19":
            x, xb, _ = _planes(x, "x")
            weight = _require(weight.contiguous(), "weight")
            y = _conv3x3x3_k19(x, xb, weight, False, O, I, dims)
        elif plan[0] == "K16":
            ctx.xp = _Padded(x, dims, 1, True)
            y = _conv_taps(ctx.xp, weight, O, I, int(weight.shape[2]), False, dims)
            x = None
        else:
            y = _lib_conv(x, weight, stride, padding, False, _DTYPE_BF16X3)
        ctx.save_for_backward(x, weight)
        ctx.geom, ctx.plan = (stride, padding), plan
        return y

    @staticmethod
    def backward(ctx, dy):
        x, w = ctx.saved_tensors
        (stride, padding), (_, dgrad, wgrad), xp = ctx.geom, ctx.plan, ctx.xp
        O, I, k = int(w.shape[0]), int(w.shape[1]), int(w.shape[2])
        if xp is not None:
            dims, dyp = xp.dims, _Padded(dy, xp.dims, 1, True, as_output_of=xp)
        else:
            dims, dy = tuple(int(v) for v in x.shape[2:]), dy.contiguous()
        dx = dW = None
        if ctx.needs_input_grad[0]:
            if dgrad == "K19":
                dx = _conv3x3x3_k19(dy, O * dims[0] * dims[1] * dims[2], w, True, I, O, dims)
            elif dgrad == "K16":
                dx = _conv_taps(dyp, w, I, O, k, True, dims)
            else:
                dx = _lib_conv_bwd(dy, x, w, stride, padding, False, (True, False, False), _DTYPE_BF16X3)[0]
        if ctx.needs_input_grad[1]:
            if wgrad == "K19":
                B = x.shape[0]
                dW = torch.empty(O, I, 3, 3, 3, device=x.device, dtype=torch.float32)
                ws = torch.empty(_lib.lib().mlagg_conv3x3x3_wgrad_workspace_floats(B, O, I, *dims), device=x.device, dtype=torch.float32)
                _launch("mlagg_conv3x3x3_wgrad", _ptr(dy), O * dims[0] * dims[1] * dims[2], _ptr(x), x.stride(0), _ptr(dW), _ptr(ws), B, O,
                        I, *dims)
            elif xp is not None:
                dW = _wgrad_from_padded(xp, dyp, k, 3).view(w.shape)
            else:
                dW = conv_weight_grad(x, dy, k, stride).view(w.shape)
        ctx.xp = None
        return dx, dW, None, None, None


def conv_nd(x, weight, stride, padding):
    plan = conv_nd_plan(x, weight, stride, padding)
    if plan is not None:
        return ConvNdFn.apply(x, weight, int(stride[0]), int(padding[0]), plan)
    return (torch.nn.functional.conv3d if x.dim() == 5 else torch.nn.functional.conv2d)(x, weight, None, stride, padding)


def _expect(t, name, dtype=torch.float32, dim=None, shape=None, contiguous=True, like=None):
    if not (isinstance(t, torch.Tensor) and t.is_cuda and t.dtype == dtype and (like is None or t.device == like.device)
            and (dim is None or t.dim() == dim) and (shape is None or tuple(t.shape) == tuple(shape))
            and (not contiguous or t.is_contiguous())):
        want = (f"{'contiguous ' if contiguous else ''}{'' if dim is None else f'{dim}-D '}{dtype} tensor"
                f"{'' if shape is None else f' of shape {tuple(shape)}'} on {'the MI355X device' if like is None else like.device}")
        strided = isinstance(t, torch.Tensor) and not t.is_contiguous()
        raise RuntimeError(f"{name}: expected a {want}, got {getattr(t, 'dtype', type(t))} {tuple(getattr(t, 'shape', ()))}"
                           f"{' (non-contiguous)' if strided else ''} on {getattr(t, 'device', '?')}")


def _sw_flips(flips):
    flips = [int(m) for m in flips]
    if len(flips) not in (1, 2, 4, 8) or any(m < 0 or m > 7 for m in flips) or len(set(flips)) != len(flips):
        raise RuntimeError(f"mirror variants {flips}: 1, 2, 4 or 8 distinct masks in [0, 7]")
    return flips


def _sw_box(origin, tile, shape, what):
    o = tuple(int(v) for v in origin)
    if len(o) != 3 or any(v < 0 or v + t > s for v, t, s in zip(o, tile, shape)):
        raise RuntimeError(f"{what}: tile at {o} of size {tuple(tile)} is not inside the volume {tuple(shape)}")
    return o


def sliding_window_gather(volume, origins, flips, tile_size):
    _expect(volume, "volume", dim=4)
    flips = _sw_flips(flips)
    tile = tuple(int(t) for t in tile_size)
    if len(tile) != 3 or min(tile) < 1:
        raise RuntimeError(f"tile_size {tile_size}: three positive sides")
    C, X, Y, Z = volume.shape
    boxes = [_sw_box(o, tile, (X, Y, Z), "sliding_window_gather") for o in origins]
    if not boxes:
        raise RuntimeError("sliding_window_gather: no tiles")
    out = torch.empty((len(flips) * len(boxes), C) + tile, device=volume.device, dtype=torch.float32)
    _launch("mlagg_sw_gather", _ptr(volume), C, X, Y, Z, _int_array([v for o in boxes for v in o]), len(boxes), _int_array(flips),
            len(flips), _ptr(out), *tile)
    return out


def sliding_window_fold(out, tile, n, flips, gaussian, origin, acc, weight):
    _expect(out, "out", dim=5)
    _expect(acc, "acc", dim=4)
    _expect(weight, "weight", dim=3)
    flips = _sw_flips(flips)
    V, n, tile = len(flips), int(n), int(tile)
    K, tx, ty, tz = (int(v) for v in out.shape[1:])
    gaussian = _require(gaussian.contiguous(), "gaussian", (tx, ty, tz))
    if out.shape[0] != V * n or not 0 <= tile < n:
        raise RuntimeError(f"sliding_window_fold: out has {out.shape[0]} rows, expected {V} variants x {n} tiles; tile {tile}")
    if acc.shape[0] != K or acc.shape[1:] != weight.shape:
        raise RuntimeError(f"sliding_window_fold: acc {tuple(acc.shape)} / weight {tuple(weight.shape)} for {K} classes")
    X, Y, Z = weight.shape
    o = _sw_box(origin, (tx, ty, tz), (X, Y, Z), "sliding_window_fold")
    _launch("mlagg_sw_fold", _ptr(out), tile, n, _int_array(flips), V, K, _ptr(gaussian), tx, ty, tz, *o, _ptr(acc), _ptr(weight), X, Y, Z)


def sliding_window_finalize(acc, weight, region, return_labels=False):
    _expect(acc, "acc", dim=4)
    _expect(weight, "weight", dim=3)
    if acc.shape[1:] != weight.shape:
        raise RuntimeError(f"sliding_window_finalize: acc {tuple(acc.shape)} / weight {tuple(weight.shape)}")
    K = int(acc.shape[0])
    shape = tuple(int(s) for s in weight.shape)
    lo, size = [], []
    for sl, s in zip(region, shape):
        a, b = (0 if sl.start is None else int(sl.start)), (s if sl.stop is None else int(sl.stop))
        if sl.step not in (None, 1) or not 0 <= a < b <= s:
            raise RuntimeError(f"sliding_window_finalize: region {region} is not inside {shape}")
        lo.append(a)
        size.append(b - a)
    if len(lo) != 3:
        raise RuntimeError("sliding_window_finalize: region must hold three slices")
    logits = torch.empty((K,) + tuple(size), device=acc.device, dtype=torch.float32)
    labels = torch.empty(tuple(size), device=acc.device, dtype=torch.int64) if return_labels else None
    _launch("mlagg_sw_finalize", _ptr(acc), _ptr(weight), K, *shape, *lo, *size, _ptr(logits), _ptr(labels))
    return logits, labels


def _strided_volume(t, name):
    _expect(t, name, dim=4, contiguous=False)
    if min(t.shape) < 1 or min(t.stride()) < 0:
        raise RuntimeError(f"{name}: expected a non-empty (C, X, Y, Z) tensor with non-negative strides, got shape {tuple(t.shape)}, "
                           f"strides {t.stride()}")
    return tuple(int(s) for s in t.shape), tuple(int(s) for s in t.stride())
# ... 366 lines not shown
```

Measured before the change: 283.8 images/sec.

## Fuse bias, residual add and GELU into conv1x1/conv3x3 forward epilogues

Adds epilogue variants of the custom conv1x1 and conv3x3 forward kernels that add the bias and an optional residual and, optionally, write a GELU-activated copy in the same store pass. A new autograd function routes eligible convolutions through them and handles the bias, residual and GELU gradients in backward before reusing the existing conv backward paths. The aim is to remove the separate elementwise epilogue kernels and their extra full-tensor reads and writes. In exchange the kernels gain extra pointer arguments and register pressure, and the fused path keeps an extra pre-activation tensor when GELU is used.

```diff
diff --git a/include/mlagg_hip.h b/include/mlagg_hip.h
--- a/include/mlagg_hip.h
+++ b/include/mlagg_hip.h
@@ -151,6 +151,8 @@
                              int I_valid, long P, int dtype, void *stream);
 int mlagg_conv1x1_fwd_acc(const float *x, long x_batch, const float *w, const float *bias, float *y, long y_batch, int B, int O, int I,
                           int I_valid, long P, int dtype, int accumulate, void *stream);
+int mlagg_conv1x1_fwd_epi(const float *x, long x_batch, const float *w, const float *bias, const float *res, float *y, float *y_act,
+                          long y_batch, int B, int O, int I, int I_valid, long P, int dtype, int act, void *stream);
 
 int mlagg_conv3x3_supported(int O, int I, int H, int W);
 size_t mlagg_conv3x3_workspace_bytes(int O, int I);
@@ -170,6 +172,8 @@
                         int I, int H, int W, void *stream);
 int mlagg_conv3x3_fwd_lp(const float *x, long x_batch, const float *w, int transposed, const float *bias, float *y, long y_batch,
                          void *workspace, int B, int O, int I, int H, int W, int dtype, void *stream);
+int mlagg_conv3x3_fwd_epi(const float *x, long x_batch, const float *w, const float *bias, const float *res, float *y, float *y_act,
+                          long y_batch, void *workspace, int B, int O, int I, int H, int W, int dtype, int act, void *stream);
 int mlagg_conv3x3_wgrad_lp(const float *dy, long dy_batch, const float *x, long x_batch, float *dW, float *workspace, int B, int O,
                            int I, int H, int W, int dtype, void *stream);
 
diff --git a/mlagg-unet_amd/csrc/channel_epilogue.hip b/mlagg-unet_amd/csrc/channel_epilogue.hip
--- a/mlagg-unet_amd/csrc/channel_epilogue.hip
+++ b/mlagg-unet_amd/csrc/channel_epilogue.hip
@@ -1,6 +1,7 @@
 #include <hip/hip_runtime.h>
 #include <stdint.h>
 
+#include "gelu.h"
 #include "internal.h"
 #include "lpio.h"
 #include "mlagg_hip.h"
@@ -8,12 +9,8 @@
 
 namespace {
 
-__device__ __forceinline__ float gelu_f(float x) { return 0.5f * x * (1.f + erff(x * 0.70710678118654752f)); }
-__device__ __forceinline__ float gelu_grad_f(float x)
-{
-    const float cdf = 0.5f * (1.f + erff(x * 0.70710678118654752f));
-    return cdf + x * 0.3989422804014327f * __expf(-0.5f * x * x);
-}
+using mlagg_internal::gelu_f;
+using mlagg_internal::gelu_grad_f;
 
 template <bool GELU>
 __global__ void __launch_bounds__(256)
diff --git a/mlagg-unet_amd/csrc/conv1x1.hip b/mlagg-unet_amd/csrc/conv1x1.hip
--- a/mlagg-unet_amd/csrc/conv1x1.hip
+++ b/mlagg-unet_amd/csrc/conv1x1.hip
@@ -7,6 +7,7 @@
 #include "bf16x3.h"
 #include "opmode.h"
 #include "internal.h"
+#include "gelu.h"
 
 namespace {
 
@@ -28,8 +29,8 @@
 
 template <int TO, int TP, int DT>
 __global__ void __launch_bounds__(64)
-conv1x1_fwd_kernel(const float *__restrict__ X, const float *__restrict__ W, const float *__restrict__ bias, float *__restrict__ Y,
-                   C1Geom g)
+conv1x1_fwd_kernel(const float *__restrict__ X, const float *__restrict__ W, const float *__restrict__ bias,
+                   const float *__restrict__ Res, float *__restrict__ Y, float *__restrict__ Yact, C1Geom g)
 {
     const int lane = threadIdx.x, col = lane & 31, kh = lane >> 5;
     const int p0 = blockIdx.x * (32 * TP), o0 = blockIdx.y * (32 * TO), b = blockIdx.z;
@@ -83,7 +84,7 @@
         consume(wa[1], xv[1]);
     }
     if (blk < nblk) consume(wa[0], xv[0]);
-    float *yb = Y + (size_t)b * g.y_batch + pc;
+    const size_t yoff = (size_t)b * g.y_batch + pc;
 #pragma unroll
     for (int a = 0; a < TO; ++a) {
 #pragma unroll
@@ -91,21 +92,38 @@
             const int o = o0 + 32 * a + (r & 3) + 8 * (r >> 2) + 4 * kh;
             if (o >= g.O) continue;
             const float bv = bias ? bias[o] : 0.f;
-            float *dst = yb + (size_t)o * g.P;
+            const size_t off = yoff + (size_t)o * g.P;
+            float *dst = Y + off;
             if (pc == pnat) {
                 FVec<TP> v;
 #pragma unroll
                 for (int j = 0; j < TP; ++j) v.v[j] = acc[a][j][r] + bv;
+                if (Res) {
+                    const FVec<TP> rv = *reinterpret_cast<const FVec<TP> *>(Res + off);
+#pragma unroll
+                    for (int j = 0; j < TP; ++j) v.v[j] += rv.v[j];
+                }
                 if (g.accumulate) {
                     const FVec<TP> old = *reinterpret_cast<const FVec<TP> *>(dst);
 #pragma unroll
                     for (int j = 0; j < TP; ++j) v.v[j] += old.v[j];
                 }
                 *reinterpret_cast<FVec<TP> *>(dst) = v;
+                if (Yact) {
+#pragma unroll
+                    for (int j = 0; j < TP; ++j) v.v[j] = mlagg_internal::gelu_f(v.v[j]);
+                    *reinterpret_cast<FVec<TP> *>(Yact + off) = v;
+                }
             } else {
 #pragma unroll
                 for (int j = 0; j < TP; ++j)
-                    if (pc + j >= pnat) dst[j] = acc[a][j][r] + bv + (g.accumulate ? dst[j] : 0.f);
+                    if (pc + j >= pnat) {
+                        float v = acc[a][j][r] + bv;
+                        if (Res) v += Res[off + j];
+                        if (g.accumulate) v += dst[j];
+                        dst[j] = v;
+                        if (Yact) Yact[off + j] = mlagg_internal::gelu_f(v);
+                    }
             }
         }
     }
@@ -223,15 +241,16 @@
 }
 
 template <int TO, int TP>
-void launch_fwd(const float *x, const float *w, const float *bias, float *y, const C1Geom &g, int dt, hipStream_t st)
+void launch_fwd(const float *x, const float *w, const float *bias, const float *res, float *y, float *yact, const C1Geom &g, int dt,
+                hipStream_t st)
 {
     const dim3 grid((g.P + 32 * TP - 1) / (32 * TP), (g.O + 32 * TO - 1) / (32 * TO), g.B);
     if (dt == MLAGG_DTYPE_BF16)
-        hipLaunchKernelGGL((conv1x1_fwd_kernel<TO, TP, MLAGG_DTYPE_BF16>), grid, dim3(64), 0, st, x, w, bias, y, g);
+        hipLaunchKernelGGL((conv1x1_fwd_kernel<TO, TP, MLAGG_DTYPE_BF16>), grid, dim3(64), 0, st, x, w, bias, res, y, yact, g);
     else if (dt == MLAGG_DTYPE_F16)
-        hipLaunchKernelGGL((conv1x1_fwd_kernel<TO, TP, MLAGG_DTYPE_F16>), grid, dim3(64), 0, st, x, w, bias, y, g);
+        hipLaunchKernelGGL((conv1x1_fwd_kernel<TO, TP, MLAGG_DTYPE_F16>), grid, dim3(64), 0, st, x, w, bias, res, y, yact, g);
     else
-        hipLaunchKernelGGL((conv1x1_fwd_kernel<TO, TP, MLAGG_DTYPE_BF16X3>), grid, dim3(64), 0, st, x, w, bias, y, g);
+        hipLaunchKernelGGL((conv1x1_fwd_kernel<TO, TP, MLAGG_DTYPE_BF16X3>), grid, dim3(64), 0, st, x, w, bias, res, y, yact, g);
 }
 
 template <int TO, int TI>
@@ -259,10 +278,12 @@
     return mlagg_conv1x1_fwd_acc(x, x_batch, w, bias, y, y_batch, B, O, I, I_valid, P, dtype, 0, stream);
 }
 
-extern "C" int mlagg_conv1x1_fwd_acc(const float *x, long x_batch, const float *w, const float *bias, float *y, long y_batch, int B,
-                                     int O, int I, int I_valid, long P, int dtype, int accumulate, void *stream)
+namespace {
+int conv1x1_fwd(const float *x, long x_batch, const float *w, const float *bias, const float *res, float *y, float *yact, long y_batch,
+                int B, int O, int I, int I_valid, long P, int dtype, int accumulate, void *stream)
 {
     if (!x || !w || !y) return MLAGG_E_NULLPTR;
+    if (accumulate && (res || yact)) return MLAGG_E_UNSUPPORTED;
     if (!opmode::valid(dtype) || I_valid <= 0 || I_valid > I) return MLAGG_E_UNSUPPORTED;
     if (B <= 0 || B > 65535 || !mlagg_conv1x1_supported(O, I, P)) return MLAGG_E_UNSUPPORTED;
     if (x_batch < (long)I_valid * P || y_batch < (long)O * P || (reinterpret_cast<uintptr_t>(w) & 15)) return MLAGG_E_UNSUPPORTED;
@@ -272,17 +293,33 @@
     int to = O <= 32 ? 1 : (O <= 64 ? 2 : 3), tp = O <= 64 ? 3 : 2;
     pick_fwd_tile(B, O, I, (int)P, to, tp);
     switch (to * 4 + tp) {
-    case 1 * 4 + 1: launch_fwd<1, 1>(x, w, bias, y, g, dtype, st); break;
-    case 1 * 4 + 2: launch_fwd<1, 2>(x, w, bias, y, g, dtype, st); break;
-    case 1 * 4 + 3: launch_fwd<1, 3>(x, w, bias, y, g, dtype, st); break;
-    case 2 * 4 + 1: launch_fwd<2, 1>(x, w, bias, y, g, dtype, st); break;
-    case 2 * 4 + 2: launch_fwd<2, 2>(x, w, bias, y, g, dtype, st); break;
-    case 2 * 4 + 3: launch_fwd<2, 3>(x, w, bias, y, g, dtype, st); break;
-    case 3 * 4 + 1: launch_fwd<3, 1>(x, w, bias, y, g, dtype, st); break;
-    case 3 * 4 + 2: launch_fwd<3, 2>(x, w, bias, y, g, dtype, st); break;
-    default: launch_fwd<3, 3>(x, w, bias, y, g, dtype, st); break;
+    case 1 * 4 + 1: launch_fwd<1, 1>(x, w, bias, res, y, yact, g, dtype, st); break;
+    case 1 * 4 + 2: launch_fwd<1, 2>(x, w, bias, res, y, yact, g, dtype, st); break;
+    case 1 * 4 + 3: launch_fwd<1, 3>(x, w, bias, res, y, yact, g, dtype, st); break;
+    case 2 * 4 + 1: launch_fwd<2, 1>(x, w, bias, res, y, yact, g, dtype, st); break;
+    case 2 * 4 + 2: launch_fwd<2, 2>(x, w, bias, res, y, yact, g, dtype, st); break;
+    case 2 * 4 + 3: launch_fwd<2, 3>(x, w, bias, res, y, yact, g, dtype, st); break;
+    case 3 * 4 + 1: launch_fwd<3, 1>(x, w, bias, res, y, yact, g, dtype, st); break;
+    case 3 * 4 + 2: launch_fwd<3, 2>(x, w, bias, res, y, yact, g, dtype, st); break;
+    default: launch_fwd<3, 3>(x, w, bias, res, y, yact, g, dtype, st); break;
     }
     return (int)hipGetLastError();
+}
+}
+
+extern "C" int mlagg_conv1x1_fwd_acc(const float *x, long x_batch, const float *w, const float *bias, float *y, long y_batch, int B,
+                                     int O, int I, int I_valid, long P, int dtype, int accumulate, void *stream)
+{
+    return conv1x1_fwd(x, x_batch, w, bias, nullptr, y, nullptr, y_batch, B, O, I, I_valid, P, dtype, accumulate, stream);
+}
+
+extern "C" int mlagg_conv1x1_fwd_epi(const float *x, long x_batch, const float *w, const float *bias, const float *res, float *y,
+                                     float *y_act, long y_batch, int B, int O, int I, int I_valid, long P, int dtype, int act,
+                                     void *stream)
+{
+    if (act != 0 && act != 1) return MLAGG_E_UNSUPPORTED;
+    if (act == 1 && !y_act) return MLAGG_E_NULLPTR;
+    return conv1x1_fwd(x, x_batch, w, bias, res, y, act ? y_act : nullptr, y_batch, B, O, I, I_valid, P, dtype, 0, stream);
 }
 
 extern "C" int mlagg_conv1x1_fwd_lp(const float *x, long x_batch, const float *w, const float *bias, float *y, long y_batch, int B,
diff --git a/mlagg-unet_amd/csrc/conv3x3.hip b/mlagg-unet_amd/csrc/conv3x3.hip
--- a/mlagg-unet_amd/csrc/conv3x3.hip
+++ b/mlagg-unet_amd/csrc/conv3x3.hip
@@ -6,6 +6,7 @@
 #include "prof.h"
 #include "bf16x3.h"
 #include "opmode.h"
+#include "gelu.h"
 
 namespace {
 
@@ -48,7 +49,7 @@
 template <int TO, int TP, int NR, int DT>
 __global__ void __launch_bounds__(64 * WAVES, (K19_OCC3 && NR == 3 && TO <= 2 && TO * TP <= 4) ? 3 : 2)
 conv3x3_kernel(const float *__restrict__ X, const unsigned short *__restrict__ Wimg, const float *__restrict__ bias,
-               float *__restrict__ Y, C3Geom g)
+               const float *__restrict__ Res, float *__restrict__ Y, float *__restrict__ Yact, C3Geom g)
 {
     constexpr int ROWS = 32 * TO;
     constexpr int NQ = opmode::Form<DT>::NQ, NT = opmode::Form<DT>::NT;
@@ -182,7 +183,9 @@
 #pragma unroll
         for (int r = 0; r < NR; ++r) stage(blk, r, r & 1);
     }
-    float *yb = Y + (size_t)b * g.y_batch + pc;
+    const float *res = NR == 3 ? Res : nullptr;
+    float *yact = NR == 3 ? Yact : nullptr;
+    const size_t yoff = (size_t)b * g.y_batch + pc;
 #pragma unroll
     for (int a = 0; a < TO; ++a) {
 #pragma unroll
@@ -190,16 +193,32 @@
             const int o = o0 + 32 * a + (r & 3) + 8 * (r >> 2) + 4 * kh;
             if (o >= g.O) continue;
             const float bv = bias ? bias[o] : 0.f;
-            float *dst = yb + (size_t)o * g.P;
+            const size_t off = yoff + (size_t)o * g.P;
+            float *dst = Y + off;
             if (pc == pnat) {
                 FVec<TP> v;
 #pragma unroll
                 for (int j = 0; j < TP; ++j) v.v[j] = acc[a][j][r] + bv;
+                if (res) {
+                    const FVec<TP> rv = *reinterpret_cast<const FVec<TP> *>(res + off);
+#pragma unroll
+                    for (int j = 0; j < TP; ++j) v.v[j] += rv.v[j];
+                }
                 *reinterpret_cast<FVec<TP> *>(dst) = v;
+                if (yact) {
+#pragma unroll
+                    for (int j = 0; j < TP; ++j) v.v[j] = mlagg_internal::gelu_f(v.v[j]);
+                    *reinterpret_cast<FVec<TP> *>(yact + off) = v;
+                }
             } else {
 #pragma unroll
                 for (int j = 0; j < TP; ++j)
-                    if (pc + j >= pnat && pnat < g.P) dst[j] = acc[a][j][r] + bv;
+                    if (pc + j >= pnat && pnat < g.P) {
+                        float v = acc[a][j][r] + bv;
+                        if (res) v += res[off + j];
+                        dst[j] = v;
+                        if (yact) yact[off + j] = mlagg_internal::gelu_f(v);
+                    }
             }
         }
     }
@@ -675,18 +694,19 @@
 
 
 template <int TO, int TP>
-void launch(const float *x, const unsigned short *wimg, const float *bias, float *y, const C3Geom &g, int dt, hipStream_t st)
+void launch(const float *x, const unsigned short *wimg, const float *bias, const float *res, float *y, float *yact, const C3Geom &g, int dt,
+            hipStream_t st)
 {
     const int groups = (g.P + 32 * TP - 1) / (32 * TP);
     const dim3 grid((groups + WAVES - 1) / WAVES, (g.O + 32 * TO - 1) / (32 * TO), g.B);
     if (g.D > 1)
-        hipLaunchKernelGGL((conv3x3_kernel<TO, TP, 9, MLAGG_DTYPE_BF16X3>), grid, dim3(64 * WAVES), 0, st, x, wimg, bias, y, g);
+        hipLaunchKernelGGL((conv3x3_kernel<TO, TP, 9, MLAGG_DTYPE_BF16X3>), grid, dim3(64 * WAVES), 0, st, x, wimg, bias, res, y, yact, g);
     else if (dt == MLAGG_DTYPE_BF16)
-        hipLaunchKernelGGL((conv3x3_kernel<TO, TP, 3, MLAGG_DTYPE_BF16>), grid, dim3(64 * WAVES), 0, st, x, wimg, bias, y, g);
+        hipLaunchKernelGGL((conv3x3_kernel<TO, TP, 3, MLAGG_DTYPE_BF16>), grid, dim3(64 * WAVES), 0, st, x, wimg, bias, res, y, yact, g);
     else if (dt == MLAGG_DTYPE_F16)
-        hipLaunchKernelGGL((conv3x3_kernel<TO, TP, 3, MLAGG_DTYPE_F16>), grid, dim3(64 * WAVES), 0, st, x, wimg, bias, y, g);
+        hipLaunchKernelGGL((conv3x3_kernel<TO, TP, 3, MLAGG_DTYPE_F16>), grid, dim3(64 * WAVES), 0, st, x, wimg, bias, res, y, yact, g);
     else
-        hipLaunchKernelGGL((conv3x3_kernel<TO, TP, 3, MLAGG_DTYPE_BF16X3>), grid, dim3(64 * WAVES), 0, st, x, wimg, bias, y, g);
+        hipLaunchKernelGGL((conv3x3_kernel<TO, TP, 3, MLAGG_DTYPE_BF16X3>), grid, dim3(64 * WAVES), 0, st, x, wimg, bias, res, y, yact, g);
 }
 
 }
@@ -694,11 +714,12 @@
 namespace {
 constexpr long K19_MAX_PLANE = (1LL << 32) / 36 - 1;
 
-int conv_fwd(const float *x, long x_batch, const float *w, int transposed, const float *bias, float *y, long y_batch, void *workspace,
-             int B, int O, int I, int D, int H, int W, int dt, void *stream)
+int conv_fwd(const float *x, long x_batch, const float *w, int transposed, const float *bias, const float *res, float *y, float *yact,
+             long y_batch, void *workspace, int B, int O, int I, int D, int H, int W, int dt, void *stream)
 {
     if (!x || !w || !y || !workspace) return MLAGG_E_NULLPTR;
     if (!opmode::valid(dt) || (D > 1 && dt != MLAGG_DTYPE_BF16X3)) return MLAGG_E_UNSUPPORTED;
+    if (D > 1 && (res || yact)) return MLAGG_E_UNSUPPORTED;
     const long P = (long)D * H * W;
     if (B <= 0 || B > 65535 || O <= 0 || I <= 0 || (I % 16) || D <= 0 || H <= 0 || W <= 0 || P < 96 || P > K19_MAX_PLANE)
         return MLAGG_E_UNSUPPORTED;
@@ -732,12 +753,12 @@
     }
     if (tp == 3) tp = 2 - (W & 1);
     switch (to * 4 + tp) {
-    case 1 * 4 + 1: launch<1, 1>(x, img, bias, y, g, dt, st); break;
-    case 1 * 4 + 2: launch<1, 2>(x, img, bias, y, g, dt, st); break;
-    case 2 * 4 + 1: launch<2, 1>(x, img, bias, y, g, dt, st); break;
-    case 2 * 4 + 2: launch<2, 2>(x, img, bias, y, g, dt, st); break;
-    case 3 * 4 + 1: launch<3, 1>(x, img, bias, y, g, dt, st); break;
-    default: launch<3, 2>(x, img, bias, y, g, dt, st); break;
+    case 1 * 4 + 1: launch<1, 1>(x, img, bias, res, y, yact, g, dt, st); break;
+    case 1 * 4 + 2: launch<1, 2>(x, img, bias, res, y, yact, g, dt, st); break;
+    case 2 * 4 + 1: launch<2, 1>(x, img, bias, res, y, yact, g, dt, st); break;
+    case 2 * 4 + 2: launch<2, 2>(x, img, bias, res, y, yact, g, dt, st); break;
+    case 3 * 4 + 1: launch<3, 1>(x, img, bias, res, y, yact, g, dt, st); break;
+    default: launch<3, 2>(x, img, bias, res, y, yact, g, dt, st); break;
     }
     return (int)hipGetLastError();
 }
@@ -754,13 +775,22 @@
 extern "C" int mlagg_conv3x3_fwd(const float *x, long x_batch, const float *w, int transposed, const float *bias, float *y,
                                  long y_batch, void *workspace, int B, int O, int I, int H, int W, void *stream)
 {
-    return conv_fwd(x, x_batch, w, transposed, bias, y, y_batch, workspace, B, O, I, 1, H, W, MLAGG_DTYPE_BF16X3, stream);
+    return conv_fwd(x, x_batch, w, transposed, bias, nullptr, y, nullptr, y_batch, workspace, B, O, I, 1, H, W, MLAGG_DTYPE_BF16X3, stream);
 }
 
 extern "C" int mlagg_conv3x3_fwd_lp(const float *x, long x_batch, const float *w, int transposed, const float *bias, float *y,
                                     long y_batch, void *workspace, int B, int O, int I, int H, int W, int dtype, void *stream)
 {
-    return conv_fwd(x, x_batch, w, transposed, bias, y, y_batch, workspace, B, O, I, 1, H, W, dtype, stream);
+    return conv_fwd(x, x_batch, w, transposed, bias, nullptr, y, nullptr, y_batch, workspace, B, O, I, 1, H, W, dtype, stream);
+}
+
+extern "C" int mlagg_conv3x3_fwd_epi(const float *x, long x_batch, const float *w, const float *bias, const float *res, float *y,
+                                     float *y_act, long y_batch, void *workspace, int B, int O, int I, int H, int W, int dtype, int act,
+                                     void *stream)
+{
+    if (act != 0 && act != 1) return MLAGG_E_UNSUPPORTED;
+    if (act == 1 && !y_act) return MLAGG_E_NULLPTR;
+    return conv_fwd(x, x_batch, w, 0, bias, res, y, act ? y_act : nullptr, y_batch, workspace, B, O, I, 1, H, W, dtype, stream);
 }
 
 extern "C" int mlagg_conv3x3x3_supported(int O, int I, int D, int H, int W)
@@ -775,7 +805,7 @@
                                    long y_batch, void *workspace, int B, int O, int I, int D, int H, int W, void *stream)
 {
     if (D <= 1) return MLAGG_E_UNSUPPORTED;
-    return conv_fwd(x, x_batch, w, transposed, bias, y, y_batch, workspace, B, O, I, D, H, W, MLAGG_DTYPE_BF16X3, stream);
+    return conv_fwd(x, x_batch, w, transposed, bias, nullptr, y, nullptr, y_batch, workspace, B, O, I, D, H, W, MLAGG_DTYPE_BF16X3, stream);
 }
 
 extern "C" int mlagg_conv3x3_wgrad_supported(int O, int I, int H, int W)
diff --git a/mlagg-unet_amd/csrc/gelu.h b/mlagg-unet_amd/csrc/gelu.h
--- /dev/null
+++ b/mlagg-unet_amd/csrc/gelu.h
@@ -0,0 +1,13 @@
+#pragma once
+#include <hip/hip_runtime.h>
+
+namespace mlagg_internal {
+
+__device__ __forceinline__ float gelu_f(float x) { return 0.5f * x * (1.f + erff(x * 0.70710678118654752f)); }
+__device__ __forceinline__ float gelu_grad_f(float x)
+{
+    const float cdf = 0.5f * (1.f + erff(x * 0.70710678118654752f));
+    return cdf + x * 0.3989422804014327f * __expf(-0.5f * x * x);
+}
+
+}
diff --git a/mlagg-unet_amd/model.py b/mlagg-unet_amd/model.py
--- a/mlagg-unet_amd/model.py
+++ b/mlagg-unet_amd/model.py
@@ -106,6 +106,10 @@
         return ops.conv2d(x, self.weight, self.stride, self.padding, self.dilation, self.groups, self.transposed, self.output_padding,
                           form)
 
+    def _native_epilogue(self, x, res, act):
+        return ops.conv2d_epilogue(x, self.weight, self.bias, res, act, self.stride, self.padding, self.dilation, self.groups,
+                                   self.transposed, self.output_padding, ops.conv_form())
+
     def raw(self, x):
         y = self._native(x, ops.conv_form())
         if y is None:
@@ -118,6 +122,9 @@
             y = self._eager(x)
             y = y if res is None else y + res
             return F.gelu(y) if act == ops.EPI_GELU else y
+        y = self._native_epilogue(x, res, act)
+        if y is not None:
+            return y
         y = self.raw(x)
         if y.dtype == torch.float32:
             return ops.channel_epilogue(y, self.bias, res if res is None or res.dtype == torch.float32 else res.float(), act)
@@ -126,6 +133,9 @@
         return ops.channel_epilogue_lp(y, self.bias, res, act, dtype or torch.float32)
 
     def _device_forward(self, x):
+        y = None if self.bias is None else self._native_epilogue(x, None, ops.EPI_NONE)
+        if y is not None:
+            return y
         y = self.raw(x)
         if y.dtype == torch.float32:
             return y if self.bias is None else ops.channel_bias(y, self.bias)
diff --git a/mlagg-unet_amd/ops.py b/mlagg-unet_amd/ops.py
--- a/mlagg-unet_amd/ops.py
+++ b/mlagg-unet_amd/ops.py
@@ -1827,7 +1827,7 @@
     return I == I16 and P >= K18_FWD_MIN_PIXELS and I >= K18_FWD_MIN_K
 
 
-def _conv1x1_k18(x, xb, w, y, B, O, I, P, form, accumulate=False):
+def _conv1x1_k18(x, xb, w, y, B, O, I, P, form, accumulate=False, epi=None):
     if y is None:
         y = torch.empty((B, O) + tuple(x.shape[2:]), device=x.device, dtype=torch.float32)
     I16 = -(-I // 16) * 16
@@ -1836,6 +1836,11 @@
         wp[:, :I] = w
         w = wp
     _flop("K18", 2 * B * O * I * P)
+    if epi is not None:
+        bias, res, y_act = epi
+        _launch("mlagg_conv1x1_fwd_epi", _ptr(x), xb, _ptr(w), _ptr(bias), _ptr(res), _ptr(y), _ptr(y_act), O * P, B, O, I16, I, P, form,
+                int(y_act is not None))
+        return y
     _launch("mlagg_conv1x1_fwd_acc", _ptr(x), xb, _ptr(w), None, _ptr(y), O * P, B, O, I16, I, P, form, int(accumulate))
     return y
 
@@ -1865,20 +1870,23 @@
     @staticmethod
     def backward(ctx, dy):
         x, w = ctx.saved_tensors
-        B, I = x.shape[:2]
-        O = w.shape[0]
-        dy, dyb, P = _planes(dy, "dy")
-        form = ctx.form
-        dx = dW = None
-        if ctx.needs_input_grad[0]:
-            if ctx.plan[1]:
-                wt = transpose_2d(w.unsqueeze(0))[0]
-                dx = _conv1x1_k18(dy, dyb, wt, None, B, I, O, P, form)
-            else:
-                dx = _lib_conv_bwd(dy, x, w.view(ctx.wshape), 1, 0, False, (True, False, False), form)[0]
-        if ctx.needs_input_grad[1]:
-            dW = _conv1x1_wgrad(dy, dyb, x, B, O, I, P, form).view(ctx.wshape)
-        return dx, dW, None, None
+        return _conv1x1_backward(x, w, ctx.wshape, ctx.plan, ctx.form, dy, ctx.needs_input_grad[0], ctx.needs_input_grad[1]) + (None, None)
+
+
+def _conv1x1_backward(x, w, wshape, plan, form, dy, need_dx, need_dw):
+    B, I = x.shape[:2]
+    O = w.shape[0]
+    dy, dyb, P = _planes(dy, "dy")
+    dx = dW = None
+    if need_dx:
+        if plan[1]:
+            wt = transpose_2d(w.unsqueeze(0))[0]
+            dx = _conv1x1_k18(dy, dyb, wt, None, B, I, O, P, form)
+        else:
+            dx = _lib_conv_bwd(dy, x, w.view(wshape), 1, 0, False, (True, False, False), form)[0]
+    if need_dw:
+        dW = _conv1x1_wgrad(dy, dyb, x, B, O, I, P, form).view(wshape)
+    return dx, dW
 
 
 def _conv1x1_plan(O, I, P, form):
@@ -1949,11 +1957,16 @@
     return tuple("K19" if on else None for on in (_k19_product(O, I, H, W, form), _k19_product(I, O, H, W, form), _k19_wgrad(O, I, H, W, form)))
 
 
-def _conv3x3_k19(x, xb, w, transposed, O, I, H, W, form, out=None):
+def _conv3x3_k19(x, xb, w, transposed, O, I, H, W, form, out=None, epi=None):
     B = x.shape[0]
     y = torch.empty(B, O, H, W, device=x.device, dtype=torch.float32) if out is None else out
     ws = torch.empty(_lib.lib().mlagg_conv3x3_workspace_bytes(O, I), device=x.device, dtype=torch.uint8)
     _flop("K19", 2 * 9 * B * O * I * H * W)
+    if epi is not None:
+        bias, res, y_act = epi
+        _launch("mlagg_conv3x3_fwd_epi", _ptr(x), xb, _ptr(w), _ptr(bias), _ptr(res), _ptr(y), _ptr(y_act), y.stride(0), _ptr(ws), B, O, I,
+                H, W, form, int(y_act is not None))
+        return y
     _launch("mlagg_conv3x3_fwd_lp", _ptr(x), xb, _ptr(w), int(transposed), None, _ptr(y), y.stride(0), _ptr(ws), B, O, I, H, W, form)
     return y
 
@@ -1976,28 +1989,32 @@
     @staticmethod
     def backward(ctx, dy):
         x, w = ctx.saved_tensors
-        B, I, H, W = x.shape
-        O = w.shape[0]
-        (_, dgrad, wgrad), form = ctx.plan, ctx.form
-        dx = dW = None
-        if ctx.needs_input_grad[0]:
-            if dgrad:
-                dy, dyb, _ = _planes(dy, "dy")
-                out = ctx.slot.view() if ctx.slot is not None else None
-                dx = _conv3x3_k19(dy, dyb, w, True, I, O, H, W, form, out)
-            else:
-                dx = _lib_conv_bwd(dy, x, w, 1, 1, False, (True, False, False), form)[0]
-        if ctx.needs_input_grad[1]:
-            if wgrad:
-                lib = _lib.lib()
-                dy, dyb, _ = _planes(dy, "dy")
-                dW = torch.empty(O, I, 3, 3, device=x.device, dtype=torch.float32)
-                ws = torch.empty(lib.mlagg_conv3x3_wgrad_workspace_floats(B, O, I, H, W), device=x.device, dtype=torch.float32)
-                _flop("K19", 2 * 9 * B * O * I * H * W)
-                _launch("mlagg_conv3x3_wgrad_lp", _ptr(dy), dyb, _ptr(x), x.stride(0), _ptr(dW), _ptr(ws), B, O, I, H, W, form)
-            else:
-                dW = _lib_conv_bwd(dy.contiguous(), x, w, 1, 1, False, (False, True, False), form)[1]
-        return dx, dW, None, None, None
+        return _conv3x3_backward(x, w, ctx.plan, ctx.form, ctx.slot, dy, ctx.needs_input_grad[0], ctx.needs_input_grad[1]) + (None,) * 3
+
+
+def _conv3x3_backward(x, w, plan, form, slot, dy, need_dx, need_dw):
+    B, I, H, W = x.shape
+    O = w.shape[0]
+    _, dgrad, wgrad = plan
+    dx = dW = None
+    if need_dx:
+        if dgrad:
+            dy, dyb, _ = _planes(dy, "dy")
+            out = slot.view() if slot is not None else None
+            dx = _conv3x3_k19(dy, dyb, w, True, I, O, H, W, form, out)
+        else:
+            dx = _lib_conv_bwd(dy, x, w, 1, 1, False, (True, False, False), form)[0]
+    if need_dw:
+        if wgrad:
+            lib = _lib.lib()
+            dy, dyb, _ = _planes(dy, "dy")
+            dW = torch.empty(O, I, 3, 3, device=x.device, dtype=torch.float32)
+            ws = torch.empty(lib.mlagg_conv3x3_wgrad_workspace_floats(B, O, I, H, W), device=x.device, dtype=torch.float32)
+            _flop("K19", 2 * 9 * B * O * I * H * W)
+            _launch("mlagg_conv3x3_wgrad_lp", _ptr(dy), dyb, _ptr(x), x.stride(0), _ptr(dW), _ptr(ws), B, O, I, H, W, form)
+        else:
+            dW = _lib_conv_bwd(dy.contiguous(), x, w, 1, 1, False, (False, True, False), form)[1]
+    return dx, dW
 
 
 K19T = _os.environ.get("MLAGG_K19T", "1") == "1"
@@ -2117,6 +2134,77 @@
     if transposed:
         return ConvT3x3S2Fn.apply(x, weight, form, plan)
     return Conv3x3Fn.apply(x, weight, form, claim_slot(x), plan)
+
+
+CONV_EPI = _os.environ.get("MLAGG_CONV_EPI", "1") == "1"
+
+
+def conv_epilogue_fused(plan, kernel, transposed):
+    if not CONV_EPI or plan is None:
+        return False
+    return (kernel == 1 and plan[0] == "K18") or (kernel == 3 and not transposed and plan[0] == "K19")
+
+
+class ConvEpilogueFn(torch.autograd.Function):
+
+    @staticmethod
+    def forward(ctx, x, weight, bias, res, act, form, slot, plan):
+        k = int(weight.shape[2])
+        x, xb, P = _planes(x, "x")
+        B, I = x.shape[:2]
+        O = weight.shape[0]
+        y = torch.empty((B, O) + tuple(x.shape[2:]), device=x.device, dtype=torch.float32)
+        res = None if res is None else _require(res.contiguous(), "res", y.shape)
+        y_act = torch.empty_like(y) if act == EPI_GELU else None
+        if k == 1:
+            w = _require(weight.reshape(O, I).contiguous(), "weight")
+            _conv1x1_k18(x, xb, w, y, B, O, I, P, form, epi=(bias, res, y_act))
+        else:
+            w = _require(weight.contiguous(), "weight")
+            _conv3x3_k19(x, xb, w, False, O, I, x.shape[2], x.shape[3], form, out=y, epi=(bias, res, y_act))
+        ctx.k, ctx.wshape, ctx.plan, ctx.form, ctx.slot = k, weight.shape, plan, form, slot
+        ctx.meta = (int(act), bias is not None, res is not None)
+        if act == EPI_GELU:
+            ctx.save_for_backward(x, w, y)
+            return y_act
+        ctx.save_for_backward(x, w)
+        return y
+
+    @staticmethod
+    def backward(ctx, dy):
+        act, has_bias, has_res = ctx.meta
+        dy = _require(dy.contiguous(), "dy")
+        B, C = dy.shape[:2]
+        hw = dy.numel() // (B * C)
+        db = torch.empty(C, device=dy.device, dtype=torch.float32) if has_bias else None
+        ws = torch.empty(_lib.lib().mlagg_channel_sum_workspace_floats(B, C), device=dy.device, dtype=torch.float32) if has_bias else None
+        if act == EPI_GELU:
+            x, w, pre = ctx.saved_tensors
+            g = torch.empty_like(dy)
+            _launch("mlagg_channel_gelu_bwd", _ptr(pre), _ptr(dy), _ptr(g), _ptr(db), _ptr(ws), B, C, hw)
+        else:
+            x, w = ctx.saved_tensors
+            g = dy
+            if has_bias:
+                _launch("mlagg_channel_sum", _ptr(dy), _ptr(db), _ptr(ws), B, C, hw)
+        need_dx, need_dw = ctx.needs_input_grad[0], ctx.needs_input_grad[1]
+        if ctx.k == 1:
+            dx, dW = _conv1x1_backward(x, w, ctx.wshape, ctx.plan, ctx.form, g, need_dx, need_dw)
+        else:
+            dx, dW = _conv3x3_backward(x, w, ctx.plan, ctx.form, ctx.slot, g, need_dx, need_dw)
+        return dx, dW, db, (g if has_res else None), None, None, None, None
+
+
+def conv2d_epilogue(x, weight, bias, res, act, stride, padding, dilation, groups, transposed, output_padding, form):
+    plan = conv_plan(x, weight, stride, padding, dilation, groups, transposed, output_padding, form)
+    k = int(weight.shape[2])
+    if not conv_epilogue_fused(plan, k, transposed):
+        return None
+    if res is not None and res.dtype != torch.float32:
+        res = res.float()
+    if k == 1:
+        return ConvEpilogueFn.apply(x, weight.permute(1, 0, 2, 3) if transposed else weight, bias, res, act, form, None, plan)
+    return ConvEpilogueFn.apply(x, weight, bias, res, act, form, claim_slot(x), plan)
 
 
 def conv1x1_supported(x, weight, stride, padding, dilation, groups, form=_DTYPE_BF16X3):
```

Measured after the change: 271.9 images/sec. 0.958x the previous value.
